# oakink/OakInk2-TaMF

Measured on AMD Instinct MI355X. Metric: sampled motion frames/s (1000-step DDPM, arch_mdm_l), higher is better.
Workload: dtype f16x3; 1 GPU; arch_mdm_l B=64/GPU T=196 1000-step DDPM (BASELINE.json configs[1]: arch_mdm_l B=64 T=196 1000-step DDPM on 1 GPU); step = one full reverse loop; headline dtype f16x3 = split-fp16 operands, fp32-TOLERANCE mode (1e-5 vs the reference, checked in-run); the same workload in the reference's own fp32 arithmetic is under roofline.reference_arithmetic (and the top-level fp32 entry); preset=2, clips_per_gpu=64, frames=196, ddpm_steps=1000, global_clips=64, parallelism=single GPU, world_size_seen=1, hipgraph=True, kernels_per_ddpm_step=43

## Files before the change

### oakink2-tamf_amd/csrc/tamf_attn.h

```cpp
#pragma once
#include "tamf_device.h"

template <class Op>
struct AttnArgs {
  const typename Op::elem_t* qk;
  const typename Op::elem_t* vt;
  typename Op::elem_t* out;
  int S, Sp, Skp, d, H;
  int abl;
  int ksplit, nwq, hw;
};

template <class Op, int HD>
struct AttnCfg {
  static constexpr int EB = Op::EB;
  static constexpr int KROWB = HD * EB;
  static constexpr int KG = KROWB / 128;
  static constexpr int VROWB = 32 * EB;
  static constexpr int VSTR = VROWB;
  static constexpr int K_BYTES = 32 * KROWB;
  static constexpr int V_BYTES = HD * VSTR;
  static constexpr int STAGE = K_BYTES + V_BYTES;
  static constexpr int SMEM = 2 * STAGE;
  static_assert(KROWB % 128 == 0, "head slice must be whole 128-byte groups");
};

template <class Op, int HD>
struct AttnBlock {
  typedef AttnCfg<Op, HD> C;
  static constexpr int EB = Op::EB, KG = C::KG, NT16 = HD / 16;
  static constexpr int KCH = C::KROWB / 16;
  static constexpr int VCH = C::VROWB / 16;
  static TAMF_DEV int kswz(int ch, int row) {
    if constexpr (C::KROWB >= 256) return (ch & ~15) | ((ch ^ row) & 15);
    else return ch ^ ((row >> 1) & 7);
  }
  static TAMF_DEV int vswz(int ch, int e) {
    if constexpr (C::VROWB == 128) return ch ^ ((e >> 1) & 7);
    else return ch ^ swz_chunk<64>(e);
  }
  static constexpr int K_RPP = 1024 / C::KROWB, K_PIECES = C::K_BYTES / 1024;
  static constexpr int V_RPP = 1024 / C::VROWB, V_PIECES = C::V_BYTES / 1024;

  static TAMF_DEV void issue(char* __restrict__ st, const char* kbase, const char* vbase, int kb, int Sp, int d, int Skp,
                             int wave, int nw, int lane) {
    for (int q = wave; q < K_PIECES; q += nw) {
      const int r = q * K_RPP + lane / KCH, pc = lane % KCH;
      int key = kb * 32 + r;
      key = key < Sp ? key : Sp - 1;
      __builtin_amdgcn_global_load_lds((const __attribute__((address_space(1))) void*)(kbase + (long)key * (2 * d) * EB + kswz(pc, r) * 16),
                                       (__attribute__((address_space(3))) void*)(st + q * 1024), 16, 0, 0);
    }
    for (int q = wave; q < V_PIECES; q += nw) {
      const int e = q * V_RPP + lane / VCH, pc = lane % VCH;
      __builtin_amdgcn_global_load_lds((const __attribute__((address_space(1))) void*)(vbase + ((long)e * Skp + kb * 32) * EB + vswz(pc, e) * 16),
                                       (__attribute__((address_space(3))) void*)(st + C::K_BYTES + q * 1024), 16, 0, 0);
    }
  }

  static TAMF_DEV void run(const char* __restrict__ cur, char* __restrict__ nxt, const char* kbase, const char* vbase,
                           int kb, int nkb, int S, int Sp, int d, int Skp, int wave, int nw, int lane, bool active,
                           const int4 (&qf)[KG][2], f32x4 (&o)[NT16], float& m_run, float& l_run) {
    const int lr = lane & 15, g = lane >> 4;
    const char* Ks = cur;
    const char* Vs = cur + C::K_BYTES;
    if (kb + 1 < nkb) issue(nxt, kbase, vbase, kb + 1, Sp, d, Skp, wave, nw, lane);
    if (!active) return;

    f32x4 st[2];
#pragma unroll
    for (int t = 0; t < 2; ++t) {
      st[t] = f32x4{0.f, 0.f, 0.f, 0.f};
      const int row = t * 16 + lr;
#pragma unroll
      for (int kg = 0; kg < KG; ++kg) {
        int4 kf[2];
        kf[0] = *(const int4*)(Ks + row * C::KROWB + kswz(kg * 8 + g, row) * 16);
        kf[1] = *(const int4*)(Ks + row * C::KROWB + kswz(kg * 8 + 4 + g, row) * 16);
        Op::mma(st[t], kf, qf[kg]);
      }
    }
    if (kb == nkb - 1) {
#pragma unroll
      for (int t = 0; t < 2; ++t)
#pragma unroll
        for (int r = 0; r < 4; ++r)
          if (kb * 32 + t * 16 + 4 * g + r >= S) st[t][r] = -1e30f;
    }
    float bm = fmaxf(fmaxf(fmaxf(st[0][0], st[0][1]), fmaxf(st[0][2], st[0][3])),
                     fmaxf(fmaxf(st[1][0], st[1][1]), fmaxf(st[1][2], st[1][3])));
    bm = groups_reduce<RedMax>(bm);
    constexpr float RESCALE_LOG2 = 8.0f;
    if (__builtin_amdgcn_ballot_w64(bm > m_run + RESCALE_LOG2) != 0ull) {
      const float m_new = fmaxf(m_run, bm);
      const float alpha = __builtin_amdgcn_exp2f(m_run - m_new);
      l_run *= alpha;
      m_run = m_new;
#pragma unroll
      for (int nt = 0; nt < NT16; ++nt) o[nt] *= alpha;
    }
    float ps = 0.f;
#pragma unroll
    for (int t = 0; t < 2; ++t)
#pragma unroll
      for (int r = 0; r < 4; ++r) {
        st[t][r] = __builtin_amdgcn_exp2f(st[t][r] - m_run);
        ps += st[t][r];
      }
    ps = groups_reduce<RedSum>(ps);
    l_run += ps;

    if constexpr (Op::PREC == 0) {
#pragma unroll
      for (int nt = 0; nt < NT16; ++nt) {
        const int e = nt * 16 + lr;
#pragma unroll
        for (int t = 0; t < 2; ++t) {
          const int4 vf = *(const int4*)(Vs + e * C::VSTR + vswz(t * 4 + g, e) * 16);
          o[nt] = __builtin_amdgcn_mfma_f32_16x16x4f32(as_f(vf.x), st[t][0], o[nt], 0, 0, 0);
          o[nt] = __builtin_amdgcn_mfma_f32_16x16x4f32(as_f(vf.y), st[t][1], o[nt], 0, 0, 0);
          o[nt] = __builtin_amdgcn_mfma_f32_16x16x4f32(as_f(vf.z), st[t][2], o[nt], 0, 0, 0);
          o[nt] = __builtin_amdgcn_mfma_f32_16x16x4f32(as_f(vf.w), st[t][3], o[nt], 0, 0, 0);
        }
      }
    } else {
      uint32_t wh[4], wl[4];
#pragma unroll
      for (int j = 0; j < 4; ++j) {
        const float p0 = st[(2 * j) >> 2][(2 * j) & 3], p1 = st[(2 * j + 1) >> 2][(2 * j + 1) & 3];
        Op::split2(p0, p1, wh[j], wl[j]);
      }
      const int4 ph = make_int4((int)wh[0], (int)wh[1], (int)wh[2], (int)wh[3]);
      const int4 pl = make_int4((int)wl[0], (int)wl[1], (int)wl[2], (int)wl[3]);
#pragma unroll
      for (int nt = 0; nt < NT16; ++nt) {
        const int e = nt * 16 + lr;
        const int4 vh = *(const int4*)(Vs + e * C::VSTR + vswz(g, e) * 16);
        if constexpr (Op::SPLIT) {
          const int4 vl = *(const int4*)(Vs + e * C::VSTR + vswz(4 + g, e) * 16);
          o[nt] = Op::mfma1(vl, ph, o[nt]);
          o[nt] = Op::mfma1(vh, pl, o[nt]);
        }
        o[nt] = Op::mfma1(vh, ph, o[nt]);
      }
    }
  }
};

#ifdef TAMF_TIMELINE
__device__ unsigned long long g_attn_ts[8192 * 4];
#endif

template <class Op, int HD>
__global__ __launch_bounds__(1024) void attn_kernel(const AttnArgs<Op> aa) {
  TAMF_TS(ts0);
  typedef AttnCfg<Op, HD> C;
  typedef AttnBlock<Op, HD> BLK;
  constexpr int EB = Op::EB, KG = C::KG;
  constexpr int NT16 = HD / 16;
  extern __shared__ __attribute__((aligned(16))) char smem[];

  const int tid = threadIdx.x, nthr = blockDim.x;
  const int lane = tid & 63, nw = nthr >> 6;
  const int wave = __builtin_amdgcn_readfirstlane(tid >> 6);
  const int lr = lane & 15, g = lane >> 4;
  const int bh = blockIdx.y, b = bh / aa.H, h = bh % aa.H;
  const int q0 = (blockIdx.x * nw + wave) * 16;
  const bool active = q0 < aa.Sp;
  const int S = aa.S, Sp = aa.Sp, d = aa.d;
  const long row_base = (long)b * Sp;

  int4 qf[KG][2];
  {
    int q = q0 + lr;
    q = q < Sp ? q : Sp - 1;
    const char* qb = (const char*)aa.qk + ((row_base + q) * (2 * d) + h * HD) * EB + g * 16;
#pragma unroll
    for (int kg = 0; kg < KG; ++kg) {
      qf[kg][0] = *(const int4*)(qb + kg * 128);
      qf[kg][1] = *(const int4*)(qb + kg * 128 + 64);
    }
  }

  f32x4 o[NT16];
#pragma unroll
  for (int nt = 0; nt < NT16; ++nt) o[nt] = f32x4{0.f, 0.f, 0.f, 0.f};
  float m_run = -1e30f, l_run = 0.f;

  const int nkb = (S + 31) / 32;
  const char* kbase = (const char*)aa.qk + (row_base * (2 * d) + d + h * HD) * EB;
  const char* vbase = (const char*)aa.vt + ((long)bh * HD) * aa.Skp * EB;

  BLK::issue(smem, kbase, vbase, 0, Sp, d, aa.Skp, wave, nw, lane);
  __syncthreads();
  TAMF_TS(ts1);
  for (int kb = 0; kb < nkb; ++kb) {
    BLK::run(smem + (kb & 1) * C::STAGE, smem + ((kb + 1) & 1) * C::STAGE, kbase, vbase, kb, nkb, S, Sp, d, aa.Skp, wave, nw,
             lane, active, qf, o, m_run, l_run);
    __syncthreads();
  }
#ifdef TAMF_TIMELINE
  if (tid == 0) {
    const int wg = blockIdx.y * gridDim.x + blockIdx.x;
    if (wg < 8192) {
      g_attn_ts[wg * 4 + 0] = ts0;
      g_attn_ts[wg * 4 + 1] = ts1;
      g_attn_ts[wg * 4 + 2] = wall_clock64();
      g_attn_ts[wg * 4 + 3] = tamf_hw_cu_id();
    }
  }
#endif

  if (!active) return;
  const int q = q0 + lr;
  if (q >= Sp) return;
  const float inv = 1.0f / l_run;
#pragma unroll
  for (int nt = 0; nt < NT16; ++nt) {
    float v[4] = {o[nt][0] * inv, o[nt][1] * inv, o[nt][2] * inv, o[nt][3] * inv};
    Op::template store<4>(aa.out, (row_base + q) * d + h * HD + nt * 16 + 4 * g, v);
  }
}

TAMF_DEV int attn_xcd_remap(int bid, int nblk) {
  const int q = nblk >> 3, r = nblk & 7, x = bid & 7, i = bid >> 3;
  return (x < r ? x * (q + 1) : r * (q + 1) + (x - r) * q) + i;
}

constexpr int attn_res_maxw(int nkb) { return nkb <= 4 ? 8 : 16; }
template <class Op, int HD, int NKB_>
struct AttnRes {
  typedef AttnCfg<Op, HD> C;
  typedef AttnBlock<Op, HD> BLK;
  static constexpr int EB = Op::EB, KG = C::KG, NT16 = HD / 16;
  static constexpr int NKB = NKB_, NKT = 2 * NKB;
  static constexpr int MAXW = attn_res_maxw(NKB_);
  static constexpr int S_MIN = NKB_ <= 4 ? 1 : NKB_ <= 6 ? 129 : 193;
  static constexpr int LDS_MAX = 160 * 1024;
  static constexpr bool TWO = Op::SPLIT || Op::PREC == 0;

  static int k_bytes(int Sp) { return Sp * C::KROWB; }
  static int nv1(int Sp, int nkb) {
    const int fit = (LDS_MAX - k_bytes(Sp)) / C::V_BYTES;
    return fit < nkb ? fit : nkb;
  }
  static bool fits(int S, int Sp) {
    const int nkb = (S + 31) / 32;
    if (nkb > NKB || S < S_MIN || Sp > NKT * 16 || (k_bytes(Sp) % 1024) != 0) return false;
    const int n1 = nv1(Sp, nkb);
    return n1 >= 1 && (nkb - n1) * C::V_BYTES <= k_bytes(Sp);
  }
  static int smem(int S, int Sp) {
    const int need = k_bytes(Sp) + nv1(Sp, (S + 31) / 32) * C::V_BYTES, rows = NKT * 16 * C::KROWB;
    return need > rows ? need : rows;
  }

  static constexpr int TPC_ = EB == 4 ? 2 : 4, NCH_ = (NT16 + TPC_ - 1) / TPC_, TPCE_ = NT16 < TPC_ ? NT16 : TPC_;
  static constexpr int KSPLIT_BYTES = NCH_ * 3 * TPCE_ * 1024 + 512;
  static int ksplit_extra(int S, int Sp, int nwq) {
    const int nkb = (S + 31) / 32, n1 = nv1(Sp, nkb), base = smem(S, Sp);
    int extra;
    if (n1 < nkb) {
      const int end = k_bytes(Sp) + nwq * 2048 + KSPLIT_BYTES;
      extra = end > base ? end - base : 0;
    } else {
      extra = KSPLIT_BYTES;
    }
    return base + extra <= LDS_MAX ? extra : -1;
  }

  static TAMF_DEV void issue_k(char* Ks, const char* kbase, int r0, int r1, int d, int wave, int nw, int lane) {
    const int q0 = r0 / BLK::K_RPP, np = r1 / BLK::K_RPP;
    for (int q = q0 + wave; q < np; q += nw) {
      const int r = q * BLK::K_RPP + lane / BLK::KCH, pc = lane % BLK::KCH;
      __builtin_amdgcn_global_load_lds((const __attribute__((address_space(1))) void*)(kbase + (long)r * (2 * d) * EB + BLK::kswz(pc, r) * 16),
                                       (__attribute__((address_space(3))) void*)(Ks + q * 1024), 16, 0, 0);
    }
  }
  static TAMF_DEV void issue_v(char* dst, const char* vbase, int kb0, int kb1, int Skp, int wave, int nw, int lane) {
    const int np = (kb1 - kb0) * BLK::V_PIECES;
    for (int q = wave; q < np; q += nw) {
      const int kb = kb0 + q / BLK::V_PIECES, qq = q % BLK::V_PIECES;
      const int e = qq * BLK::V_RPP + lane / BLK::VCH, pc = lane % BLK::VCH;
      __builtin_amdgcn_global_load_lds((const __attribute__((address_space(1))) void*)(vbase + ((long)e * Skp + kb * 32) * EB + BLK::vswz(pc, e) * 16),
                                       (__attribute__((address_space(3))) void*)(dst + q * 1024), 16, 0, 0);
    }
  }

  struct KOff { int o[KG][2]; };
  static TAMF_DEV KOff koff(int lr, int g) {
    KOff k;
#pragma unroll
    for (int kg = 0; kg < KG; ++kg) {
      k.o[kg][0] = lr * C::KROWB + BLK::kswz(kg * 8 + g, lr) * 16;
      k.o[kg][1] = lr * C::KROWB + BLK::kswz(kg * 8 + 4 + g, lr) * 16;
    }
    return k;
  }
  static TAMF_DEV void kfrag(const char* Ks, int i, const KOff& ko, int4 (&kf)[2]) {
    const int kt = i / KG, kg = i % KG;
    kf[0] = *(const int4*)(Ks + kt * (16 * C::KROWB) + ko.o[kg][0]);
    kf[1] = *(const int4*)(Ks + kt * (16 * C::KROWB) + ko.o[kg][1]);
  }
  template <int T0, int T1>
  static TAMF_DEV void scores(const char* __restrict__ Ks, char* __restrict__ K2, char* __restrict__ Vs, const char* kbase,
                              const char* vbase, int k2r0, int k2r1, int d, int n1, int Skp, int wave, int nw, int lane,
                              const int4 (&qf)[KG][2], f32x4 (&st)[NKT], int abl, unsigned mask = ~0u) {
    const int lr = lane & 15, g = lane >> 4;
    if (T0 == 0 && !(abl & 1)) {
      if (k2r1 > k2r0) issue_k(K2 - (long)k2r0 * C::KROWB, kbase, k2r0, k2r1, d, wave, nw, lane);
      issue_v(Vs, vbase, 0, n1, Skp, wave, nw, lane);
    }
    constexpr int F0 = T0 * KG, NF = T1 * KG, LA = 2;
    const KOff ko = koff(lr, g);
    int4 kf[LA + 1][2];
#pragma unroll
    for (int i = 0; i <= LA; ++i) kf[i][0] = kf[i][1] = qf[0][0];
    auto on = [&](int i) { return ((mask >> (i / KG / 2)) & 1u) != 0; };
#pragma unroll
    for (int i = F0; i < F0 + LA; ++i)
      if (!(abl & 4) && on(i)) kfrag(Ks, i, ko, kf[i % (LA + 1)]);
#pragma unroll
    for (int i = F0; i < NF; ++i) {
      if (i + LA < NF && !(abl & 4) && on(i + LA)) kfrag(Ks, i + LA, ko, kf[(i + LA) % (LA + 1)]);
      __builtin_amdgcn_sched_barrier(0);
      if (on(i)) {
        if (i % KG == 0) st[i / KG] = f32x4{0.f, 0.f, 0.f, 0.f};
        if (!(abl & 2)) Op::mma(st[i / KG], kf[i % (LA + 1)], qf[i % KG]);
      }
      __builtin_amdgcn_sched_barrier(0);
    }
  }
  static TAMF_DEV void vfrag(const char* vb, int nt, int vo0, int vo1, int4 (&vf)[2]) {
    vf[0] = *(const int4*)(vb + nt * (16 * C::VSTR) + vo0);
    if constexpr (TWO) vf[1] = *(const int4*)(vb + nt * (16 * C::VSTR) + vo1);
  }
  static TAMF_DEV void pv(const char* __restrict__ Vs, char* __restrict__ dma_dst, const char* vbase, int kb0, int kb1, int dkb0,
                          int dkb1, int Skp, int wave, int nw, int lane, const uint32_t (&ph)[NKB][4], const uint32_t (&pl)[NKB][4],
                          f32x4 (&o)[NT16], int abl, unsigned mask = ~0u) {
    const int lr = lane & 15, g = lane >> 4;
    const int vo0 = lr * C::VSTR + BLK::vswz(g, lr) * 16, vo1 = lr * C::VSTR + BLK::vswz(4 + g, lr) * 16;
    if (dkb1 > dkb0 && !(abl & 1)) issue_v(dma_dst, vbase, dkb0, dkb1, Skp, wave, nw, lane);
#pragma unroll
    for (int kb = 0; kb < NKB; ++kb) {
      if (kb >= kb0 && kb < kb1 && ((mask >> kb) & 1u)) {
        const char* vb = Vs + (kb - kb0) * C::V_BYTES;
        const int4 p_h = make_int4((int)ph[kb][0], (int)ph[kb][1], (int)ph[kb][2], (int)ph[kb][3]);
        const int4 p_l = make_int4((int)pl[kb][0], (int)pl[kb][1], (int)pl[kb][2], (int)pl[kb][3]);
        constexpr int LA = 2;
        int4 vf[LA + 1][2];
#pragma unroll
        for (int nt = 0; nt <= LA; ++nt) vf[nt][0] = vf[nt][1] = p_h;
#pragma unroll
        for (int nt = 0; nt < LA; ++nt)
          if (!(abl & 4)) vfrag(vb, nt, vo0, vo1, vf[nt]);
#pragma unroll
        for (int nt = 0; nt < NT16; ++nt) {
          if (nt + LA < NT16 && !(abl & 4)) vfrag(vb, nt + LA, vo0, vo1, vf[(nt + LA) % (LA + 1)]);
          __builtin_amdgcn_sched_barrier(0);
          const int4 vh = vf[nt % (LA + 1)][0];
          if (!(abl & 2)) {
            if constexpr (Op::PREC == 0) {
              const int4 v1 = vf[nt % (LA + 1)][1];
              o[nt] = __builtin_amdgcn_mfma_f32_16x16x4f32(as_f(vh.x), __builtin_bit_cast(float, ph[kb][0]), o[nt], 0, 0, 0);
              o[nt] = __builtin_amdgcn_mfma_f32_16x16x4f32(as_f(vh.y), __builtin_bit_cast(float, ph[kb][1]), o[nt], 0, 0, 0);
              o[nt] = __builtin_amdgcn_mfma_f32_16x16x4f32(as_f(vh.z), __builtin_bit_cast(float, ph[kb][2]), o[nt], 0, 0, 0);
              o[nt] = __builtin_amdgcn_mfma_f32_16x16x4f32(as_f(vh.w), __builtin_bit_cast(float, ph[kb][3]), o[nt], 0, 0, 0);
              o[nt] = __builtin_amdgcn_mfma_f32_16x16x4f32(as_f(v1.x), __builtin_bit_cast(float, pl[kb][0]), o[nt], 0, 0, 0);
              o[nt] = __builtin_amdgcn_mfma_f32_16x16x4f32(as_f(v1.y), __builtin_bit_cast(float, pl[kb][1]), o[nt], 0, 0, 0);
              o[nt] = __builtin_amdgcn_mfma_f32_16x16x4f32(as_f(v1.z), __builtin_bit_cast(float, pl[kb][2]), o[nt], 0, 0, 0);
              o[nt] = __builtin_amdgcn_mfma_f32_16x16x4f32(as_f(v1.w), __builtin_bit_cast(float, pl[kb][3]), o[nt], 0, 0, 0);
            } else {
              if constexpr (Op::SPLIT) {
                const int4 vl = vf[nt % (LA + 1)][1];
                o[nt] = Op::mfma1(vl, p_h, o[nt]);
                o[nt] = Op::mfma1(vh, p_l, o[nt]);
              }
              o[nt] = Op::mfma1(vh, p_h, o[nt]);
            }
          }
          __builtin_amdgcn_sched_barrier(0);
        }
      }
    }
  }
};

template <class Op, int HD, int NKB_>
__global__ __launch_bounds__(attn_res_maxw(NKB_) * 64) void attn_res_kernel(const AttnArgs<Op> aa) {
  typedef AttnCfg<Op, HD> C;
  typedef AttnRes<Op, HD, NKB_> R;
  constexpr int EB = Op::EB, KG = C::KG, NT16 = HD / 16, NKB = R::NKB, NKT = R::NKT;
  extern __shared__ __attribute__((aligned(16))) char smem[];

  const int tid = threadIdx.x, nthr = blockDim.x;
  const int lane = tid & 63, nw = nthr >> 6;
  const int wave = __builtin_amdgcn_readfirstlane(tid >> 6);
  const int lr = lane & 15, g = lane >> 4;
  int bh = blockIdx.y;
  if (gridDim.x == 1 && !(TAMF_ABL(aa.abl) & 32)) bh = attn_xcd_remap(bh, gridDim.y);
  const int b = bh / aa.H, h = bh % aa.H;
  const int S = aa.S, Sp = aa.Sp, d = aa.d;
  const int nwq = aa.ksplit ? aa.nwq : nw;
  const int nqt = (Sp + 15) / 16;
  const int nqt_own = aa.ksplit ? nqt - 1 : nqt;
  int tile = blockIdx.x * nwq + wave;
  int hq = -1;
  unsigned kmask = ~0u;
  bool idle = wave >= nwq || tile >= nqt_own;
  if (aa.ksplit && blockIdx.x == gridDim.x - 1) {
#pragma unroll
    for (int j = 0; j < 4; ++j)
      if (wave == ((aa.hw >> (4 * j)) & 15)) hq = j;
    if (hq >= 0) { idle = false; tile = nqt - 1; kmask = 0x11111111u << hq; }
  }
  if (idle) { kmask = 0u; tile = nqt - 1; }
  const int q0 = tile * 16;
  const long row_base = (long)b * Sp;
  const int nkb = (S + 31) / 32;
  const int kbytes = Sp * C::KROWB;
  int n1 = (R::LDS_MAX - kbytes) / C::V_BYTES;
  n1 = n1 < nkb ? n1 : nkb;
  char* Ks = smem;
  char* Vs = smem + kbytes;

  const char* kbase = (const char*)aa.qk + (row_base * (2 * d) + d + h * HD) * EB;
  const char* vbase = (const char*)aa.vt + ((long)bh * HD) * aa.Skp * EB;

  int4 qf[KG][2];
  {
    int q = q0 + lr;
    q = q < Sp ? q : Sp - 1;
    const char* qb = (const char*)aa.qk + ((row_base + q) * (2 * d) + h * HD) * EB + g * 16;
#pragma unroll
    for (int kg = 0; kg < KG; ++kg) {
      qf[kg][0] = *(const int4*)(qb + kg * 128);
      qf[kg][1] = *(const int4*)(qb + kg * 128 + 64);
    }
  }
  const int abl = TAMF_ABL(aa.abl);
  constexpr int TH = NKT / 2;
  const int kh = TH * 16 < Sp ? TH * 16 : Sp;
  if (!(abl & 1)) R::issue_k(Ks, kbase, 0, kh, d, wave, nw, lane);
  __syncthreads();

  f32x4 st[NKT];
  if (kmask != ~0u) {
#pragma unroll
    for (int kt = 0; kt < NKT; ++kt) st[kt] = f32x4{-1e30f, -1e30f, -1e30f, -1e30f};
  }
  R::template scores<0, TH>(Ks, Ks + (long)kh * C::KROWB, Vs, kbase, vbase, kh, Sp, d, n1, aa.Skp, wave, nw, lane, qf, st, abl, kmask);
  __syncthreads();
  R::template scores<TH, NKT>(Ks, Vs, Vs, kbase, vbase, 0, 0, d, 0, aa.Skp, wave, nw, lane, qf, st, abl, kmask);

#pragma unroll
  for (int kt = 0; kt < NKT; ++kt)
    if (kt * 16 + 15 >= R::S_MIN) {
#pragma unroll
      for (int r = 0; r < 4; ++r) st[kt][r] = (kt * 16 + 4 * g + r >= S) ? -1e30f : st[kt][r];
    }
  float m = -1e30f;
#pragma unroll
  for (int kt = 0; kt < NKT; ++kt) m = fmaxf(m, fmaxf(fmaxf(st[kt][0], st[kt][1]), fmaxf(st[kt][2], st[kt][3])));
  m = groups_reduce<RedMax>(m);
  float l = 0.f;
  uint32_t ph[NKB][4], pl[NKB][4];
#pragma unroll
  for (int kb = 0; kb < NKB; ++kb) {
#pragma unroll
    for (int t = 0; t < 2; ++t)
#pragma unroll
      for (int r = 0; r < 4; ++r) {
        const float p = (abl & 8) ? st[2 * kb + t][r] : __builtin_amdgcn_exp2f(st[2 * kb + t][r] - m);
        st[2 * kb + t][r] = p;
        l += p;
      }
#pragma unroll
    for (int j = 0; j < 4; ++j) {
      if constexpr (Op::PREC == 0) {
        const float p0 = st[2 * kb][j], p1 = st[2 * kb + 1][j];
        ph[kb][j] = __builtin_bit_cast(uint32_t, p0);
        pl[kb][j] = __builtin_bit_cast(uint32_t, p1);
      } else {
        if (abl & 8) { const float pa = st[2 * kb + (j >> 1)][(2 * j) & 3]; ph[kb][j] = pl[kb][j] = __builtin_bit_cast(uint32_t, pa); }
        else Op::split2(st[2 * kb + (j >> 1)][(2 * j) & 3], st[2 * kb + (j >> 1)][((2 * j) & 3) + 1], ph[kb][j], pl[kb][j]);
      }
    }
  }
  l = groups_reduce<RedSum>(l);

  f32x4 o[NT16];
#pragma unroll
  for (int nt = 0; nt < NT16; ++nt) o[nt] = f32x4{0.f, 0.f, 0.f, 0.f};

  __syncthreads();
  R::pv(Vs, Ks, vbase, 0, n1, n1, nkb, aa.Skp, wave, nw, lane, ph, pl, o, abl, kmask);
  if (n1 < nkb) {
    __syncthreads();
    R::pv(Ks, Vs, vbase, n1, nkb, 0, 0, aa.Skp, wave, nw, lane, ph, pl, o, abl, kmask);
  }
  if (idle) {
    if (aa.ksplit) __syncthreads();
    return;
  }

  if ((abl & 16) && l != 12345.0f) return;
  constexpr int TPC = Op::EB == 4 ? 2 : 4;
  constexpr int NCH = (NT16 + TPC - 1) / TPC, TPCE = NT16 < TPC ? NT16 : TPC;
  if (hq >= 0) {
    const int base_bytes = kbytes + n1 * C::V_BYTES > NKT * 16 * C::KROWB ? kbytes + n1 * C::V_BYTES : NKT * 16 * C::KROWB;
    char* part = n1 < nkb ? Vs + nwq * 2048 : smem + base_bytes;
    float* ml = (float*)(part + NCH * 3 * TPCE * 1024);
    if (g == 0) { ml[hq * 32 + lr] = m; ml[hq * 32 + 16 + lr] = l; }
#pragma unroll
    for (int ch = 0; ch < NCH; ++ch)
      if (ch != hq) {
        const int src = hq < ch ? hq : hq - 1;
#pragma unroll
        for (int tl = 0; tl < TPCE; ++tl) *(f32x4*)(part + ((ch * 3 + src) * TPCE + tl) * 1024 + lane * 16) = o[ch * TPC + tl];
      }
    __syncthreads();
    if (hq >= NCH || q0 + lr >= Sp) return;
    float mi[4], li[4], mg = -1e30f;
#pragma unroll
    for (int i = 0; i < 4; ++i) { mi[i] = ml[i * 32 + lr]; li[i] = ml[i * 32 + 16 + lr]; mg = fmaxf(mg, mi[i]); }
    float w[4], lg = 0.f;
#pragma unroll
    for (int i = 0; i < 4; ++i) { w[i] = __builtin_amdgcn_exp2f(mi[i] - mg); lg += li[i] * w[i]; }
    const float invg = 1.0f / lg;
    char* grow = (char*)aa.out + ((row_base + q0 + lr) * d + h * HD) * EB + hq * 128;
#pragma unroll
    for (int ch = 0; ch < NCH; ++ch) {
      if (ch != hq) continue;
#pragma unroll
      for (int tl = 0; tl < TPCE; ++tl) {
        f32x4 acc = f32x4{0.f, 0.f, 0.f, 0.f};
#pragma unroll
        for (int i = 0; i < 4; ++i) {
          const f32x4 mine = o[ch * TPC + tl];
          const f32x4 theirs = *(const f32x4*)(part + ((ch * 3 + (i < ch ? i : (i > 0 ? i - 1 : 0))) * TPCE + tl) * 1024 + lane * 16);
          const f32x4 oi = i == ch ? mine : theirs;
          acc += oi * w[i];
        }
        const float v0 = acc[0] * invg, v1 = acc[1] * invg, v2 = acc[2] * invg, v3 = acc[3] * invg;
        if constexpr (Op::PREC == 0) {
          *(int4*)(grow + (4 * tl + g) * 16) = make_int4(as_i(v0), as_i(v1), as_i(v2), as_i(v3));
        } else {
          uint32_t h0, l0, h1, l1;
          Op::split2(v0, v1, h0, l0);
          Op::split2(v2, v3, h1, l1);
          char* gp = grow + (2 * tl + (g >> 1)) * 16 + 8 * (g & 1);
          *(int2*)gp = make_int2((int)h0, (int)h1);
          if constexpr (Op::SPLIT) *(int2*)(gp + 64) = make_int2((int)l0, (int)l1);
        }
      }
    }
    return;
  }
  const float inv = 1.0f / l;
  constexpr int RS = 128;
  char* slot = (n1 < nkb ? Vs : Ks) + wave * (16 * RS);
  char* gout = (char*)aa.out + ((row_base + q0) * d + h * HD) * EB;
  const int srow = lane >> 3, spiece = lane & 7;
#pragma unroll
  for (int ch = 0; ch < NCH; ++ch) {
#pragma unroll
    for (int tl = 0; tl < TPCE; ++tl) {
      const int nt = ch * TPC + tl;
      const float v0 = o[nt][0] * inv, v1 = o[nt][1] * inv, v2 = o[nt][2] * inv, v3 = o[nt][3] * inv;
      if (q0 + lr >= Sp) continue;
      if constexpr (Op::PREC == 0) {
        const int c = 4 * tl + g;
        *(int4*)(slot + lr * RS + ((c ^ (lr & 7)) << 4)) = make_int4(as_i(v0), as_i(v1), as_i(v2), as_i(v3));
      } else {
        uint32_t h0, l0, h1, l1;
        Op::split2(v0, v1, h0, l0);
        Op::split2(v2, v3, h1, l1);
        const int c = 2 * tl + (g >> 1);
        char* sp = slot + lr * RS + 8 * (g & 1);
        *(int2*)(sp + ((c ^ (lr & 7)) << 4)) = make_int2((int)h0, (int)h1);
        if constexpr (Op::SPLIT) *(int2*)(sp + (((c + 4) ^ (lr & 7)) << 4)) = make_int2((int)l0, (int)l1);
      }
    }
#pragma unroll
    for (int i = 0; i < 2; ++i) {
      const int row = i * 8 + srow;
      const int4 w = *(const int4*)(slot + row * RS + ((spiece ^ (row & 7)) << 4));
      if (q0 + row < Sp && (NT16 >= TPC || spiece * 16 < NT16 * 16 * Op::EB))
        *(int4*)(gout + (long)row * d * EB + ch * 128 + spiece * 16) = w;
    }
  }
  if (aa.ksplit) __syncthreads();
}
```

### oakink2-tamf_amd/csrc/tamf_hip.hip

```cpp
#include "../../include/tamf_hip.h"

#include <hip/hip_runtime.h>

#include <algorithm>
#include <atomic>
#include <cmath>
#include <cstdio>
#include <cstdlib>
#include <cstring>
#include <map>
#include <mutex>
#include <string>
#include <type_traits>
#include <vector>

#include "tamf_attn.h"
#include "tamf_gemm.h"
#include "tamf_gemm_clip.h"
#include "tamf_gemm_deep.h"
#include "tamf_geom.h"
#include "tamf_misc.h"
#include "tamf_encoder.h"
#include "tamf_spectrum.h"
#include "tamf_shapes.h"
#include "tamf_weight_prep.h"

#define TAMF_WITH_OP(prec, EXPR)                                         \
  switch (prec) {                                                        \
    case TAMF_PREC_F32: { typedef OpF32 Op; EXPR; } break;               \
    case TAMF_PREC_BF16: { typedef OpBF16 Op; EXPR; } break;             \
    case TAMF_PREC_BF16X3: { typedef OpBF16X3 Op; EXPR; } break;         \
    default: { typedef OpF16X3 Op; EXPR; } break;                        \
  }

static thread_local std::string g_noctx_err;

struct OperandBuf {
  void* p = nullptr;
  float inv_scale = 1.0f;
};

struct LayerW {
  OperandBuf Win, Wout, W1, W2;
  float *c2_in = nullptr, *c2_ff = nullptr;
  float *g_att = nullptr, *bb_att = nullptr, *g_ffn = nullptr, *bb_ffn = nullptr;
};

struct GraphKey {
  int B = -1, T = -1, n_steps = -1, steps_per_graph = 0;
  bool operator==(const GraphKey& o) const {
    return B == o.B && T == o.T && n_steps == o.n_steps && steps_per_graph == o.steps_per_graph;
  }
};

struct GuardRec {
  char* base;
  size_t bytes, guard;
  const char* tag;
  bool ws;
};
static constexpr unsigned char GUARD_BYTE = 0xA5;
static std::atomic<size_t> g_guard_bytes{0};
static thread_local const char* g_alloc_tag = "";

struct Workspaces {
  int Bmax = 0, Tmax = 0;
  long Mmax = 0;
  float *xs = nullptr, *cobj = nullptr, *X = nullptr, *pstatic = nullptr;
  OperandBuf xs_op, h1_op, X_op, QK_op, Vt_op, A_op, H_op;
  void *X_st = nullptr, *xs_st = nullptr;
  int* tcur = nullptr;
  unsigned* status = nullptr;
  unsigned char* side_dev = nullptr;
  int* objnum_dev = nullptr;
  float2 *stat_att = nullptr, *stat_ffn = nullptr;
  LoopParams* loop_params = nullptr;
  std::vector<void*> ws_allocs;
};

struct tamf_ctx : Workspaces {
  tamf_arch arch{};
  int prec = 0, device = 0;
  int d = 0, ff = 0, L = 0, H = 0, hd = 0, P = 0, F = 0, has_t = 0;
  int XK = 0;
  int XN = 128;
  int EB = 4;
  std::string err;
  std::vector<void*> allocs;
  bool alloc_ws = false;
  std::vector<GuardRec> guards;
  std::map<std::string, std::vector<int64_t>> expected;
  std::map<std::string, std::vector<float>> raw;
  bool finalized = false, cond_set = false;
  int n_t = 0;
  int n_steps = 0;
  std::vector<float> h_c1, h_c2, h_sigma;
  float *c1 = nullptr, *c2 = nullptr, *sigma = nullptr;
  std::vector<LayerW> layers;
  OperandBuf Wfused, Wm2, Wf;
  float *bm2 = nullptr, *bf = nullptr;
  float* pe = nullptr;
  float* temb = nullptr;
  float* temb_loop = nullptr;
  int temb_loop_cap = 0;
  bool tmap_on = false, in_loop = false;
  int tmap_max = -1;
  OperandBuf Wt1_f32, Wt2_f32;
  float *bt1 = nullptr, *bt2 = nullptr;
  float *WtxtT = nullptr, *btxt = nullptr, *WshapeT = nullptr, *bshape = nullptr, *WobjT = nullptr, *bobj = nullptr;
  float *WcT = nullptr, *bc = nullptr, *rh = nullptr, *lh = nullptr;
  int B = 0, T = 0, S = 0, Sp = 0, Skp = 0, M = 0;
  float* enc_w = nullptr;
  int enc_kin = 0;
  unsigned host_status = 0;
  std::string weight_note;
  hipStream_t cap_stream = nullptr;
  hipGraph_t graph = nullptr;
  hipGraphExec_t graph_exec = nullptr;
  GraphKey graph_key;
  hipEvent_t graph_done = nullptr;
  bool graph_in_flight = false;
  int sched_cap = 0;
  int graph_captures = 0, graph_launches_last_loop = 0;
  int step_kernels = 0;
  bool prof_on = false;
  std::vector<hipEvent_t> prof_ev;
  std::vector<std::string> prof_names;
  std::vector<double> prof_flops;
};

static std::vector<tamf_ctx*> g_live_ctx;
static std::mutex g_live_mu;
static std::recursive_mutex g_launch_mu;
#ifdef TAMF_TEST_HOOKS
#define TAMF_LAUNCH_LOCK std::lock_guard<std::recursive_mutex> launch_lock_(g_launch_mu)
#else
#define TAMF_LAUNCH_LOCK ((void)0)
#endif
#define TAMF_STATE_LOCK std::lock_guard<std::recursive_mutex> state_lock_(g_launch_mu)

static int fail(tamf_ctx* ctx, int code, const std::string& msg) {
  if (ctx) ctx->err = msg;
  else g_noctx_err = msg;
  return code;
}
static int launched() {
  const hipError_t e = hipGetLastError();
  return e == hipSuccess ? 0 : fail(nullptr, TAMF_ERR_HIP, hipGetErrorString(e));
}
enum : unsigned { KIND_G = 1u << TAMF_KIND_G, KIND_R = 1u << TAMF_KIND_R, KIND_E = 1u << TAMF_KIND_E };
static int need_kind(tamf_ctx* ctx, const char* func, unsigned mask) {
  if (!ctx) return fail(ctx, TAMF_ERR_INVALID, std::string(func) + ": null ctx");
  if (mask & (1u << ctx->arch.kind)) return 0;
  if (ctx->arch.kind == TAMF_KIND_E) return fail(ctx, TAMF_ERR_STATE, std::string(func) + ": not available on a SegmentEncoder (TAMF_KIND_E) context");
  return fail(ctx, TAMF_ERR_STATE, std::string(func) + (mask == KIND_E   ? " needs a SegmentEncoder (TAMF_KIND_E) context"
                                                        : mask == KIND_G ? " needs a G context"
                                                        : mask == KIND_R ? " needs an R context"
                                                                         : " needs a G or R context"));
}
#define HIPCHK(ctx, call)                                                                                         \
  do {                                                                                                            \
    hipError_t e_ = (call);                                                                                       \
    if (e_ != hipSuccess)                                                                                         \
      return fail(ctx, TAMF_ERR_HIP, std::string(#call) + ": " + hipGetErrorString(e_) + " (" + __FILE__ + ":" +  \
                                         std::to_string(__LINE__) + ")");                                        \
  } while (0)
#define TRY(expr)           \
  do {                      \
    int rc_ = (expr);       \
    if (rc_ != 0) return rc_; \
  } while (0)

static inline dim3 grid1d(long n, int bs = 256) { return dim3((unsigned)((n + bs - 1) / bs)); }

static std::atomic<int> g_fail_alloc_in{-1};
static int dev_alloc(tamf_ctx* ctx, void** p, size_t bytes, bool zero = false) {
  if (bytes == 0) bytes = 16;
  const size_t guard = g_guard_bytes.load();
  if (g_fail_alloc_in.load() >= 0 && g_fail_alloc_in.fetch_sub(1) == 0)
    return fail(ctx, TAMF_ERR_NOMEM, "hipMalloc failed: injected by tamf_test_fail_alloc_after");
  hipError_t e = hipMalloc(p, bytes + 2 * guard);
  if (e != hipSuccess) return fail(ctx, TAMF_ERR_NOMEM, std::string("hipMalloc failed: ") + hipGetErrorString(e));
  (ctx->alloc_ws ? ctx->ws_allocs : ctx->allocs).push_back(*p);
  if (guard) {
    char* base = (char*)*p;
    HIPCHK(ctx, hipMemset(base, GUARD_BYTE, guard));
    HIPCHK(ctx, hipMemset(base + guard + bytes, GUARD_BYTE, guard));
    ctx->guards.push_back(GuardRec{base, bytes, guard, g_alloc_tag, ctx->alloc_ws});
    *p = base + guard;
  }
  if (zero) HIPCHK(ctx, hipMemset(*p, 0, bytes));
  return 0;
}
template <class T>
static int dev_upload(tamf_ctx* ctx, T** p, const T* host, size_t n) {
  TRY(dev_alloc(ctx, (void**)p, n * sizeof(T)));
  HIPCHK(ctx, hipMemcpy(*p, host, n * sizeof(T), hipMemcpyHostToDevice));
  return 0;
}

static int upload_operand(tamf_ctx* ctx, int prec, const float* w, int N, int K, int ldk, OperandBuf* out, const char* what) {
  const PackedOperand po = pack_operand(prec, w, N, K, ldk);
  if (po.refused) return fail(ctx, po.error_code(), po.error_message(what));
  out->inv_scale = po.inv_scale;
  if (po.small_share_noted()) {
    ctx->host_status |= TAMF_STATUS_F16_WEIGHT_RANGE;
    if (ctx->weight_note.empty()) ctx->weight_note = po.range_note(what);
  }
  return dev_upload(ctx, (unsigned char**)&out->p, po.image.data(), po.image.size());
}
static int upload_vec(tamf_ctx* ctx, float** p, const std::vector<float>& v) { return dev_upload(ctx, p, v.data(), v.size()); }

#include "tamf_launch.h"

extern "C" const char* tamf_last_error(const tamf_ctx* ctx) { return ctx ? ctx->err.c_str() : g_noctx_err.c_str(); }

static int alloc_operand(tamf_ctx* ctx, OperandBuf* ob, long elems, bool zero = false) {
  return dev_alloc(ctx, &ob->p, (size_t)elems * ctx->EB, zero);
}

static int check_dims(const tamf_arch* arch, int max_batch, int max_frames) {
  if (max_batch <= 0 || max_frames <= 0 || max_frames > 4990) return fail(nullptr, TAMF_ERR_INVALID, "bad max_batch/max_frames");
  if (!dims_fit_32bit_offsets(max_batch, max_frames, arch->ff_size, arch->latent_dim))
    return fail(nullptr, TAMF_ERR_INVALID, "max_batch x max_frames too large for one context (32-bit operand offsets): split the batch");
  return 0;
}

static int place_scratch_views(tamf_ctx* ctx, const ScratchLayout& sl) {
  char* host = (char*)ctx->H_op.p;
  ctx->QK_op.p = host + sl.qk_off;
  ctx->A_op.p = host + sl.a_off;
  ctx->h1_op.p = host + sl.h1_off;
  const size_t guard = g_guard_bytes.load();
  if (!guard) return 0;
  const struct { size_t off, bytes; const char* tag; } views[3] = {{(size_t)sl.qk_off, (size_t)sl.qk_bytes, "view QK_op of H_op's allocation"},
                                                                  {(size_t)sl.a_off, (size_t)sl.a_bytes, "view A_op of H_op's allocation"},
                                                                  {(size_t)sl.h1_off, (size_t)sl.h1_bytes, "view h1_op of H_op's allocation"}};
  for (const auto& v : views) {
    HIPCHK(ctx, hipMemset(host + v.off - guard, GUARD_BYTE, guard));
    ctx->guards.push_back(GuardRec{host + v.off - guard, v.bytes, guard, v.tag, true});
  }
  return 0;
}

static int alloc_workspaces(tamf_ctx* ctx, int max_batch, int max_frames) {
  const int d = ctx->d;
  const SeqShape smax = seq_shape_max(max_frames, ctx->P);
  const long BT = (long)max_batch * max_frames;
  const long Mmax = (long)max_batch * smax.Sp;
  ctx->Mmax = Mmax;
  ctx->Bmax = max_batch;
  ctx->Tmax = max_frames;
  ctx->alloc_ws = true;
  int rc = 0;
#define A(call)             \
  do {                      \
    g_alloc_tag = #call;    \
    if (rc == 0) rc = call; \
  } while (0)
  A(dev_alloc(ctx, (void**)&ctx->xs, BT * ctx->XK * 4, true));
  if (ctx->prec == TAMF_PREC_F32) ctx->xs_op.p = ctx->xs;
  else { A(alloc_operand(ctx, &ctx->xs_op, BT * ctx->XK, true)); ctx->xs_st = ctx->xs_op.p; }
  A(dev_alloc(ctx, (void**)&ctx->cobj, BT * d * 4));
  const ScratchLayout sl = scratch_layout(Mmax, BT, d, ctx->ff, ctx->EB, g_guard_bytes.load());
  if (!sl.alias) A(alloc_operand(ctx, &ctx->h1_op, BT * d));
  A(dev_alloc(ctx, (void**)&ctx->X, Mmax * d * 4, true));
  if (ctx->prec == TAMF_PREC_F32) ctx->X_op.p = ctx->X;
  else { A(alloc_operand(ctx, &ctx->X_op, Mmax * d, true)); ctx->X_st = ctx->X_op.p; }
  if (!sl.alias) A(alloc_operand(ctx, &ctx->QK_op, Mmax * 2 * d, true));
  A(alloc_operand(ctx, &ctx->Vt_op, (long)max_batch * d * smax.Skp, true));
  if (!sl.alias) A(alloc_operand(ctx, &ctx->A_op, Mmax * d, true));
  if (!sl.alias) A(alloc_operand(ctx, &ctx->H_op, Mmax * ctx->ff, true));
  else {
    A(dev_alloc(ctx, &ctx->H_op.p, sl.host_bytes, true));
    A(place_scratch_views(ctx, sl));
  }
  A(dev_alloc(ctx, (void**)&ctx->pstatic, (long)max_batch * ctx->P * d * 4, true));
  A(dev_alloc(ctx, (void**)&ctx->tcur, (long)max_batch * 4, true));
  A(dev_alloc(ctx, (void**)&ctx->status, 16, true));
  A(dev_alloc(ctx, (void**)&ctx->side_dev, max_batch, true));
  A(dev_alloc(ctx, (void**)&ctx->objnum_dev, (long)max_batch * 4, true));
  A(dev_alloc(ctx, (void**)&ctx->stat_att, Mmax * (d / 32) * 8, true));
  A(dev_alloc(ctx, (void**)&ctx->stat_ffn, Mmax * (d / 32) * 8, true));
  A(dev_alloc(ctx, (void**)&ctx->loop_params, sizeof(LoopParams), true));
#undef A
  g_alloc_tag = "(weights / tables)";
  ctx->alloc_ws = false;
  return rc;
}

static int enc_max_frames(int ff, int kin) {
  int t = 0;
  while (t < 5000 && enc_lds_bytes(t + 1 + ENC_P + 1, ff, kin) <= ENC_LDS_BYTES) ++t;
  return t;
}
static int enc_check_shape(const tamf_arch* a, int max_batch, int max_frames) {
  if (a->latent_dim != ENC_D || a->num_heads != 4)
    return fail(nullptr, TAMF_ERR_INVALID, "SegmentEncoder (TAMF_KIND_E): latent_dim must be 64 with num_heads 4 (head dim 16)");
  if (a->ff_size < 16 || a->ff_size > 512 || a->ff_size % 16)
    return fail(nullptr, TAMF_ERR_INVALID, "SegmentEncoder (TAMF_KIND_E): ff_size must be a multiple of 16 in [16, 512]");
  if (a->num_layers < 1 || a->num_layers > 64) return fail(nullptr, TAMF_ERR_INVALID, "SegmentEncoder (TAMF_KIND_E): num_layers must be in [1, 64]");
  if (a->input_dim < 1 || a->input_dim > 128 || a->obj_input_dim < 1 || a->obj_input_dim > 16 || a->hand_shape_dim < 1 ||
      a->hand_shape_dim > 64 || a->obj_embed_dim < 1 || a->obj_embed_dim > 4096)
    return fail(nullptr, TAMF_ERR_INVALID, "SegmentEncoder (TAMF_KIND_E): input_dim must be in [1, 128], obj_input_dim in [1, 16], "
                                           "hand_shape_dim in [1, 64], obj_embed_dim in [1, 4096]");
  if (max_batch <= 0 || max_batch > (1 << 20) || max_frames <= 0) return fail(nullptr, TAMF_ERR_INVALID, "bad max_batch/max_frames");
  const int tmax = enc_max_frames(a->ff_size, round_up(a->input_dim + a->obj_input_dim, 4));
  if (max_frames > tmax)
    return fail(nullptr, TAMF_ERR_INVALID, "SegmentEncoder (TAMF_KIND_E): max_frames " + std::to_string(max_frames) + " exceeds the limit of " +
                                               std::to_string(tmax) + " frames (a clip's token rows live in the 160 KiB LDS of one CU)");
  return 0;
}
static int enc_alloc_workspaces(tamf_ctx* ctx, int max_batch, int max_frames) {
  ctx->Bmax = max_batch;
  ctx->Tmax = max_frames;
  ctx->alloc_ws = true;
  g_alloc_tag = "encoder workspaces";
  int rc = dev_alloc(ctx, (void**)&ctx->pstatic, (size_t)max_batch * ENC_P * ctx->d * 4, true);
  if (rc == 0) rc = dev_alloc(ctx, (void**)&ctx->objnum_dev, (size_t)max_batch * 4, true);
  g_alloc_tag = "(weights / tables)";
  ctx->alloc_ws = false;
  return rc;
}
static int alloc_workspaces_of_kind(tamf_ctx* ctx, int max_batch, int max_frames) {
  return ctx->arch.kind == TAMF_KIND_E ? enc_alloc_workspaces(ctx, max_batch, max_frames) : alloc_workspaces(ctx, max_batch, max_frames);
}

static int enc_check_create(const tamf_arch* arch, int max_batch, int max_frames, int precision) {
  if (precision != TAMF_PREC_F32) return fail(nullptr, TAMF_ERR_INVALID, "SegmentEncoder (TAMF_KIND_E) runs in fp32 only (TAMF_PREC_F32)");
  return enc_check_shape(arch, max_batch, max_frames);
}
static int gr_check_arch(const tamf_arch* arch, int precision) {
  const int d = arch->latent_dim;
  if (!(d == 128 || d == 256 || d == 512)) return fail(nullptr, TAMF_ERR_INVALID, "latent_dim must be 128, 256 or 512");
  if (arch->num_heads <= 0 || d % arch->num_heads) return fail(nullptr, TAMF_ERR_INVALID, "bad num_heads");
  const int hd = d / arch->num_heads;
  if (!(hd == 64 || hd == 128)) return fail(nullptr, TAMF_ERR_INVALID, "head dim (latent_dim/num_heads) must be 64 or 128");
  if (arch->ff_size <= 0 || arch->ff_size % 128) return fail(nullptr, TAMF_ERR_INVALID, "ff_size must be a multiple of 128");
  if (arch->num_layers <= 0 || arch->num_layers > 64) return fail(nullptr, TAMF_ERR_INVALID, "bad num_layers");
  if (arch->input_dim <= 0 || arch->input_dim > 128) return fail(nullptr, TAMF_ERR_INVALID, "input_dim must be in [1,128]");
  if (precision < 0 || precision > TAMF_PREC_F16X3) return fail(nullptr, TAMF_ERR_INVALID, "unknown precision");
  if (arch->kind != TAMF_KIND_G && arch->kind != TAMF_KIND_R) return fail(nullptr, TAMF_ERR_INVALID, "unknown model kind");
  return 0;
}
static int enc_prepare(tamf_ctx* ctx) {
  hipError_t e = lds_once<encoder_kernel>((int)ENC_LDS_BYTES);
  if (e != hipSuccess) return fail(ctx, TAMF_ERR_HIP, std::string("encoder kernel attribute setup failed: ") + hipGetErrorString(e));
  return 0;
}
static int gr_prepare(tamf_ctx* ctx) {
  {
    int cus = 0;
    if (hipDeviceGetAttribute(&cus, hipDeviceAttributeMultiprocessorCount, ctx->device) == hipSuccess && cus > 0)
      g_wg_slots_dev[ctx->device & 63].store(2 * cus, std::memory_order_relaxed);
  }
  hipError_t pe;
  {
    TAMF_STATE_LOCK;
    pe = prepare_all<OpF32>();
    if (pe == hipSuccess && ctx->prec != TAMF_PREC_F32) TAMF_WITH_OP(ctx->prec, pe = prepare_all<Op>());
  }
  if (pe != hipSuccess) return fail(ctx, TAMF_ERR_HIP, std::string("kernel attribute setup failed: ") + hipGetErrorString(pe));
  if (hipStreamCreateWithFlags(&ctx->cap_stream, hipStreamNonBlocking) != hipSuccess) return fail(ctx, TAMF_ERR_HIP, "hipStreamCreate failed");
  return 0;
}

extern "C" int tamf_ctx_create(const tamf_arch* arch, int32_t max_batch, int32_t max_frames, int32_t precision,
                               int32_t device, tamf_ctx** out) {
  if (!arch || !out) return fail(nullptr, TAMF_ERR_INVALID, "null argument");
  *out = nullptr;
  const bool enc = arch->kind == TAMF_KIND_E;
  if (int rc = enc ? enc_check_create(arch, max_batch, max_frames, precision) : gr_check_arch(arch, precision)) return rc;
  int ndev = 0;
  hipError_t de = hipGetDeviceCount(&ndev);
  if (de != hipSuccess || ndev <= 0)
    return fail(nullptr, TAMF_ERR_HIP, std::string("no HIP device visible (") + hipGetErrorString(de) +
                                           "): libtamf_hip has no CPU fallback");
  if (device < 0 || device >= ndev) return fail(nullptr, TAMF_ERR_INVALID, "device index out of range");
  if (!enc)
    if (int rc = check_dims(arch, max_batch, max_frames)) return rc;

  tamf_ctx* ctx = new tamf_ctx();
  ctx->arch = *arch;
  ctx->prec = precision;
  ctx->device = device;
  ctx->d = arch->latent_dim;
  ctx->ff = arch->ff_size;
  ctx->L = arch->num_layers;
  ctx->H = arch->num_heads;
  ctx->hd = arch->latent_dim / arch->num_heads;
  ctx->F = arch->input_dim;
  ctx->has_t = arch->kind == TAMF_KIND_G ? 1 : 0;
  ctx->EB = precision == TAMF_PREC_BF16 ? 2 : 4;
  if (enc) {
    ctx->P = ENC_P;
    ctx->enc_kin = round_up(arch->input_dim + arch->obj_input_dim, 4);
  } else {
    ctx->P = arch->kind == TAMF_KIND_G ? PREFIX_ROWS_G : PREFIX_ROWS_R;
    ctx->XK = arch->kind == TAMF_KIND_G ? 128 : round_up(arch->input_dim + arch->h2o_dim, 64);
    ctx->layers.resize(ctx->L);
  }
  ctx->expected = expected_shapes(ctx->arch);

  auto bail = [&](int rc) {
    std::string e = ctx->err;
    tamf_ctx_destroy(ctx);
    g_noctx_err = e;
    return rc;
  };
  if (hipSetDevice(device) != hipSuccess) return bail(fail(ctx, TAMF_ERR_HIP, "hipSetDevice failed"));
  if (int rc = enc ? enc_prepare(ctx) : gr_prepare(ctx)) return bail(rc);
  if (int rc = alloc_workspaces_of_kind(ctx, max_batch, max_frames)) return bail(rc);
  if (!enc && hipEventCreateWithFlags(&ctx->graph_done, hipEventDisableTiming) != hipSuccess)
    return bail(fail(ctx, TAMF_ERR_HIP, "hipEventCreate failed"));
  {
    std::lock_guard<std::mutex> lk(g_live_mu);
    g_live_ctx.push_back(ctx);
  }
  *out = ctx;
  return 0;
}

extern "C" void tamf_ctx_destroy(tamf_ctx* ctx) {
  if (!ctx) return;
  TAMF_LAUNCH_LOCK;
  {
    std::lock_guard<std::mutex> lk(g_live_mu);
    g_live_ctx.erase(std::remove(g_live_ctx.begin(), g_live_ctx.end(), ctx), g_live_ctx.end());
  }
  (void)hipSetDevice(ctx->device);
  (void)hipDeviceSynchronize();
  if (ctx->graph_done) (void)hipEventDestroy(ctx->graph_done);
  if (ctx->graph_exec) (void)hipGraphExecDestroy(ctx->graph_exec);
  if (ctx->graph) (void)hipGraphDestroy(ctx->graph);
  if (ctx->cap_stream) (void)hipStreamDestroy(ctx->cap_stream);
  for (void* p : ctx->allocs) (void)hipFree(p);
  for (void* p : ctx->ws_allocs) (void)hipFree(p);
  delete ctx;
}

static int retire_graph(tamf_ctx* ctx);

struct TakenWorkspaces {
  Workspaces ws;
  std::vector<GuardRec> guards;
};
static TakenWorkspaces ws_take(tamf_ctx* c) {
  TakenWorkspaces t;
  std::swap(t.ws, static_cast<Workspaces&>(*c));
  const auto first_ws = std::stable_partition(c->guards.begin(), c->guards.end(), [](const GuardRec& g) { return !g.ws; });
  t.guards.assign(first_ws, c->guards.end());
  c->guards.erase(first_ws, c->guards.end());
  return t;
}
static void ws_put(tamf_ctx* c, TakenWorkspaces& t) {
  std::swap(t.ws, static_cast<Workspaces&>(*c));
  c->guards.insert(c->guards.end(), t.guards.begin(), t.guards.end());
}
static void ws_free(const TakenWorkspaces& t) {
  for (void* p : t.ws.ws_allocs) (void)hipFree(p);
}

extern "C" int tamf_ctx_resize(tamf_ctx* ctx, int32_t max_batch, int32_t max_frames) {
  TAMF_LAUNCH_LOCK;
  if (!ctx) return fail(ctx, TAMF_ERR_INVALID, "null ctx");
  const bool enc = ctx->arch.kind == TAMF_KIND_E;
  if (int rc = enc ? enc_check_shape(&ctx->arch, max_batch, max_frames) : check_dims(&ctx->arch, max_batch, max_frames)) {
    ctx->err = g_noctx_err;
    return rc;
  }
  HIPCHK(ctx, hipSetDevice(ctx->device));
  HIPCHK(ctx, hipDeviceSynchronize());
  if (!enc) TRY(retire_graph(ctx));
  TakenWorkspaces old = ws_take(ctx);
  int rc = alloc_workspaces_of_kind(ctx, max_batch, max_frames);
  if (rc == 0 && old.ws.status && ctx->status &&
      hipMemcpy(ctx->status, old.ws.status, 16, hipMemcpyDeviceToDevice) != hipSuccess)
    rc = fail(ctx, TAMF_ERR_HIP, "tamf_ctx_resize: carrying the status word over failed");
  if (rc != 0) {
    const std::string why = ctx->err;
    ws_free(ws_take(ctx));
    ws_put(ctx, old);
    ctx->err = "tamf_ctx_resize(" + std::to_string(max_batch) + ", " + std::to_string(max_frames) + ") failed, the context keeps its " +
               std::to_string(ctx->Bmax) + " x " + std::to_string(ctx->Tmax) + " workspaces: " + why;
    return rc;
  }
  ws_free(old);
  if (!enc) {
    ctx->cond_set = false;
    ctx->B = ctx->T = ctx->S = ctx->Sp = ctx->Skp = ctx->M = 0;
  }
  return 0;
}

extern "C" int tamf_load_weight(tamf_ctx* ctx, const char* name, const float* host_data, const int64_t* shape,
                                int32_t ndim) {
  if (!ctx || !name || !host_data || !shape || ndim <= 0) return fail(ctx, TAMF_ERR_INVALID, "null/invalid argument");
  if (ctx->finalized) return fail(ctx, TAMF_ERR_STATE, "weights already finalised");
  const auto it = ctx->expected.find(name);
  if (it == ctx->expected.end()) return 0;
  std::vector<int64_t> shp(shape, shape + ndim);
  if (shp != it->second) return fail(ctx, TAMF_ERR_INVALID, std::string("shape mismatch for ") + name);
  int64_t n = 1;
  for (auto v : shp) n *= v;
  ctx->raw[name].assign(host_data, host_data + n);
  return 0;
}

static int upload_f32(tamf_ctx* ctx, const std::string& name, float** p) {
  const auto& v = ctx->raw.at(name);
  return dev_upload(ctx, p, v.data(), v.size());
}
static int upload_T(tamf_ctx* ctx, const std::string& name, int N, int K, float** p) {
  return upload_vec(ctx, p, transposed(ctx->raw.at(name).data(), N, K));
}
static int upload_prefix_tables(tamf_ctx* ctx) {
  const int d = ctx->d;
  TRY(upload_T(ctx, "hand_shape_process.shape_embed.weight", d, ctx->arch.hand_shape_dim, &ctx->WshapeT));
  TRY(upload_f32(ctx, "hand_shape_process.shape_embed.bias", &ctx->bshape));
  TRY(upload_T(ctx, "obj_embed_process.embedding.weight", d, ctx->arch.obj_embed_dim, &ctx->WobjT));
  TRY(upload_f32(ctx, "obj_embed_process.embedding.bias", &ctx->bobj));
  TRY(upload_f32(ctx, "hand_side_process.rh_embed", &ctx->rh));
  return upload_f32(ctx, "hand_side_process.lh_embed", &ctx->lh);
}
static int enc_finalize(tamf_ctx* ctx) {
  const int d = ctx->d, ff = ctx->ff, F = ctx->F, qd = ctx->arch.obj_input_dim, kin = ctx->enc_kin, hd = ctx->hd, H = ctx->H;
  auto R = [&](const std::string& n) -> const float* { return ctx->raw.at(n).data(); };
  const EncHeadOff ho = enc_head_off(kin, F);
  const EncLayerOff lo = enc_layer_off(ff);
  std::vector<float> w((size_t)(ho.layers + (long)ctx->L * lo.stride), 0.f);
  auto put = [&](long off, const std::string& n, size_t cnt) { memcpy(w.data() + off, R(n), cnt * 4); };
  put(ho.cls, "classification_token", d);
  {
    const float *Wm1 = R("input_merge.0.weight"), *bm1 = R("input_merge.0.bias");
    const float *Wp = R("input_process.poseEmbedding.weight"), *bp = R("input_process.poseEmbedding.bias");
    const float *Wq = R("obj_input_process.poseEmbedding.weight"), *bq = R("obj_input_process.poseEmbedding.bias");
    input_bias_two_terms_per_column(Wm1, d, bm1, bp, bq, w.data() + ho.bin);
    compose_block(Wm1, 2 * d, 0, d, Wp, F, w.data() + ho.win, kin, 1);
    compose_block(Wm1, 2 * d, d, d, Wq, qd, w.data() + ho.win + F, kin, 1);
  }
  put(ho.wm2, "input_merge.2.weight", (size_t)d * d);
  put(ho.bm2, "input_merge.2.bias", d);
  put(ho.p0, "output_process.poseFinal.0.weight", (size_t)d * d);
  put(ho.pb0, "output_process.poseFinal.0.bias", d);
  put(ho.p2, "output_process.poseFinal.2.weight", (size_t)d * d);
  put(ho.pb2, "output_process.poseFinal.2.bias", d);
  put(ho.p4, "output_process.poseFinal.4.weight", (size_t)F * d);
  put(ho.pb4, "output_process.poseFinal.4.bias", F);
  for (int l = 0; l < ctx->L; ++l) {
    const std::string p = "seqTransEncoder.layers." + std::to_string(l);
    const long base = ho.layers + (long)l * lo.stride;
    const float *Win = R(p + ".self_attn.in_proj_weight"), *bin = R(p + ".self_attn.in_proj_bias");
    for (int h = 0; h < H; ++h)
      for (int part = 0; part < 3; ++part)
        for (int j = 0; j < hd; ++j) {
          const int dst = h * 3 * hd + part * hd + j, src = part * d + h * hd + j;
          memcpy(w.data() + base + lo.wqkv + (long)dst * d, Win + (size_t)src * d, (size_t)d * 4);
          w[base + lo.bqkv + dst] = bin[src];
        }
    put(base + lo.wo, p + ".self_attn.out_proj.weight", (size_t)d * d);
    put(base + lo.bo, p + ".self_attn.out_proj.bias", d);
    put(base + lo.w1, p + ".linear1.weight", (size_t)ff * d);
    put(base + lo.b1, p + ".linear1.bias", ff);
    put(base + lo.w2, p + ".linear2.weight", (size_t)d * ff);
    put(base + lo.b2, p + ".linear2.bias", d);
    put(base + lo.g1, p + ".norm1.weight", d);
    put(base + lo.be1, p + ".norm1.bias", d);
    put(base + lo.g2, p + ".norm2.weight", d);
    put(base + lo.be2, p + ".norm2.bias", d);
  }
  TRY(dev_upload(ctx, &ctx->enc_w, w.data(), w.size()));
  TRY(upload_f32(ctx, "sequence_pos_encoder.pe", &ctx->pe));
  return upload_prefix_tables(ctx);
}

extern "C" int tamf_finalize_weights(tamf_ctx* ctx, int32_t max_timesteps, void* stream) {
  TAMF_LAUNCH_LOCK;
  if (!ctx) return fail(ctx, TAMF_ERR_INVALID, "null ctx");
  if (ctx->finalized) return fail(ctx, TAMF_ERR_STATE, "weights already finalised");
  if (max_timesteps <= 0 || max_timesteps > 5000) return fail(ctx, TAMF_ERR_INVALID, "max_timesteps must be in [1,5000]");
  HIPCHK(ctx, hipSetDevice(ctx->device));
  hipStream_t st = (hipStream_t)stream;
  for (const auto& kv : ctx->expected)
    if (!ctx->raw.count(kv.first)) return fail(ctx, TAMF_ERR_MISSING, "missing checkpoint tensor: " + kv.first);
  auto done = [&]() {
    ctx->raw.clear();
    ctx->expected.clear();
    ctx->finalized = true;
    if (!ctx->weight_note.empty()) ctx->err = ctx->weight_note;
    return 0;
  };
  if (ctx->arch.kind == TAMF_KIND_E) {
    TRY(enc_finalize(ctx));
    return done();
  }
  const int d = ctx->d, ff = ctx->ff, F = ctx->F, prec = ctx->prec;
  auto R = [&](const std::string& n) -> const float* { return ctx->raw.at(n).data(); };
  auto upload_folded = [&](const std::string& weight, const std::string& bias, int N, int Npad, const float* g, const float* be, OperandBuf* ob,
                           float** c2) -> int {
    const FoldedLinear f = fold_layernorm(R(weight), R(bias), N, Npad, d, g, be);
    TRY(upload_operand(ctx, prec, f.w.data(), Npad, d, d, ob, weight.c_str()));
    return upload_vec(ctx, c2, f.c2);
  };
  auto upload_residual_ln = [&](const float* g, const float* be, const std::string& bias, float** g_dev, float** bb_dev) -> int {
    const ResidualLn r = residual_ln(g, be, R(bias), d);
    TRY(upload_vec(ctx, g_dev, r.g));
    return upload_vec(ctx, bb_dev, r.bb);
  };

  for (int l = 0; l < ctx->L; ++l) {
    const std::string p = "seqTransEncoder.layers." + std::to_string(l);
    LayerW& w = ctx->layers[l];
    {
      const std::string pp = "seqTransEncoder.layers." + std::to_string(l - 1);
      const float* g_in = l ? R(pp + ".norm2.weight") : nullptr;
      const float* be_in = l ? R(pp + ".norm2.bias") : nullptr;
      const float* g1 = R(p + ".norm1.weight");
      const float* be1 = R(p + ".norm1.bias");
      TRY(upload_folded(p + ".self_attn.in_proj_weight", p + ".self_attn.in_proj_bias", 3 * d, 3 * d, g_in, be_in, &w.Win, &w.c2_in));
      TRY(upload_folded(p + ".linear1.weight", p + ".linear1.bias", ff, ff, g1, be1, &w.W1, &w.c2_ff));
      TRY(upload_residual_ln(g_in, be_in, p + ".self_attn.out_proj.bias", &w.g_att, &w.bb_att));
      TRY(upload_residual_ln(g1, be1, p + ".linear2.bias", &w.g_ffn, &w.bb_ffn));
    }
    TRY(upload_operand(ctx, prec, R(p + ".self_attn.out_proj.weight"), d, d, d, &w.Wout, (p + ".self_attn.out_proj.weight").c_str()));
    TRY(upload_operand(ctx, prec, R(p + ".linear2.weight"), d, ff, ff, &w.W2, (p + ".linear2.weight").c_str()));
  }
  {
    const bool isR = ctx->arch.kind == TAMF_KIND_R;
    const FusedInput fi = fuse_input(d, F, ctx->arch.obj_input_dim, ctx->arch.h2o_dim, ctx->XK, R("input_merge.0.weight"), R("input_merge.0.bias"),
                                     R("input_process.poseEmbedding.weight"), R("input_process.poseEmbedding.bias"),
                                     R("obj_input_process.poseEmbedding.weight"), R("obj_input_process.poseEmbedding.bias"),
                                     isR ? R("h2o_dist_input_process.poseEmbedding.weight") : nullptr,
                                     isR ? R("h2o_dist_input_process.poseEmbedding.bias") : nullptr);
    TRY(upload_operand(ctx, prec, fi.w.data(), d, ctx->XK, ctx->XK, &ctx->Wfused, "input_merge.0.weight x poseEmbedding.weight (fused)"));
    TRY(upload_vec(ctx, &ctx->WcT, fi.wct));
    TRY(upload_vec(ctx, &ctx->bc, fi.bias));
  }
  TRY(upload_operand(ctx, prec, R("input_merge.2.weight"), d, d, d, &ctx->Wm2, "input_merge.2.weight"));
  TRY(upload_f32(ctx, "input_merge.2.bias", &ctx->bm2));
  {
    const std::string pl = "seqTransEncoder.layers." + std::to_string(ctx->L - 1);
    TRY(upload_folded("output_process.poseFinal.weight", "output_process.poseFinal.bias", F, ctx->XN, R(pl + ".norm2.weight"), R(pl + ".norm2.bias"),
                      &ctx->Wf, &ctx->bf));
  }
  TRY(upload_f32(ctx, "sequence_pos_encoder.pe", &ctx->pe));
  if (ctx->arch.hand_shape_dim > 64 || ctx->arch.obj_input_dim > COBJ_QMAX || d > 1024)
    return fail(ctx, TAMF_ERR_INVALID, "hand_shape_dim > 64, obj_input_dim > 16 or latent_dim > 1024");
  TRY(upload_prefix_tables(ctx));
  if (ctx->has_t) {
    TRY(upload_T(ctx, "embed_text.weight", d, ctx->arch.clip_dim, &ctx->WtxtT));
    TRY(upload_f32(ctx, "embed_text.bias", &ctx->btxt));
    TRY(upload_operand(ctx, TAMF_PREC_F32, R("embed_timestep.time_embed.0.weight"), d, d, d, &ctx->Wt1_f32, "embed_timestep.time_embed.0.weight"));
    TRY(upload_operand(ctx, TAMF_PREC_F32, R("embed_timestep.time_embed.2.weight"), d, d, d, &ctx->Wt2_f32, "embed_timestep.time_embed.2.weight"));
    TRY(upload_f32(ctx, "embed_timestep.time_embed.0.bias", &ctx->bt1));
    TRY(upload_f32(ctx, "embed_timestep.time_embed.2.bias", &ctx->bt2));
    ctx->n_t = max_timesteps;
    float* tmp = nullptr;
    TRY(dev_alloc(ctx, (void**)&ctx->temb, (size_t)ctx->n_t * d * 4));
    TRY(dev_alloc(ctx, (void**)&tmp, (size_t)ctx->n_t * d * 4));
    GemmArgs<OpF32> g1{ctx->pe, d, (const float*)ctx->Wt1_f32.p, d, ctx->n_t, d, d, 0};
    EpiBiasAct<OpF32> e1{ctx->bt1, nullptr, 0, tmp, d, ACT_SILU};
    HIPCHK(ctx, gemm128<OpF32>(g1, e1, st));
    GemmArgs<OpF32> g2{tmp, d, (const float*)ctx->Wt2_f32.p, d, ctx->n_t, d, d, 0};
    EpiSeqRows<OpF32> e2{ctx->bt2, ctx->pe, 0, ctx->temb, nullptr, d, 0x7FFFFFFF, 0, 0, nullptr, nullptr, nullptr, 0, 0, 0};
    HIPCHK(ctx, gemm128<OpF32>(g2, e2, st));
  }
  HIPCHK(ctx, hipStreamSynchronize(st));
  return done();
}

static int retire_graph(tamf_ctx* ctx) {
  if (ctx->graph_in_flight) {
    HIPCHK(ctx, hipEventSynchronize(ctx->graph_done));
    ctx->graph_in_flight = false;
  }
  if (ctx->graph_exec) { (void)hipGraphExecDestroy(ctx->graph_exec); ctx->graph_exec = nullptr; }
  if (ctx->graph) { (void)hipGraphDestroy(ctx->graph); ctx->graph = nullptr; }
  ctx->graph_key = GraphKey();
  return 0;
}

extern "C" int tamf_set_schedule(tamf_ctx* ctx, int32_t n_steps, const double* c1, const double* c2, const double* logvar) {
  TAMF_LAUNCH_LOCK;
  TRY(need_kind(ctx, __func__, KIND_G | KIND_R));
  if (!c1 || !c2 || !logvar || n_steps <= 0) return fail(ctx, TAMF_ERR_INVALID, "null/invalid argument");
  HIPCHK(ctx, hipSetDevice(ctx->device));
  ctx->h_c1.resize(n_steps);
  ctx->h_c2.resize(n_steps);
  ctx->h_sigma.resize(n_steps);
  for (int i = 0; i < n_steps; ++i) {
    ctx->h_c1[i] = (float)c1[i];
    ctx->h_c2[i] = (float)c2[i];
    ctx->h_sigma[i] = expf(0.5f * (float)logvar[i]);
  }
  ctx->n_steps = n_steps;
  if (ctx->tmap_on) {
    TRY(retire_graph(ctx));
    ctx->tmap_on = false;
    ctx->tmap_max = -1;
  }
  if (n_steps > ctx->sched_cap) {
    TRY(retire_graph(ctx));
    const int cap = std::max(n_steps, 1000);
    TRY(dev_alloc(ctx, (void**)&ctx->c1, (size_t)cap * 4));
    TRY(dev_alloc(ctx, (void**)&ctx->c2, (size_t)cap * 4));
    TRY(dev_alloc(ctx, (void**)&ctx->sigma, (size_t)cap * 4));
    ctx->sched_cap = cap;
  }
  HIPCHK(ctx, hipDeviceSynchronize());
  HIPCHK(ctx, hipMemcpy(ctx->c1, ctx->h_c1.data(), (size_t)n_steps * 4, hipMemcpyHostToDevice));
  HIPCHK(ctx, hipMemcpy(ctx->c2, ctx->h_c2.data(), (size_t)n_steps * 4, hipMemcpyHostToDevice));
  HIPCHK(ctx, hipMemcpy(ctx->sigma, ctx->h_sigma.data(), (size_t)n_steps * 4, hipMemcpyHostToDevice));
  return 0;
}

extern "C" int tamf_set_timestep_map(tamf_ctx* ctx, int32_t n_steps, const int32_t* map_host) {
  TAMF_LAUNCH_LOCK;
  TRY(need_kind(ctx, __func__, KIND_G));
  if (!ctx->finalized) return fail(ctx, TAMF_ERR_STATE, "tamf_set_timestep_map needs a G context with finalised weights");
  if (ctx->n_steps <= 0 || n_steps != ctx->n_steps) return fail(ctx, TAMF_ERR_STATE, "tamf_set_timestep_map: set the schedule of the same length first");
  HIPCHK(ctx, hipSetDevice(ctx->device));
  TRY(retire_graph(ctx));
  if (!map_host) {
    ctx->tmap_on = false;
    ctx->tmap_max = -1;
    return 0;
  }
  int mx = -1;
  for (int i = 0; i < n_steps; ++i) {
    if (map_host[i] < 0 || map_host[i] >= ctx->n_t)
      return fail(ctx, TAMF_ERR_INVALID, "timestep map entry " + std::to_string(map_host[i]) + " outside the timestep table (max_timesteps = " + std::to_string(ctx->n_t) + ")");
    if (i && map_host[i] <= map_host[i - 1]) return fail(ctx, TAMF_ERR_INVALID, "timestep map must be strictly increasing (respace.py:76-82)");
    mx = std::max(mx, (int)map_host[i]);
  }
  if (n_steps > ctx->temb_loop_cap) {
    const int cap = std::max(n_steps, 1000);
    TRY(dev_alloc(ctx, (void**)&ctx->temb_loop, (size_t)cap * ctx->d * 4));
    ctx->temb_loop_cap = cap;
  }
  int* map_dev = nullptr;
  HIPCHK(ctx, hipDeviceSynchronize());
  HIPCHK(ctx, hipMalloc((void**)&map_dev, (size_t)n_steps * 4));
  hipError_t e = hipMemcpy(map_dev, map_host, (size_t)n_steps * 4, hipMemcpyHostToDevice);
  if (e == hipSuccess) {
    hipLaunchKernelGGL(gather_rows_kernel, grid1d((long)n_steps * ctx->d), dim3(256), 0, nullptr, ctx->temb_loop, ctx->temb, map_dev, n_steps, ctx->d);
    e = hipGetLastError();
  }
  if (e == hipSuccess) e = hipDeviceSynchronize();
  (void)hipFree(map_dev);
  HIPCHK(ctx, e);
  ctx->tmap_on = true;
  ctx->tmap_max = mx;
  return 0;
}

static int check_obj_num(tamf_ctx* ctx, const int32_t* obj_num_host, int B, int nobj) {
  if (obj_num_host)
    for (int b = 0; b < B; ++b)
      if (obj_num_host[b] < 1 || obj_num_host[b] > nobj)
        return fail(ctx, TAMF_ERR_INVALID, "obj_num[" + std::to_string(b) + "] = " + std::to_string(obj_num_host[b]) + " outside [1, nobj]");
  return 0;
}
static int upload_obj_num(tamf_ctx* ctx, const int32_t* obj_num_host, int B, hipStream_t st, const int** cnt) {
  *cnt = nullptr;
  if (!obj_num_host) return 0;
  HIPCHK(ctx, hipMemcpyAsync(ctx->objnum_dev, obj_num_host, sizeof(int32_t) * B, hipMemcpyHostToDevice, st));
  *cnt = ctx->objnum_dev;
  return 0;
}

extern "C" int tamf_set_cond(tamf_ctx* ctx, int32_t B, int32_t T, int32_t nobj, const float* text_emb_dev,
                             const uint8_t* hand_side_host, const float* shape_dev, const float* obj_emb_dev,
                             const float* obj_traj_dev, void* stream) {
  return tamf_set_cond_ragged(ctx, B, T, nobj, nullptr, text_emb_dev, hand_side_host, shape_dev, obj_emb_dev, obj_traj_dev, stream);
}

extern "C" int tamf_set_cond_ragged(tamf_ctx* ctx, int32_t B, int32_t T, int32_t nobj, const int32_t* obj_num_host,
                                    const float* text_emb_dev, const uint8_t* hand_side_host, const float* shape_dev,
                                    const float* obj_emb_dev, const float* obj_traj_dev, void* stream) {
  TAMF_LAUNCH_LOCK;
  TRY(need_kind(ctx, __func__, KIND_G | KIND_R));
  if (!ctx->finalized) return fail(ctx, TAMF_ERR_STATE, "weights not finalised");
  if (B <= 0 || B > ctx->Bmax || T <= 0 || T > ctx->Tmax || nobj <= 0) return fail(ctx, TAMF_ERR_INVALID, "B/T/nobj out of range");
  if (!hand_side_host || !shape_dev || !obj_emb_dev || !obj_traj_dev || (ctx->has_t && !text_emb_dev))
    return fail(ctx, TAMF_ERR_INVALID, "null conditioning tensor");
  for (int b = 0; b < B; ++b)
    if (hand_side_host[b] > 1) return fail(ctx, TAMF_ERR_INVALID, "unexpected hand_side: " + std::to_string(hand_side_host[b]));
  TRY(check_obj_num(ctx, obj_num_host, B, nobj));
  HIPCHK(ctx, hipSetDevice(ctx->device));
  hipStream_t st = (hipStream_t)stream;
  const int* cnt = nullptr;
  TRY(upload_obj_num(ctx, obj_num_host, B, st, &cnt));
  const int d = ctx->d, P = ctx->P, ht = ctx->has_t, nrows = P - ht;
  ctx->B = B;
  ctx->T = T;
  const SeqShape sq = seq_shape(T, P);
  ctx->S = sq.S;
  ctx->Sp = sq.Sp;
  ctx->Skp = sq.Skp;
  ctx->M = B * sq.Sp;
  ctx->cond_set = false;
  HIPCHK(ctx, hipMemcpyAsync(ctx->side_dev, hand_side_host, B, hipMemcpyHostToDevice, st));
  const int sd = ctx->arch.hand_shape_dim, od = ctx->arch.obj_embed_dim, qd = ctx->arch.obj_input_dim, cd = ht ? ctx->arch.clip_dim : 0;
  PrefixArgs pa{};
  pa.text = ht ? text_emb_dev : nullptr; pa.WtxtT = ctx->WtxtT; pa.btxt = ctx->btxt;
  pa.side = ctx->side_dev; pa.rh = ctx->rh; pa.lh = ctx->lh;
  pa.shape = shape_dev; pa.WshapeT = ctx->WshapeT; pa.bshape = ctx->bshape;
  pa.oemb = obj_emb_dev; pa.WobjT = ctx->WobjT; pa.bobj = ctx->bobj; pa.cnt = cnt;
  pa.pe = ctx->pe; pa.pstatic = ctx->pstatic;
  pa.B = B; pa.d = d; pa.T = T; pa.sd = sd; pa.nobj = nobj; pa.od = od; pa.clip_dim = cd; pa.nrows = nrows; pa.ht = ht;
  const size_t psm = (size_t)(std::max(std::max(cd, od), sd) + 1024) * sizeof(float);
  hipLaunchKernelGGL(prefix_rows_kernel, dim3(B, nrows), dim3(1024), psm, st, pa);
  hipLaunchKernelGGL(cobj_kernel, dim3((unsigned)(((long)B * T + COBJ_ROWS - 1) / COBJ_ROWS)), dim3(256), 0, st, obj_traj_dev, ctx->WcT, ctx->bc,
                     ctx->cobj, B, nobj, T, qd, d, cnt);
  HIPCHK(ctx, hipGetLastError());
  ctx->cond_set = true;
  return 0;
}

template <class Op>
static int enqueue_step(tamf_ctx* ctx, hipStream_t st, const EpiHead<Op>& head_in, int t_off = 0) {
  typedef typename Op::elem_t E;
  const int d = ctx->d, ff = ctx->ff, B = ctx->B, T = ctx->T, S = ctx->S, Sp = ctx->Sp, M = ctx->M, P = ctx->P;
  int nk = 0;
  const double BS = (double)B * S, BT = (double)B * T, dd = d, F = ctx->F;
  auto mark = [&](const char* name, double flops) {
    ++nk;
    if (!ctx->prof_on) return;
    hipEvent_t ev;
    if (hipEventCreate(&ev) != hipSuccess) return;
    (void)hipEventRecord(ev, st);
    ctx->prof_ev.push_back(ev);
    ctx->prof_names.push_back(name);
    ctx->prof_flops.push_back(flops);
  };
  {
    GemmArgs<Op> ga{(const E*)ctx->xs_op.p, ctx->XK, (const E*)ctx->Wfused.p, ctx->XK, B * T, d, ctx->XK, 0};
    EpiBiasAct<Op> ep{nullptr, ctx->cobj, d, (E*)ctx->h1_op.p, d, ACT_SILU, {ctx->Wfused.inv_scale, ctx->status}};
    HIPCHK(ctx, gemm128<Op>(ga, ep, st));
    mark("gemm_input_merge0", BT * (2.0 * F * dd + 2.0 * dd * (ctx->arch.kind == TAMF_KIND_R ? 3 : 2) * dd +
                                    (ctx->arch.kind == TAMF_KIND_R ? 2.0 * ctx->arch.h2o_dim * dd : 0.0)));
  }
  {
    GemmArgs<Op> ga{(const E*)ctx->h1_op.p, d, (const E*)ctx->Wm2.p, d, B * T, d, d, 0};
    const float* temb_now = (ctx->in_loop && ctx->tmap_on) ? ctx->temb_loop : ctx->temb;
    EpiSeqRows<Op> ep{ctx->bm2, ctx->pe + (long)P * d, d, ctx->X, (E*)ctx->X_st, d, T, Sp, P, ctx->pstatic, temb_now, ctx->tcur, ctx->has_t, S, t_off, {ctx->Wm2.inv_scale, ctx->status}};
    HIPCHK(ctx, launch_rows<Op>(ga, ep, st));
    mark("gemm_input_merge2", BT * 2.0 * dd * dd + (ctx->has_t ? B * 4.0 * dd * dd : 0.0));
  }
  const float qscale = 1.4426950408889634f / sqrtf((float)ctx->hd);
  const int NB = d / 32;
  const float inv_d = 1.0f / (float)d;
  for (int l = 0; l < ctx->L; ++l) {
    LayerW& w = ctx->layers[l];
    const LnStats ln_in{l ? ctx->stat_ffn : nullptr, NB, inv_d, 1e-5f};
    const LnStats ln_ff{ctx->stat_att, NB, inv_d, 1e-5f};
    {
      GemmArgs<Op> ga{(const E*)ctx->X_op.p, d, (const E*)w.Win.p, d, M, 3 * d, d, 0};
      EpiQKV<Op, true> ep{w.c2_in, (E*)ctx->QK_op.p, (E*)ctx->Vt_op.p, d, ctx->H, ctx->hd, Sp, ctx->Skp, qscale, {w.Win.inv_scale, ctx->status}, ln_in};
      HIPCHK(ctx, launch_qkv<Op>(ga, ep, B, Sp, st, [&](const char* name, int cols) { mark(name, BS * 2.0 * dd * cols); }));
    }
    {
      AttnArgs<Op> aa{(const E*)ctx->QK_op.p, (const E*)ctx->Vt_op.p, (E*)ctx->A_op.p, S, Sp, ctx->Skp, d, ctx->H, 0};
      HIPCHK(ctx, launch_attn<Op>(aa, B, ctx->hd, st));
      mark("attention", 4.0 * B * (double)S * S * dd);
    }
    {
      GemmArgs<Op> ga{(const E*)ctx->A_op.p, d, (const E*)w.Wout.p, d, M, d, d, 0};
      EpiResid<Op> ep{w.bb_att, w.g_att, ctx->X, (E*)ctx->X_st, d, ctx->stat_att, ACT_NONE, {w.Wout.inv_scale, ctx->status}, ln_in};
      HIPCHK(ctx, launch_resid<Op>(ga, ep, B, Sp, st));
      mark("gemm_outproj", BS * 2.0 * dd * dd);
    }
    {
      GemmArgs<Op> ga{(const E*)ctx->X_op.p, d, (const E*)w.W1.p, d, M, ff, d, 0};
      EpiBiasAct<Op, true> ep{w.c2_ff, nullptr, 0, (E*)ctx->H_op.p, ff, ACT_GELU, {w.W1.inv_scale, ctx->status}, ln_ff};
      HIPCHK(ctx, launch_ffn1<Op>(ga, ep, B, Sp, st));
      mark("gemm_ffn1_gelu", BS * 2.0 * dd * ff);
    }
    {
      GemmArgs<Op> ga{(const E*)ctx->H_op.p, ff, (const E*)w.W2.p, ff, M, d, ff, 0};
      EpiResid<Op> ep{w.bb_ffn, w.g_ffn, ctx->X, (E*)ctx->X_st, d, ctx->stat_ffn, ACT_NONE, {w.W2.inv_scale, ctx->status}, ln_ff};
      HIPCHK(ctx, launch_resid<Op>(ga, ep, B, Sp, st));
      mark("gemm_ffn2", BS * 2.0 * dd * ff);
    }
  }
  {
    GemmArgs<Op> ga{(const E*)ctx->X_op.p, d, (const E*)ctx->Wf.p, d, M, ctx->XN, d, 0};
    EpiHead<Op> head = head_in;
    head.t_off = t_off;
    HIPCHK(ctx, launch_rows<Op>(ga, head, st));
    mark("gemm_head_ddpm", BT * 2.0 * dd * F);
  }
  ctx->step_kernels = nk;
  return 0;
}

template <class Op>
static EpiHead<Op> make_head(tamf_ctx* ctx, int mode) {
  EpiHead<Op> h{};
  h.bias = ctx->bf;
  h.mode = mode;
  h.F = ctx->F;
  h.T = ctx->T;
  h.Sp = ctx->Sp;
  h.P = ctx->P;
  h.XK = ctx->XK;
  h.xs = ctx->xs;
  h.xs_op = (typename Op::elem_t*)ctx->xs_st;
  h.tcur = ctx->tcur;
  h.c1 = ctx->c1;
  h.c2 = ctx->c2;
  h.sigma = ctx->sigma;
  h.n_steps = ctx->n_steps;
  h.lp = ctx->loop_params;
  h.ctl = EpiCtl{ctx->Wf.inv_scale, ctx->status};
  h.ln = LnStats{ctx->stat_ffn, ctx->d / 32, 1.0f / (float)ctx->d, 1e-5f};
  return h;
}

template <class Op>
static int denoise_impl(tamf_ctx* ctx, const float* x, const int64_t* t_dev, float* out, hipStream_t st) {
  typedef typename Op::elem_t E;
  const int B = ctx->B, T = ctx->T;
  hipLaunchKernelGGL((state_in_kernel<Op>), grid1d((long)B * T * (ctx->XK / 8)), dim3(256), 0, st, x, ctx->xs, (E*)ctx->xs_st,
                     B, ctx->F, T, ctx->XK, 0, 0ull, 0ll, ctx->status);
  hipLaunchKernelGGL(set_t_kernel, grid1d(B), dim3(256), 0, st, ctx->tcur, (const long long*)t_dev, 0, B, ctx->n_t > 0 ? ctx->n_t : 1);
  EpiHead<Op> h = make_head<Op>(ctx, HEAD_X0);
  h.x0_out = out;
  TRY(enqueue_step<Op>(ctx, st, h));
  HIPCHK(ctx, hipGetLastError());
  return 0;
}

extern "C" int tamf_denoise(tamf_ctx* ctx, const float* x_dev, const int64_t* t_dev, float* x0_out_dev, void* stream) {
  TAMF_LAUNCH_LOCK;
  TRY(need_kind(ctx, __func__, KIND_G));
  if (!x_dev || !t_dev || !x0_out_dev) return fail(ctx, TAMF_ERR_INVALID, "null argument");
  if (!ctx->cond_set) return fail(ctx, TAMF_ERR_STATE, "conditioning not set");
  HIPCHK(ctx, hipSetDevice(ctx->device));
  hipStream_t st = (hipStream_t)stream;
  TAMF_WITH_OP(ctx->prec, return denoise_impl<Op>(ctx, x_dev, t_dev, x0_out_dev, st));
  return 0;
}

template <class Op>
static int refine_impl(tamf_ctx* ctx, const float* x_in, const float* h2o, float* out, hipStream_t st) {
  typedef typename Op::elem_t E;
  const int B = ctx->B, T = ctx->T;
  hipLaunchKernelGGL((refine_in_kernel<Op>), grid1d((long)B * T * (ctx->XK / 8)), dim3(256), 0, st, x_in, h2o, (E*)ctx->xs_op.p,
                     B * T, ctx->F, ctx->arch.h2o_dim, ctx->XK, ctx->status);
  EpiHead<Op> h = make_head<Op>(ctx, HEAD_RESIDUAL);
  h.x0_out = out;
  h.x_in = x_in;
  TRY(enqueue_step<Op>(ctx, st, h));
  HIPCHK(ctx, hipGetLastError());
  return 0;
}

extern "C" int tamf_refine(tamf_ctx* ctx, const float* sample_pose_repr_dev, const float* h2o_dist_dev, float* out_dev,
                           void* stream) {
  TAMF_LAUNCH_LOCK;
  TRY(need_kind(ctx, __func__, KIND_R));
  if (!sample_pose_repr_dev || !h2o_dist_dev || !out_dev) return fail(ctx, TAMF_ERR_INVALID, "null argument");
  if (!ctx->cond_set) return fail(ctx, TAMF_ERR_STATE, "conditioning not set");
  HIPCHK(ctx, hipSetDevice(ctx->device));
  hipStream_t st = (hipStream_t)stream;
  TAMF_WITH_OP(ctx->prec, return refine_impl<Op>(ctx, sample_pose_repr_dev, h2o_dist_dev, out_dev, st));
  return 0;
}

extern "C" int tamf_ddpm_step(tamf_ctx* ctx, const float* x_t_dev, const float* x0_dev, int32_t t, const float* noise_dev,
                              float* x_out_dev, int64_t n, void* stream) {
  TRY(need_kind(ctx, __func__, KIND_G | KIND_R));
  if (!x_t_dev || !x0_dev || !x_out_dev || n <= 0) return fail(ctx, TAMF_ERR_INVALID, "null/invalid argument");
  if (ctx->n_steps <= 0) return fail(ctx, TAMF_ERR_STATE, "schedule not set");
  if (t < 0 || t >= ctx->n_steps) return fail(ctx, TAMF_ERR_INVALID, "t out of range");
  if (t != 0 && !noise_dev) return fail(ctx, TAMF_ERR_INVALID, "noise required for t != 0");
  HIPCHK(ctx, hipSetDevice(ctx->device));
  hipLaunchKernelGGL(ddpm_step_kernel, grid1d(n), dim3(256), 0, (hipStream_t)stream, x_t_dev, x0_dev, noise_dev, x_out_dev,
                     (long)n, ctx->h_c1[t], ctx->h_c2[t], ctx->h_sigma[t], t);
  HIPCHK(ctx, hipGetLastError());
  return 0;
}

template <class Op>
static int loop_impl(tamf_ctx* ctx, const float* noise, uint64_t seed, int64_t clip_base, float* out, float* dump,
                     int use_graph, hipStream_t st) {
  typedef typename Op::elem_t E;
  const int B = ctx->B, T = ctx->T, N = ctx->n_steps;
  hipLaunchKernelGGL((state_in_kernel<Op>), grid1d((long)B * T * (ctx->XK / 8)), dim3(256), 0, st, noise, ctx->xs,
                     (E*)ctx->xs_st, B, ctx->F, T, ctx->XK, noise ? 0 : 1, (unsigned long long)seed,
                     (long long)clip_base, ctx->status);
  hipLaunchKernelGGL(set_t_kernel, grid1d(B), dim3(256), 0, st, ctx->tcur, (const long long*)nullptr, N - 1, B, ctx->n_t > 0 ? ctx->n_t : 1);
  EpiHead<Op> h = make_head<Op>(ctx, HEAD_DDPM);
  struct InLoop {
    tamf_ctx* c;
    explicit InLoop(tamf_ctx* c_) : c(c_) { c->in_loop = true; }
    ~InLoop() { c->in_loop = false; }
  } in_loop_(ctx);
  hipLaunchKernelGGL(set_loop_params_kernel, dim3(1), dim3(64), 0, st, ctx->loop_params, noise, dump, (long)B * ctx->F * T,
                     (unsigned long long)seed, (long long)clip_base);
  if (!use_graph) {
    for (int i = 0; i < N; ++i) {
      TRY(enqueue_step<Op>(ctx, st, h));
      hipLaunchKernelGGL(advance_t_kernel, grid1d(B), dim3(256), 0, st, ctx->tcur, B, 1);
    }
  } else {
    int G = 1;
    for (int g = 2; g <= 16; ++g)
      if (N % g == 0) G = g;
    GraphKey key;
    key.B = B; key.T = T; key.n_steps = N; key.steps_per_graph = G;
    if (!(key == ctx->graph_key) || !ctx->graph_exec) {
      TRY(retire_graph(ctx));
      HIPCHK(ctx, hipStreamBeginCapture(ctx->cap_stream, hipStreamCaptureModeRelaxed));
      int rc = 0;
      for (int g = 0; g < G && rc == 0; ++g) rc = enqueue_step<Op>(ctx, ctx->cap_stream, h, g);
      hipLaunchKernelGGL(advance_t_kernel, grid1d(B), dim3(256), 0, ctx->cap_stream, ctx->tcur, B, G);
      hipError_t ee = hipStreamEndCapture(ctx->cap_stream, &ctx->graph);
      if (rc) return rc;
      HIPCHK(ctx, ee);
      HIPCHK(ctx, hipGraphInstantiate(&ctx->graph_exec, ctx->graph, nullptr, nullptr, 0));
      ctx->graph_key = key;
      ++ctx->graph_captures;
    }
    for (int i = 0; i < N / G; ++i) HIPCHK(ctx, hipGraphLaunch(ctx->graph_exec, st));
    ctx->graph_launches_last_loop = N / G;
    HIPCHK(ctx, hipEventRecord(ctx->graph_done, st));
    ctx->graph_in_flight = true;
  }
  hipLaunchKernelGGL(state_out_kernel, grid1d((long)B * ctx->F * T), dim3(256), 0, st, ctx->xs, out, B, ctx->F, T, ctx->XK);
  HIPCHK(ctx, hipGetLastError());
  return 0;
}

extern "C" int tamf_sample_loop(tamf_ctx* ctx, const float* noise_dev, uint64_t seed, int64_t clip_id_base, float* x0_out_dev,
                                float* dump_dev, int32_t use_graph, void* stream) {
  TAMF_LAUNCH_LOCK;
  TRY(need_kind(ctx, __func__, KIND_G));
  if (!x0_out_dev) return fail(ctx, TAMF_ERR_INVALID, "null argument");
  if (!ctx->cond_set) return fail(ctx, TAMF_ERR_STATE, "conditioning not set");
  if (ctx->n_steps <= 0) return fail(ctx, TAMF_ERR_STATE, "schedule not set");
  if (ctx->n_steps > ctx->n_t) return fail(ctx, TAMF_ERR_STATE, "schedule longer than the timestep table (max_timesteps)");
  HIPCHK(ctx, hipSetDevice(ctx->device));
  hipStream_t st = (hipStream_t)stream;
  TAMF_WITH_OP(ctx->prec, return loop_impl<Op>(ctx, noise_dev, seed, clip_id_base, x0_out_dev, dump_dev, use_graph, st));
  return 0;
}

extern "C" int tamf_get_status_flags(tamf_ctx* ctx, uint32_t* flags, int32_t clear, void* stream) {
  TRY(need_kind(ctx, __func__, KIND_G | KIND_R));
  if (!flags) return fail(ctx, TAMF_ERR_INVALID, "null argument");
  HIPCHK(ctx, hipSetDevice(ctx->device));
  HIPCHK(ctx, hipStreamSynchronize((hipStream_t)stream));
  unsigned v = 0;
  HIPCHK(ctx, hipMemcpy(&v, ctx->status, sizeof(v), hipMemcpyDeviceToHost));
  *flags = v | ctx->host_status;
  if (clear && v) HIPCHK(ctx, hipMemset(ctx->status, 0, sizeof(v)));
  return 0;
}

extern "C" int tamf_step_kernel_count(const tamf_ctx* ctx) { return ctx ? ctx->step_kernels : 0; }

extern "C" int tamf_loop_stats(const tamf_ctx* ctx, int32_t* graph_captures, int32_t* graph_launches_last_loop) {
  if (!ctx) return TAMF_ERR_INVALID;
  if (graph_captures) *graph_captures = ctx->graph_captures;
  if (graph_launches_last_loop) *graph_launches_last_loop = ctx->graph_launches_last_loop;
  return 0;
}

template <class Op>
static int profile_impl(tamf_ctx* ctx, hipStream_t st) {
  EpiHead<Op> h = make_head<Op>(ctx, HEAD_DDPM);
  hipLaunchKernelGGL(set_loop_params_kernel, dim3(1), dim3(64), 0, st, ctx->loop_params, (const float*)nullptr, (float*)nullptr,
                     (long)ctx->B * ctx->F * ctx->T, 1ull, 0ll);
  return enqueue_step<Op>(ctx, st, h);
}

template <class Body>
static int profile_run(tamf_ctx* ctx, int32_t max_n, float* ms_host, double* flops_host, char* names_host, hipStream_t st, Body body) {
  ctx->prof_ev.clear();
  ctx->prof_names.clear();
  ctx->prof_flops.clear();
  hipEvent_t ev0;
  HIPCHK(ctx, hipEventCreate(&ev0));
  hipEvent_t cal[6];
  for (hipEvent_t& e : cal) HIPCHK(ctx, hipEventCreate(&e));
  ctx->prof_on = true;
  for (hipEvent_t& e : cal) (void)hipEventRecord(e, st);
  (void)hipEventRecord(ev0, st);
  int rc = body();
  ctx->prof_on = false;
  hipError_t se = hipStreamSynchronize(st);
  int n = 0;
  if (rc == 0 && se == hipSuccess) {
    float gaps[5];
    for (int i = 0; i < 5; ++i) {
      gaps[i] = 0.f;
      (void)hipEventElapsedTime(&gaps[i], cal[i], cal[i + 1]);
    }
    std::sort(gaps, gaps + 5);
    const float ev_cost = gaps[2];
    hipEvent_t prev = ev0;
    for (size_t i = 0; i < ctx->prof_ev.size() && n < max_n; ++i, ++n) {
      float ms = 0.f;
      (void)hipEventElapsedTime(&ms, prev, ctx->prof_ev[i]);
      ms = ms > ev_cost ? ms - ev_cost : ms;
      ms_host[n] = ms;
      flops_host[n] = ctx->prof_flops[i];
      snprintf(names_host + (size_t)n * 48, 48, "%s", ctx->prof_names[i].c_str());
      prev = ctx->prof_ev[i];
    }
  }
  for (hipEvent_t e : ctx->prof_ev) (void)hipEventDestroy(e);
  for (hipEvent_t e : cal) (void)hipEventDestroy(e);
  (void)hipEventDestroy(ev0);
  ctx->prof_ev.clear();
  if (rc) return rc;
  HIPCHK(ctx, se);
  return n;
}

extern "C" int tamf_step_profile(tamf_ctx* ctx, int32_t max_n, float* ms_host, double* flops_host, char* names_host,
                                 void* stream) {
  TAMF_LAUNCH_LOCK;
  TRY(need_kind(ctx, __func__, KIND_G));
  if (!ms_host || !flops_host || !names_host || max_n <= 0) return fail(ctx, TAMF_ERR_INVALID, "null/invalid argument");
  if (!ctx->cond_set || ctx->n_steps <= 0) return fail(ctx, TAMF_ERR_STATE, "conditioning / schedule not set");
  HIPCHK(ctx, hipSetDevice(ctx->device));
  hipStream_t st = (hipStream_t)stream;
  hipLaunchKernelGGL(set_t_kernel, grid1d(ctx->B), dim3(256), 0, st, ctx->tcur, (const long long*)nullptr, ctx->n_steps / 2, ctx->B, ctx->n_t > 0 ? ctx->n_t : 1);
  return profile_run(ctx, max_n, ms_host, flops_host, names_host, st, [&]() {
    int rc = 0;
    TAMF_WITH_OP(ctx->prec, rc = profile_impl<Op>(ctx, st));
    return rc;
  });
}

extern "C" int tamf_refine_profile(tamf_ctx* ctx, const float* sample_pose_repr_dev, const float* h2o_dist_dev, float* out_dev,
                                   int32_t max_n, float* ms_host, double* flops_host, char* names_host, void* stream) {
  TAMF_LAUNCH_LOCK;
  TRY(need_kind(ctx, __func__, KIND_R));
  if (!sample_pose_repr_dev || !h2o_dist_dev || !out_dev || !ms_host || !flops_host || !names_host || max_n <= 0)
    return fail(ctx, TAMF_ERR_INVALID, "null/invalid argument");
  if (!ctx->cond_set) return fail(ctx, TAMF_ERR_STATE, "conditioning not set");
  HIPCHK(ctx, hipSetDevice(ctx->device));
  hipStream_t st = (hipStream_t)stream;
  return profile_run(ctx, max_n, ms_host, flops_host, names_host, st, [&]() {
    int rc = 0;
    TAMF_WITH_OP(ctx->prec, rc = refine_impl<Op>(ctx, sample_pose_repr_dev, h2o_dist_dev, out_dev, st));
    return rc;
  });
}

extern "C" int tamf_encode(tamf_ctx* ctx, int32_t B, int32_t T, int32_t nobj, const int32_t* obj_num_host, const float* pose_repr_dev,
                           const float* shape_dev, const uint8_t* hand_side_dev, const float* obj_emb_dev, const float* obj_traj_dev,
                           float* encoding_out_dev, float* activation_out_dev, void* stream) {
  TAMF_LAUNCH_LOCK;
  TRY(need_kind(ctx, __func__, KIND_E));
  if (!ctx->finalized) return fail(ctx, TAMF_ERR_STATE, "weights not finalised");
  if (B <= 0 || B > ctx->Bmax || T <= 0 || T > ctx->Tmax || nobj <= 0)
    return fail(ctx, TAMF_ERR_INVALID, "B/T/nobj out of range (B = " + std::to_string(B) + " of max_batch " + std::to_string(ctx->Bmax) +
                                           ", T = " + std::to_string(T) + " of max_frames " + std::to_string(ctx->Tmax) + ")");
  if (!pose_repr_dev || !shape_dev || !hand_side_dev || !obj_emb_dev || !obj_traj_dev || !encoding_out_dev)
    return fail(ctx, TAMF_ERR_INVALID, "null tensor");
  TRY(check_obj_num(ctx, obj_num_host, B, nobj));
  HIPCHK(ctx, hipSetDevice(ctx->device));
  hipStream_t st = (hipStream_t)stream;
  const int* cnt = nullptr;
  TRY(upload_obj_num(ctx, obj_num_host, B, st, &cnt));
  const int d = ctx->d, sd = ctx->arch.hand_shape_dim, od = ctx->arch.obj_embed_dim;
  PrefixArgs pa{};
  pa.side = hand_side_dev; pa.rh = ctx->rh; pa.lh = ctx->lh;
  pa.shape = shape_dev; pa.WshapeT = ctx->WshapeT; pa.bshape = ctx->bshape;
  pa.oemb = obj_emb_dev; pa.WobjT = ctx->WobjT; pa.bobj = ctx->bobj; pa.cnt = cnt;
  pa.pe = ctx->pe; pa.pstatic = ctx->pstatic;
  pa.B = B; pa.d = d; pa.T = T; pa.sd = sd; pa.nobj = nobj; pa.od = od; pa.clip_dim = 0; pa.nrows = ENC_P; pa.ht = 0;
  hipLaunchKernelGGL(prefix_rows_kernel, dim3(B, ENC_P), dim3(1024), (size_t)(std::max(od, sd) + 1024) * sizeof(float), st, pa);
  EncArgs ea{};
  ea.w = ctx->enc_w; ea.pe = ctx->pe; ea.pstatic = ctx->pstatic; ea.pose = pose_repr_dev; ea.traj = obj_traj_dev; ea.cnt = cnt;
  ea.enc = encoding_out_dev; ea.act = activation_out_dev;
  ea.T = T; ea.nobj = nobj; ea.F = ctx->F; ea.qd = ctx->arch.obj_input_dim; ea.kin = ctx->enc_kin; ea.ff = ctx->ff; ea.L = ctx->L;
  hipLaunchKernelGGL(encoder_kernel, dim3(B), dim3(ENC_NT), (size_t)enc_lds_bytes(T + ENC_P + 1, ctx->ff, ctx->enc_kin), st, ea);
  HIPCHK(ctx, hipGetLastError());
  return 0;
}

extern "C" int tamf_pose_decode(const float* pose_repr_dev, int64_t n_frames, int32_t n_joints, float* tsl_out_dev,
                                float* quat_out_dev, void* stream) {
  if (!pose_repr_dev || !quat_out_dev || n_frames <= 0 || n_joints <= 0) return fail(nullptr, TAMF_ERR_INVALID, "bad argument");
  hipLaunchKernelGGL(pose_decode_kernel, grid1d(n_frames * n_joints), dim3(256), 0, (hipStream_t)stream, pose_repr_dev,
                     tsl_out_dev, quat_out_dev, (long)n_frames, n_joints, 3 + 6 * n_joints);
  return launched();
}

static int h2o_launch(const float* hand_verts_dev, const float* obj_traj_dev, const float* obj_points_dev,
                      const int32_t* obj_num_dev, int32_t B, int32_t T, int32_t V, int32_t nobj, int32_t P, float* h2o_out_dev,
                      float* frame_min_dev, void* stream) {
  if (!hand_verts_dev || !obj_traj_dev || !obj_points_dev || (!h2o_out_dev && !frame_min_dev))
    return fail(nullptr, TAMF_ERR_INVALID, "null argument");
  if (B <= 0 || T <= 0 || V <= 0 || nobj <= 0 || P <= 0) return fail(nullptr, TAMF_ERR_INVALID, "bad shape");
  if (V > 256 * H2O_VPT) return fail(nullptr, TAMF_ERR_INVALID, "at most 1024 hand vertices per frame (MANO has 778)");
  if (B > 65535) return fail(nullptr, TAMF_ERR_INVALID, "batch too large for one launch");
  hipLaunchKernelGGL(h2o_dist_kernel, dim3(T, B), dim3(256), 0, (hipStream_t)stream, hand_verts_dev, obj_traj_dev,
                     obj_points_dev, (const int*)obj_num_dev, h2o_out_dev, frame_min_dev, T, V, nobj, P);
  return launched();
}

extern "C" int tamf_h2o_dist(const float* hand_verts_dev, const float* obj_traj_dev, const float* obj_points_dev,
                             const int32_t* obj_num_dev, int32_t B, int32_t T, int32_t V, int32_t nobj, int32_t P,
                             float* h2o_out_dev, void* stream) {
  if (!h2o_out_dev) return fail(nullptr, TAMF_ERR_INVALID, "null argument");
  return h2o_launch(hand_verts_dev, obj_traj_dev, obj_points_dev, obj_num_dev, B, T, V, nobj, P, h2o_out_dev, nullptr, stream);
}

extern "C" int tamf_contact_min_dist(const float* hand_verts_dev, const float* obj_traj_dev, const float* obj_points_dev,
                                     const int32_t* obj_num_dev, int32_t B, int32_t T, int32_t V, int32_t nobj, int32_t P,
                                     float* min_dist_out_dev, void* stream) {
  if (!min_dist_out_dev) return fail(nullptr, TAMF_ERR_INVALID, "null argument");
  return h2o_launch(hand_verts_dev, obj_traj_dev, obj_points_dev, obj_num_dev, B, T, V, nobj, P, nullptr, min_dist_out_dev, stream);
}

extern "C" int tamf_transform_points(const void* obj_traj_dev, const void* obj_points_dev, int32_t n_obj, int32_t T, int32_t P,
                                     int32_t is_f64, void* out_dev, void* stream) {
  if (!obj_traj_dev || !obj_points_dev || !out_dev) return fail(nullptr, TAMF_ERR_INVALID, "null argument");
  if (n_obj <= 0 || T <= 0 || P <= 0 || n_obj > 65535) return fail(nullptr, TAMF_ERR_INVALID, "bad shape");
  if (is_f64)
    hipLaunchKernelGGL((transform_points_kernel<double>), dim3(T, n_obj), dim3(256), 0, (hipStream_t)stream, (const double*)obj_traj_dev,
                       (const double*)obj_points_dev, (double*)out_dev, T, P);
  else
    hipLaunchKernelGGL((transform_points_kernel<float>), dim3(T, n_obj), dim3(256), 0, (hipStream_t)stream, (const float*)obj_traj_dev,
                       (const float*)obj_points_dev, (float*)out_dev, T, P);
  return launched();
}

extern "C" int tamf_vertex_normals(const float* verts_dev, int64_t n_mesh, int32_t V, const int32_t* csr_off_dev,
                                    const int32_t* csr_ent_dev, float* normals_out_dev, void* stream) {
  if (!verts_dev || !csr_off_dev || !csr_ent_dev || !normals_out_dev) return fail(nullptr, TAMF_ERR_INVALID, "null argument");
  if (n_mesh <= 0 || V <= 0) return fail(nullptr, TAMF_ERR_INVALID, "bad shape");
  hipLaunchKernelGGL(vertex_normals_kernel, grid1d((long)n_mesh * V), dim3(256), 0, (hipStream_t)stream, verts_dev, csr_off_dev,
                     csr_ent_dev, normals_out_dev, (long)n_mesh, V);
  return launched();
}

extern "C" int tamf_mesh_contains(const double* verts_dev, const int32_t* faces_dev, int32_t n_faces, const double* points_dev,
                                  int64_t n_points, const double* scale3, const double* translate3, int32_t resolution,
                                  double* tri_workspace_dev, uint8_t* contains_out_dev, void* stream) {
  if (!verts_dev || !faces_dev || !points_dev || !scale3 || !translate3 || !tri_workspace_dev || !contains_out_dev)
    return fail(nullptr, TAMF_ERR_INVALID, "null argument");
  if (n_faces <= 0 || n_points <= 0 || resolution <= 1) return fail(nullptr, TAMF_ERR_INVALID, "bad shape");
  hipStream_t st = (hipStream_t)stream;
  hipLaunchKernelGGL(mesh_prepare_kernel, grid1d(n_faces), dim3(256), 0, st, verts_dev, (const int*)faces_dev, n_faces, scale3[0],
                     scale3[1], scale3[2], translate3[0], translate3[1], translate3[2], tri_workspace_dev);
  hipLaunchKernelGGL(mesh_contains_kernel, grid1d(n_points), dim3(256), 0, st, tri_workspace_dev, n_faces, points_dev,
                     (long)n_points, scale3[0], scale3[1], scale3[2], translate3[0], translate3[1], translate3[2],
                     (double)resolution, contains_out_dev);
  return launched();
}

extern "C" int tamf_power_spectrum_sum(const float* joints_dev, const int32_t* len_host, int32_t N, int32_t T, int32_t F,
                                       int32_t accumulate, double* psd_sum_dev, double* psd_clip_dev, void* stream) {
  if (N < 1 || F < 1) return fail(nullptr, TAMF_ERR_INVALID, "bad shape (N = " + std::to_string(N) + ", F = " + std::to_string(F) + ")");
  if (T < 3) return fail(nullptr, TAMF_ERR_INVALID, "T = " + std::to_string(T) + ": the second difference needs at least 3 frames");
  if (T > PS_MAX_T)
    return fail(nullptr, TAMF_ERR_INVALID, "T = " + std::to_string(T) + " above the " + std::to_string(PS_MAX_T) +
                                               " frames whose accelerations and twiddle table fit the LDS");
  if (!joints_dev || !psd_sum_dev) return fail(nullptr, TAMF_ERR_INVALID, "null argument");
  if (len_host)
    for (int n = 0; n < N; ++n)
      if (len_host[n] < 1 || len_host[n] > T)
        return fail(nullptr, TAMF_ERR_INVALID, "len[" + std::to_string(n) + "] = " + std::to_string(len_host[n]) + " outside [1, T]");
  const int L = T - 2, K = L / 2 + 1;
  const size_t lds = ps_lds_bytes(L);
  const hipError_t e = lds_once<power_spectrum_kernel>((int)ps_lds_bytes(PS_MAX_T - 2));
  if (e != hipSuccess) return fail(nullptr, TAMF_ERR_HIP, std::string("power spectrum kernel attribute setup failed: ") + hipGetErrorString(e));
  const dim3 grid((F + PS_FT - 1) / PS_FT, (K + PS_KT - 1) / PS_KT);
  PsLens lens;
  memset(&lens, 0, sizeof(lens));
  for (int n0 = 0; n0 < N; n0 += PS_LENS) {
    const int n = std::min(PS_LENS, N - n0);
    if (len_host)
      for (int i = 0; i < n; ++i) lens.v[i] = (uint16_t)len_host[n0 + i];
    hipLaunchKernelGGL(power_spectrum_kernel, grid, dim3(PS_NT), lds, (hipStream_t)stream, joints_dev + (size_t)n0 * T * F, lens,
                       len_host ? 1 : 0, n, T, F, (accumulate || n0 > 0) ? 1 : 0, psd_sum_dev,
                       psd_clip_dev ? psd_clip_dev + (size_t)n0 * L * F : nullptr);
  }
  return launched();
}

#ifdef TAMF_TEST_HOOKS
#include "tamf_hip_hooks.h"
#endif
```

### oakink2-tamf_amd/csrc/tamf_hip_hooks.h

```cpp
#pragma once
#include "../../include/tamf_hip_test.h"

extern "C" int tamf_test_set_guard_bytes(int64_t bytes) {
  if (bytes < 0 || bytes > (1 << 20) || bytes % 256) return fail(nullptr, TAMF_ERR_INVALID, "guard bytes must be a multiple of 256 in [0, 1 MiB]");
  g_guard_bytes.store((size_t)bytes);
  return 0;
}

extern "C" int tamf_test_fail_alloc_after(int32_t n) {
  g_fail_alloc_in.store(n);
  return 0;
}
extern "C" int tamf_test_poke(tamf_ctx* ctx, int32_t alloc_index, int64_t offset, int32_t nbytes) {
  if (!ctx || alloc_index < 0 || (size_t)alloc_index >= ctx->guards.size() || nbytes <= 0) return fail(ctx, TAMF_ERR_INVALID, "bad argument");
  const GuardRec& g = ctx->guards[alloc_index];
  if (offset < -(int64_t)g.guard || offset + nbytes > (int64_t)(g.bytes + g.guard)) return fail(ctx, TAMF_ERR_INVALID, "outside the allocation and its margins");
  HIPCHK(ctx, hipSetDevice(ctx->device));
  HIPCHK(ctx, hipMemset(g.base + g.guard + offset, 0, nbytes));
  return 0;
}

extern "C" int tamf_test_check_guards(tamf_ctx* ctx, int32_t* n_checked) {
  if (!ctx) return fail(ctx, TAMF_ERR_INVALID, "null ctx");
  HIPCHK(ctx, hipSetDevice(ctx->device));
  HIPCHK(ctx, hipDeviceSynchronize());
  if (n_checked) *n_checked = (int32_t)ctx->guards.size();
  std::vector<unsigned char> host;
  int bad = 0;
  std::string report;
  for (size_t i = 0; i < ctx->guards.size(); ++i) {
    const GuardRec& g = ctx->guards[i];
    host.resize(g.guard);
    for (int side = 0; side < 2; ++side) {
      const char* src = side ? g.base + g.guard + g.bytes : g.base;
      HIPCHK(ctx, hipMemcpy(host.data(), src, g.guard, hipMemcpyDeviceToHost));
      size_t first = g.guard, last = 0, n = 0;
      for (size_t k = 0; k < g.guard; ++k)
        if (host[k] != GUARD_BYTE) {
          if (first == g.guard) first = k;
          last = k;
          ++n;
        }
      if (n) {
        ++bad;
        if (report.size() < 1500)
          report += std::string(report.empty() ? "" : "; ") + "allocation #" + std::to_string(i) + " [" + g.tag + "] of " +
                    std::to_string(g.bytes) + " bytes: " + std::to_string(n) + " bytes written " +
                    (side ? "BEYOND its end (offsets +" + std::to_string(first) + " .. +" + std::to_string(last) + ")"
                          : "BELOW its start (offsets -" + std::to_string(g.guard - first) + " .. -" + std::to_string(g.guard - last) + ")");
      }
    }
  }
  if (bad) return fail(ctx, TAMF_ERR_STATE, "out-of-bounds device stores: " + report);
  return 0;
}

extern "C" int tamf_test_fill_scratch(tamf_ctx* ctx, int32_t byte) {
  TAMF_LAUNCH_LOCK;
  TRY(need_kind(ctx, __func__, KIND_G | KIND_R));
  if (byte < 0 || byte > 255) return fail(ctx, TAMF_ERR_INVALID, "byte must be in [0, 255]");
  HIPCHK(ctx, hipSetDevice(ctx->device));
  HIPCHK(ctx, hipDeviceSynchronize());
  const size_t eb = (size_t)ctx->EB, M = (size_t)ctx->Mmax, d = (size_t)ctx->d, BT = (size_t)ctx->Bmax * ctx->Tmax;
  HIPCHK(ctx, hipMemset(ctx->H_op.p, byte, M * ctx->ff * eb));
  HIPCHK(ctx, hipMemset(ctx->QK_op.p, byte, M * 2 * d * eb));
  HIPCHK(ctx, hipMemset(ctx->A_op.p, byte, M * d * eb));
  HIPCHK(ctx, hipMemset(ctx->h1_op.p, byte, BT * d * eb));
  HIPCHK(ctx, hipDeviceSynchronize());
  return 0;
}

struct TmpBufs {
  std::vector<void*> v;
  ~TmpBufs() {
    for (void* p : v) (void)hipFree(p);
  }
  void* get(size_t bytes) {
    void* p = nullptr;
    if (hipMalloc(&p, bytes ? bytes : 16) != hipSuccess) return nullptr;
    v.push_back(p);
    return p;
  }
};

template <class Op>
static int test_gemm_impl(int M, int N, int K, const float* a, const float* w, const float* bias, int act, float* c,
                          const float* gamma, const float2* stats_in, float2* stats_out, bool resid, hipStream_t st) {
  typedef typename Op::elem_t E;
  if (prepare_all<Op>() != hipSuccess) return fail(nullptr, TAMF_ERR_HIP, "prepare failed");
  const int Kp = round_up(K, 64);
  TmpBufs tb;
  E* ao = (E*)tb.get((size_t)M * Kp * Op::EB);
  E* wo = (E*)tb.get((size_t)N * Kp * Op::EB);
  E* yo = (E*)tb.get((size_t)M * N * Op::EB);
  if (!ao || !wo || !yo) return fail(nullptr, TAMF_ERR_NOMEM, "hipMalloc failed");
  hipLaunchKernelGGL((pack_operand_kernel<Op>), grid1d((long)M * (Kp / 8)), dim3(256), 0, st, a, ao, (long)M, K, Kp);
  hipLaunchKernelGGL((pack_operand_kernel<Op>), grid1d((long)N * (Kp / 8)), dim3(256), 0, st, w, wo, (long)N, K, Kp);
  GemmArgs<Op> ga{ao, Kp, wo, Kp, M, N, Kp, 0};
  hipError_t e;
  if (resid) {
    EpiResid<Op> ep{bias, gamma, c, Op::PREC == 0 ? nullptr : yo, N, stats_out, ACT_NONE, {}, LnStats{stats_in, N / 32, 1.0f / (float)N, 1e-5f}};
    const int sp = clip_rows_of_m(M);
    e = sp ? launch_resid<Op>(ga, ep, M / sp, sp, st) : launch_rows<Op>(ga, ep, st);
  } else {
    EpiStoreF32 ep{bias, c, N, act};
    const int nc = M / 208;
    bool done = false;
    if (M % 208 == 0 && N % 256 == 0 && ClipLaunch<Op, 4, EpiStoreF32>::applies(nc, 208, N, Kp)) {
      e = ClipLaunch<Op, 4, EpiStoreF32>::launch(nullptr, ao, Kp, wo, Kp, nc, 208, N, Kp, ep, st);
      done = true;
    } else {
      const int sp = clip_rows_of_m(M);
      if (sp) {
        TAMF_CLIP_NSUB(sp, {
          if (ClipLaunch<Op, 2, EpiStoreF32, NSP, 2>::applies_parts(M / sp, sp, N, Kp)) {
            e = ClipLaunch<Op, 2, EpiStoreF32, NSP, 2>::launch(nullptr, ao, Kp, wo, Kp, M / sp, sp, N, Kp, ep, st);
            done = true;
          } else if (ClipLaunch<Op, 2, EpiStoreF32, NS>::applies(M / sp, sp, N, Kp)) {
            e = ClipLaunch<Op, 2, EpiStoreF32, NS>::launch(nullptr, ao, Kp, wo, Kp, M / sp, sp, N, Kp, ep, st);
            done = true;
          }
        })
      }
    }
    if (!done) e = gemm128<Op>(ga, ep, st);
  }
  if (e != hipSuccess) return fail(nullptr, TAMF_ERR_HIP, std::string("gemm launch: ") + hipGetErrorString(e));
  if (hipStreamSynchronize(st) != hipSuccess) return fail(nullptr, TAMF_ERR_HIP, "sync failed");
  e = hipGetLastError();
  if (e != hipSuccess) return fail(nullptr, TAMF_ERR_HIP, std::string("gemm run: ") + hipGetErrorString(e));
  return 0;
}

extern "C" int tamf_test_gemm(int32_t precision, int32_t M, int32_t N, int32_t K, const float* a_dev, const float* w_dev,
                              const float* bias_dev, int32_t act, float* c_dev, void* stream) {
  TAMF_LAUNCH_LOCK;
  if (M <= 0 || N <= 0 || K <= 0 || N % 128) return fail(nullptr, TAMF_ERR_INVALID, "N must be a multiple of 128");
  hipStream_t st = (hipStream_t)stream;
  if (precision < 0 || precision > TAMF_PREC_F16X3) return fail(nullptr, TAMF_ERR_INVALID, "unknown precision");
  TAMF_WITH_OP(precision, return test_gemm_impl<Op>(M, N, K, a_dev, w_dev, bias_dev, act, c_dev, nullptr, nullptr, nullptr, false, st));
  return 0;
}

extern "C" int tamf_test_gemm_resid(int32_t precision, int32_t M, int32_t N, int32_t K, const float* a_dev, const float* w_dev,
                                    const float* bb_dev, const float* gamma_dev, const float* stats_in_dev, float* x_dev,
                                    float* stats_out_dev, void* stream) {
  TAMF_LAUNCH_LOCK;
  if (M <= 0 || K <= 0 || !(N == 128 || N == 256 || N == 512)) return fail(nullptr, TAMF_ERR_INVALID, "N must be 128/256/512");
  if (!a_dev || !w_dev || !bb_dev || !gamma_dev || !x_dev || !stats_out_dev) return fail(nullptr, TAMF_ERR_INVALID, "null argument");
  hipStream_t st = (hipStream_t)stream;
  if (precision < 0 || precision > TAMF_PREC_F16X3) return fail(nullptr, TAMF_ERR_INVALID, "unknown precision");
  TAMF_WITH_OP(precision, return test_gemm_impl<Op>(M, N, K, a_dev, w_dev, bb_dev, 0, x_dev, gamma_dev, (const float2*)stats_in_dev,
                                                    (float2*)stats_out_dev, true, st));
  return 0;
}

template <class Op>
static int test_attn_impl(int B, int S, int H, int hd, const float* qkv, float* out, hipStream_t st) {
  typedef typename Op::elem_t E;
  const int d = H * hd, Sp = round_up(S, 8), Skp = round_up(S, 32);
  const long M = (long)B * Sp;
  TmpBufs tb;
  const size_t qk_n = (size_t)M * 2 * d, vt_n = (size_t)B * d * Skp, o_n = (size_t)M * d;
  E* qk = (E*)tb.get(qk_n * Op::EB);
  E* vt = (E*)tb.get(vt_n * Op::EB);
  E* oo = (E*)tb.get(o_n * Op::EB);
  float* of = (float*)tb.get(o_n * 4);
  if (!qk || !vt || !oo || !of) return fail(nullptr, TAMF_ERR_NOMEM, "hipMalloc failed");
  (void)hipMemsetAsync(vt, 0, vt_n * Op::EB, st);
  const float qscale = 1.4426950408889634f / sqrtf((float)hd);
  hipLaunchKernelGGL((qkv_pack_kernel<Op>), grid1d(M * 3 * d), dim3(256), 0, st, qkv, qk, vt, B, S, Sp, Skp, H, hd, qscale);
  AttnArgs<Op> aa{qk, vt, oo, S, Sp, Skp, d, H, 0};
  hipError_t e = launch_attn<Op>(aa, B, hd, st);
  if (e != hipSuccess) return fail(nullptr, TAMF_ERR_HIP, std::string("attn launch: ") + hipGetErrorString(e));
  hipLaunchKernelGGL((unpack_operand_kernel<Op>), grid1d(M * d), dim3(256), 0, st, oo, of, M, d, d);
  for (int b = 0; b < B; ++b)
    (void)hipMemcpyAsync(out + (size_t)b * S * d, of + (size_t)b * Sp * d, (size_t)S * d * 4, hipMemcpyDeviceToDevice, st);
  if (hipStreamSynchronize(st) != hipSuccess) return fail(nullptr, TAMF_ERR_HIP, "sync failed");
  e = hipGetLastError();
  if (e != hipSuccess) return fail(nullptr, TAMF_ERR_HIP, std::string("attn run: ") + hipGetErrorString(e));
  return 0;
}

extern "C" int tamf_test_attention(int32_t precision, int32_t B, int32_t S, int32_t H, int32_t hd, const float* qkv_dev,
                                   float* out_dev, void* stream) {
  TAMF_LAUNCH_LOCK;
  if (B <= 0 || S <= 0 || H <= 0 || !(hd == 64 || hd == 128)) return fail(nullptr, TAMF_ERR_INVALID, "bad attention shape");
  hipStream_t st = (hipStream_t)stream;
  if (precision < 0 || precision > TAMF_PREC_F16X3) return fail(nullptr, TAMF_ERR_INVALID, "unknown precision");
  TAMF_WITH_OP(precision, return test_attn_impl<Op>(B, S, H, hd, qkv_dev, out_dev, st));
  return 0;
}

template <class Op>
__global__ void fill_operand_kernel(typename Op::elem_t* out, long n, unsigned salt) {
  const long i = ((long)blockIdx.x * blockDim.x + threadIdx.x) * 8;
  if (i >= n) return;
  float v[8];
#pragma unroll
  for (int j = 0; j < 8; ++j) {
    unsigned h = (unsigned)(i + j) * 2654435761u + salt;
    h ^= h >> 15; h *= 2246822519u; h ^= h >> 13;
    v[j] = (float)(h >> 8) * (2.0f / 16777216.0f) - 1.0f;
  }
  Op::template store<8>(out, i, v);
}

template <class Op>
static int bench_gemm_impl(int epi_kind, int M, int N, int K, int iters, float* ms_out, hipStream_t st) {
  typedef typename Op::elem_t E;
  if (prepare_all<Op>() != hipSuccess) return fail(nullptr, TAMF_ERR_HIP, "prepare failed");
  TmpBufs tb;
  const long an = (long)M * K, wn = (long)N * K, on = (long)M * N;
  E* a = (E*)tb.get((size_t)an * Op::EB);
  E* w = (E*)tb.get((size_t)wn * Op::EB);
  E* o = (E*)tb.get((size_t)on * Op::EB);
  E* o2 = (E*)tb.get((size_t)on * Op::EB);
  float* x = (float*)tb.get((size_t)on * 4);
  float* vec = (float*)tb.get((size_t)N * 4 * 4);
  if (!a || !w || !o || !o2 || !x || !vec) return fail(nullptr, TAMF_ERR_NOMEM, "hipMalloc failed");
  hipLaunchKernelGGL((fill_operand_kernel<Op>), grid1d(an / 8), dim3(256), 0, st, a, an, 1u);
  hipLaunchKernelGGL((fill_operand_kernel<Op>), grid1d(wn / 8), dim3(256), 0, st, w, wn, 2u);
  hipLaunchKernelGGL((fill_operand_kernel<OpF32>), grid1d(on / 8), dim3(256), 0, st, x, on, 3u);
  hipLaunchKernelGGL((fill_operand_kernel<OpF32>), grid1d(N * 4 / 8), dim3(256), 0, st, vec, (long)N * 4, 4u);
  GemmArgs<Op> ga{a, K, w, K, M, N, K, 0};
  hipEvent_t e0, e1;
  if (hipEventCreate(&e0) != hipSuccess || hipEventCreate(&e1) != hipSuccess) return fail(nullptr, TAMF_ERR_HIP, "event");
  hipError_t e = hipSuccess;
  for (int it = -2; it < iters && e == hipSuccess; ++it) {
    if (it == 0) (void)hipEventRecord(e0, st);
    if (epi_kind == 2) {
      e = hipErrorInvalidValue;
    } else if (epi_kind == 3) {
      EpiStoreF32 ep{vec, x, N, ACT_NONE};
      if (M % 208 == 0 && ClipLaunch<Op, 2, EpiStoreF32>::applies(M / 208, 208, N, K))
        e = ClipLaunch<Op, 2, EpiStoreF32>::launch(nullptr, a, K, w, K, M / 208, 208, N, K, ep, st);
      else
        e = gemm128<Op>(ga, ep, st);
    } else if (epi_kind == 1) {
      const int d = N / 3;
      EpiQKV<Op> ep{vec, o, o2, d, d / 128, 128, 208, 224, 0.1f};
      e = gemm128<Op>(ga, ep, st);
    } else if (epi_kind >= 10 && epi_kind <= 12) {
      {
        const LnStats ln{(const float2*)x, K / 32, 1.0f / (float)K, 1e-5f};
        if (epi_kind == 10) {
          EpiBiasAct<Op, true> ep{vec, nullptr, 0, o, N, ACT_GELU, {}, ln};
          e = clip_rows_of_m(M) == 208 ? launch_ffn1<Op>(ga, ep, M / 208, 208, st) : gemm128<Op>(ga, ep, st);
        } else if (epi_kind == 11) {
          const int d = N / 3;
          EpiQKV<Op, true> ep{vec, o, o2, d, d / 128, 128, 208, 224, 0.1f, {}, ln};
          e = gemm128<Op>(ga, ep, st);
        } else {
          EpiResid<Op> ep{vec, vec + N, x, o, N, (float2*)o2, ACT_NONE, {}, LnStats{nullptr, N / 32, 1.0f / (float)N, 1e-5f}};
          e = clip_rows_of_m(M) == 208 ? launch_resid<Op>(ga, ep, M / 208, 208, st) : gemm128<Op>(ga, ep, st);
        }
      }
    } else {
      EpiBiasAct<Op> ep{vec, nullptr, 0, o, N, ACT_GELU};
      if (M % 208 == 0 && ClipLaunch<Op, 4, EpiBiasAct<Op>>::applies(M / 208, 208, N, K)) {
        e = ClipLaunch<Op, 4, EpiBiasAct<Op>>::launch(nullptr, a, K, w, K, M / 208, 208, N, K, ep, st);
      } else {
        if (g_krot >= 0 && (g_krot & 0x20000)) ep.ldo = 0;
        if (g_krot >= 0 && (g_krot & 0x8000)) ep.act = ACT_NONE;
        e = gemm128<Op>(ga, ep, st);
      }
    }
  }
  (void)hipEventRecord(e1, st);
  hipError_t se = hipStreamSynchronize(st);
  float ms = 0.f;
  (void)hipEventElapsedTime(&ms, e0, e1);
  (void)hipEventDestroy(e0);
  (void)hipEventDestroy(e1);
  if (e != hipSuccess || se != hipSuccess)
    return fail(nullptr, TAMF_ERR_HIP, std::string("bench gemm: ") + hipGetErrorString(e != hipSuccess ? e : se));
  *ms_out = ms / iters;
  return 0;
}

template <class Op>
static int bench_attn_impl(int B, int S, int H, int hd, int iters, int abl, float* ms_out, hipStream_t st) {
  typedef typename Op::elem_t E;
  if (prepare_all<Op>() != hipSuccess) return fail(nullptr, TAMF_ERR_HIP, "prepare failed");
  const int d = H * hd, Sp = round_up(S, 8), Skp = round_up(S, 32);
  const long M = (long)B * Sp, qk_n = M * 2 * d, vt_n = (long)B * d * Skp, o_n = M * d;
  TmpBufs tb;
  E* qk = (E*)tb.get((size_t)qk_n * Op::EB);
  E* vt = (E*)tb.get((size_t)vt_n * Op::EB);
  E* oo = (E*)tb.get((size_t)o_n * Op::EB);
  if (!qk || !vt || !oo) return fail(nullptr, TAMF_ERR_NOMEM, "hipMalloc failed");
  hipLaunchKernelGGL((fill_operand_kernel<Op>), grid1d(qk_n / 8), dim3(256), 0, st, qk, qk_n, 5u);
  hipLaunchKernelGGL((fill_operand_kernel<Op>), grid1d(vt_n / 8), dim3(256), 0, st, vt, vt_n, 6u);
  AttnArgs<Op> aa{qk, vt, oo, S, Sp, Skp, d, H, abl};
  hipEvent_t e0, e1;
  if (hipEventCreate(&e0) != hipSuccess || hipEventCreate(&e1) != hipSuccess) return fail(nullptr, TAMF_ERR_HIP, "event");
  hipError_t e = hipSuccess;
  for (int it = -2; it < iters && e == hipSuccess; ++it) {
    if (it == 0) (void)hipEventRecord(e0, st);
    e = launch_attn<Op>(aa, B, hd, st);
  }
  (void)hipEventRecord(e1, st);
  hipError_t se = hipStreamSynchronize(st);
  float ms = 0.f;
  (void)hipEventElapsedTime(&ms, e0, e1);
  (void)hipEventDestroy(e0);
  (void)hipEventDestroy(e1);
  if (e != hipSuccess || se != hipSuccess)
    return fail(nullptr, TAMF_ERR_HIP, std::string("bench attention: ") + hipGetErrorString(e != hipSuccess ? e : se));
  *ms_out = ms / iters;
  return 0;
}

extern "C" int tamf_bench_attention(int32_t precision, int32_t B, int32_t S, int32_t H, int32_t hd, int32_t iters, int32_t abl,
                                    int32_t tuning, float* ms_out, void* stream) {
  TAMF_LAUNCH_LOCK;
  if (B <= 0 || S <= 0 || H <= 0 || !(hd == 64 || hd == 128) || iters <= 0 || !ms_out) return fail(nullptr, TAMF_ERR_INVALID, "bad argument");
  if (precision < 0 || precision > TAMF_PREC_F16X3) return fail(nullptr, TAMF_ERR_INVALID, "unknown precision");
  const int saved_rot = g_krot, saved_sel = g_sel;
  tamf_set_gemm_tuning(tuning);
  int rc = 0;
  TAMF_WITH_OP(precision, rc = bench_attn_impl<Op>(B, S, H, hd, iters, abl, ms_out, (hipStream_t)stream));
  g_krot = saved_rot;
  g_sel = saved_sel;
  return rc;
}

extern "C" int tamf_bench_mfma_rate(int32_t precision, int32_t millis, float* tflops_out, float* mhz_out, void* stream) {
  if (precision < 0 || precision > TAMF_PREC_F16X3 || millis <= 0 || millis > 20000 || !tflops_out) return fail(nullptr, TAMF_ERR_INVALID, "bad argument");
  hipStream_t st = (hipStream_t)stream;
  float* sink = nullptr;
  int cus = 0, dev = 0;
  if (hipGetDevice(&dev) != hipSuccess || hipDeviceGetAttribute(&cus, hipDeviceAttributeMultiprocessorCount, dev) != hipSuccess || cus <= 0)
    return fail(nullptr, TAMF_ERR_HIP, "no device");
  const int grid = 2 * cus, block = 512, iters = 4000;
  if (hipMalloc(&sink, (size_t)grid * block * sizeof(float)) != hipSuccess) return fail(nullptr, TAMF_ERR_HIP, "hipMalloc failed");
  hipEvent_t e0 = nullptr, e1 = nullptr;
  hipEventCreate(&e0);
  hipEventCreate(&e1);
  auto launch = [&]() {
    if (precision == TAMF_PREC_F32) hipLaunchKernelGGL(mfma_rate_kernel<0>, dim3(grid), dim3(block), 0, st, sink, iters);
    else if (precision == TAMF_PREC_F16X3) hipLaunchKernelGGL(mfma_rate_kernel<2>, dim3(grid), dim3(block), 0, st, sink, iters);
    else hipLaunchKernelGGL(mfma_rate_kernel<1>, dim3(grid), dim3(block), 0, st, sink, iters);
  };
  float ms1 = 0.f, ms = 0.f;
  launch();
  hipEventRecord(e0, st);
  launch();
  hipEventRecord(e1, st);
  hipEventSynchronize(e1);
  hipEventElapsedTime(&ms1, e0, e1);
  const int n_all = (int)(millis / (ms1 > 1e-3f ? ms1 : 1e-3f)) + 3, n_settle = n_all / 3, n = n_all - n_settle;
  for (int i = 0; i < n_settle; ++i) launch();
  hipEventRecord(e0, st);
  for (int i = 0; i < n; ++i) launch();
  hipEventRecord(e1, st);
  hipError_t e = hipEventSynchronize(e1);
  hipEventElapsedTime(&ms, e0, e1);
  hipEventDestroy(e0);
  hipEventDestroy(e1);
  hipFree(sink);
  if (e != hipSuccess || !(ms > 0.f)) return fail(nullptr, TAMF_ERR_HIP, e != hipSuccess ? hipGetErrorString(e) : "no time measured");
  const double mfmas = (double)n * grid * (block / 64) * (double)iters * 8;
  const double flop_per_mfma = precision == TAMF_PREC_F32 ? 2.0 * 16 * 16 * 4 : 2.0 * 16 * 16 * 32;
  *tflops_out = (float)(mfmas * flop_per_mfma / (ms * 1e-3) / 1e12);
  if (mhz_out) *mhz_out = (float)(mfmas / (cus * 4.0) * (precision == TAMF_PREC_F32 ? 32.0 : 16.0) / (ms * 1e-3) / 1e6);
  return 0;
}

extern "C" int tamf_bench_gemm(int32_t precision, int32_t epi_kind, int32_t krot, int32_t M, int32_t N, int32_t K,
                               int32_t iters, float* ms_out, void* stream) {
  TAMF_LAUNCH_LOCK;
  if (M <= 0 || N <= 0 || K <= 0 || iters <= 0 || !ms_out) return fail(nullptr, TAMF_ERR_INVALID, "bad argument");
  if (epi_kind == 1 && (N % 384 || M % 208)) return fail(nullptr, TAMF_ERR_INVALID, "qkv bench needs N = 3d, M multiple of 208");
  const int saved_rot = g_krot, saved_sel = g_sel;
  tamf_set_gemm_tuning(krot);
  hipStream_t st = (hipStream_t)stream;
  int rc = 0;
  if (precision < 0 || precision > TAMF_PREC_F16X3) rc = fail(nullptr, TAMF_ERR_INVALID, "unknown precision");
  else TAMF_WITH_OP(precision, rc = bench_gemm_impl<Op>(epi_kind, M, N, K, iters, ms_out, st));
  g_krot = saved_rot;
  g_sel = saved_sel;
  return rc;
}

extern "C" int tamf_set_gemm_tuning(int32_t krot) {
  TAMF_LAUNCH_LOCK;
  int sel = krot >= 0 ? (krot >> 20) & 0x7FF : 0;
  const int low = krot & 0xFFFFF;
  int rot = -1;
  if (krot >= 0 && low == 0x7FFFF) sel |= 2048;
  else if (krot >= 0 && low != 0xFFFFF) rot = low;
  if (sel != g_sel || rot != g_krot) {
    std::lock_guard<std::mutex> lk(g_live_mu);
    for (tamf_ctx* c : g_live_ctx) (void)retire_graph(c);
  }
  g_sel = sel;
  g_krot = rot;
  return 0;
}

extern "C" int tamf_test_philox(uint64_t seed, int64_t clip_id_base, int32_t draw, int32_t B, int32_t n_feat, int32_t T,
                                float* out_dev, void* stream) {
  if (B <= 0 || n_feat <= 0 || T <= 0 || !out_dev) return fail(nullptr, TAMF_ERR_INVALID, "bad argument");
  hipLaunchKernelGGL(philox_fill_kernel, grid1d((long)B * n_feat * T), dim3(256), 0, (hipStream_t)stream, out_dev,
                     (unsigned long long)seed, (long long)clip_id_base, (unsigned)draw, B, n_feat, T);
  hipError_t e = hipGetLastError();
  if (e != hipSuccess) return fail(nullptr, TAMF_ERR_HIP, hipGetErrorString(e));
  return 0;
}

#ifdef TAMF_TIMELINE
extern "C" int tamf_debug_timeline(int which, void* dst, size_t bytes) {
  if (which == 0) return (int)hipMemcpyFromSymbol(dst, HIP_SYMBOL(g_gemm_ts), bytes, 0, hipMemcpyDeviceToHost);
  if (which == 2) return (int)hipMemcpyFromSymbol(dst, HIP_SYMBOL(g_clip_ts), bytes, 0, hipMemcpyDeviceToHost);
  return (int)hipMemcpyFromSymbol(dst, HIP_SYMBOL(g_attn_ts), bytes, 0, hipMemcpyDeviceToHost);
}
#endif
```

### oakink2-tamf_amd/csrc/tamf_shapes.h

```cpp
#pragma once

static inline int round_up(int v, int m) { return (v + m - 1) / m * m; }

static inline int clip_tile_rows(int Sp) { return (Sp > 176 && Sp <= 208) ? 208 : (Sp > 144 && Sp <= 176) ? 176 : 0; }
static constexpr int CLIP_TILE_ROWS_MAX = 208;
static inline int clip_rows_of_m(int M) { return M % 208 == 0 ? 208 : (M % 168 == 0 ? 168 : 0); }

static inline double round_util(int tiles, int slots) { return (double)tiles / (double)(((tiles + slots - 1) / slots) * slots); }

static inline int vt_row_keys(int S, int Sp) {
  const int tile = clip_tile_rows(Sp);
  return ((S > tile ? S : tile) + 31) / 32 * 32;
}

static constexpr int PREFIX_ROWS_G = 5, PREFIX_ROWS_R = 3;
struct SeqShape {
  int S, Sp, Skp;
};
static inline SeqShape seq_shape(int T, int P) {
  SeqShape s{};
  s.S = T + P;
  s.Sp = round_up(s.S, 8);
  s.Skp = vt_row_keys(s.S, s.Sp);
  return s;
}
static inline SeqShape seq_shape_max(int Tmax, int P) {
  SeqShape s = seq_shape(Tmax, P);
  s.Skp = round_up(s.S > CLIP_TILE_ROWS_MAX ? s.S : CLIP_TILE_ROWS_MAX, 32);
  return s;
}
static inline bool dims_fit_32bit_offsets(int max_batch, int max_frames, int ff_size, int latent_dim) {
  const long long mmax = (long long)max_batch * seq_shape(max_frames, PREFIX_ROWS_G).Sp;
  const long long widest = ff_size > 3LL * latent_dim ? ff_size : 3LL * latent_dim;
  return mmax * widest * 4 < (1LL << 32) && (long long)max_batch * max_frames * 896 * 4 < (1LL << 32);
}

struct ScratchLayout {
  bool alias;
  unsigned long long host_bytes;
  unsigned long long qk_off, a_off, h1_off;
  unsigned long long qk_bytes, a_bytes, h1_bytes, hidden_bytes;
};
static inline ScratchLayout scratch_layout(long long Mmax, long long BT, int d, int ff, int elem_bytes, unsigned long long guard) {
  auto up = [](unsigned long long v) { return (v + 255ull) / 256ull * 256ull; };
  ScratchLayout s{};
  s.hidden_bytes = up((unsigned long long)Mmax * ff * elem_bytes);
  s.qk_bytes = up((unsigned long long)Mmax * 2 * d * elem_bytes);
  s.a_bytes = up((unsigned long long)Mmax * d * elem_bytes);
  s.h1_bytes = up((unsigned long long)BT * d * elem_bytes);
  s.host_bytes = s.hidden_bytes;
  s.alias = s.qk_bytes + s.a_bytes <= s.hidden_bytes && s.h1_bytes <= s.qk_bytes;
  if (!s.alias) return s;
  if (guard == 0) {
    s.qk_off = 0;
    s.a_off = s.qk_bytes;
    s.h1_off = 0;
  } else {
    s.qk_off = s.hidden_bytes + guard;
    s.a_off = s.qk_off + s.qk_bytes + guard;
    s.h1_off = s.a_off + s.a_bytes + guard;
    s.host_bytes = s.h1_off + s.h1_bytes;
  }
  return s;
}
```

### oakink2-tamf_amd/oakink2_tamf_amd/_lib.py

```python
from __future__ import annotations

import ctypes
import os
import shutil
import subprocess
import threading
from dataclasses import dataclass
from typing import NamedTuple

_HERE = os.path.dirname(os.path.abspath(__file__))
CSRC = os.path.normpath(os.path.join(_HERE, "..", "csrc"))
INCLUDE = os.path.normpath(os.path.join(_HERE, "..", "..", "include"))
LIB_DIR = os.path.join(_HERE, "lib")
LIB_PATH = os.path.join(LIB_DIR, "libtamf_hip.so")
HOOKS_PATH = os.path.join(LIB_DIR, "libtamf_hip_hooks.so")
EVAL_LIB_PATH = os.path.join(LIB_DIR, "libtamf_eval.so")
MANO_LIB_PATH = os.path.join(LIB_DIR, "libtamf_mano.so")
POINTENC_LIB_PATH = os.path.join(LIB_DIR, "libtamf_pointenc.so")
TEXTENC_LIB_PATH = os.path.join(LIB_DIR, "libtamf_textenc.so")
ENCTRAIN_LIB_PATH = os.path.join(LIB_DIR, "libtamf_enctrain.so")
CONTACT_LIB_PATH = os.path.join(LIB_DIR, "libtamf_contact.so")
REFINETRAIN_LIB_PATH = os.path.join(LIB_DIR, "libtamf_refinetrain.so")
MDMTRAIN_LIB_PATH = os.path.join(LIB_DIR, "libtamf_mdmtrain.so")
OPTIM_LIB_PATH = os.path.join(LIB_DIR, "libtamf_optim.so")
RENDER_LIB_PATH = os.path.join(LIB_DIR, "libtamf_render.so")
SURFACE_LIB_PATH = os.path.join(LIB_DIR, "libtamf_surface.so")
MESHDIST_LIB_PATH = os.path.join(LIB_DIR, "libtamf_meshdist.so")
SDFGRID_LIB_PATH = os.path.join(LIB_DIR, "libtamf_sdfgrid.so")
WINDING_LIB_PATH = os.path.join(LIB_DIR, "libtamf_winding.so")

EXPORTS = [
    "tamf_ctx_create", "tamf_ctx_resize", "tamf_ctx_destroy", "tamf_last_error", "tamf_load_weight", "tamf_finalize_weights",
    "tamf_set_schedule", "tamf_set_timestep_map", "tamf_set_cond", "tamf_set_cond_ragged", "tamf_denoise", "tamf_ddpm_step", "tamf_sample_loop", "tamf_refine",
    "tamf_encode",
    "tamf_pose_decode", "tamf_h2o_dist", "tamf_contact_min_dist", "tamf_mesh_contains", "tamf_transform_points", "tamf_vertex_normals",
    "tamf_power_spectrum_sum",
    "tamf_get_status_flags", "tamf_step_kernel_count", "tamf_loop_stats", "tamf_step_profile", "tamf_refine_profile",
]
HOOK_EXPORTS = [
    "tamf_test_gemm", "tamf_test_gemm_resid", "tamf_test_attention", "tamf_test_philox", "tamf_test_set_guard_bytes", "tamf_test_check_guards",
    "tamf_test_poke", "tamf_test_fail_alloc_after", "tamf_test_fill_scratch", "tamf_bench_gemm", "tamf_bench_attention", "tamf_bench_mfma_rate", "tamf_set_gemm_tuning",
]
EVAL_EXPORTS = [
    "tamf_eval_last_error", "tamf_voxelize_lattice", "tamf_mesh_contains_count_workspace", "tamf_mesh_contains_count",
]
MANO_EXPORTS = [
    "tamf_mano_last_error", "tamf_mano_model_create", "tamf_mano_model_destroy", "tamf_mano_model_set_tiles", "tamf_mano_forward",
    "tamf_mano_backward",
]
POINTENC_EXPORTS = [
    "tamf_pointenc_last_error", "tamf_pointenc_model_create", "tamf_pointenc_load_weight", "tamf_pointenc_finalize", "tamf_pointenc_destroy",
    "tamf_pointenc_fold_bn", "tamf_pointenc_fps", "tamf_pointenc_group", "tamf_pointenc_workspace_bytes", "tamf_pointenc_encode",
]
TEXTENC_EXPORTS = [
    "tamf_textenc_last_error", "tamf_textenc_model_create", "tamf_textenc_load_weight", "tamf_textenc_finalize", "tamf_textenc_destroy",
    "tamf_textenc_workspace_bytes", "tamf_textenc_encode",
]
ENCTRAIN_EXPORTS = [
    "tamf_enctrain_last_error", "tamf_enctrain_create", "tamf_enctrain_destroy", "tamf_enctrain_bind", "tamf_enctrain_step",
    "tamf_enctrain_dropout_mask",
]
CONTACT_EXPORTS = [
    "tamf_contact_last_error", "tamf_contact_forward", "tamf_contact_backward",
]
REFINETRAIN_EXPORTS = [
    "tamf_refinetrain_last_error", "tamf_refinetrain_create", "tamf_refinetrain_destroy", "tamf_refinetrain_bind", "tamf_refinetrain_forward",
    "tamf_refinetrain_backward", "tamf_refinetrain_dropout_mask", "tamf_refinetrain_set_profile", "tamf_refinetrain_get_profile",
]
MDMTRAIN_EXPORTS = [
    "tamf_mdmtrain_last_error", "tamf_mdmtrain_create", "tamf_mdmtrain_destroy", "tamf_mdmtrain_bind", "tamf_mdmtrain_forward",
    "tamf_mdmtrain_backward", "tamf_mdmtrain_dropout_mask", "tamf_mdmtrain_set_profile", "tamf_mdmtrain_get_profile",
]
OPTIM_EXPORTS = [
    "tamf_optim_last_error", "tamf_optim_create", "tamf_optim_destroy", "tamf_optim_bind", "tamf_optim_grad_norms", "tamf_optim_step",
]
RENDER_EXPORTS = [
    "tamf_render_last_error", "tamf_render_project", "tamf_render_clear", "tamf_render_raster", "tamf_render_points", "tamf_render_shade_mesh",
    "tamf_render_shade_points", "tamf_render_fill", "tamf_render_raster_behind", "tamf_render_points_behind", "tamf_render_shade_mesh_colors",
    "tamf_render_shade_points_colors", "tamf_render_composite", "tamf_render_resolve",
]
SURFACE_EXPORTS = [
    "tamf_surface_last_error", "tamf_surface_workspace_bytes", "tamf_surface_sample",
]
MESHDIST_EXPORTS = [
    "tamf_meshdist_last_error", "tamf_meshdist_workspace", "tamf_meshdist_prepare", "tamf_meshdist_points_workspace", "tamf_meshdist_points",
    "tamf_meshdist_lattice",
]
SDFGRID_EXPORTS = [
    "tamf_sdfgrid_last_error", "tamf_sdfgrid_forward", "tamf_sdfgrid_backward",
]
WINDING_EXPORTS = [
    "tamf_winding_last_error", "tamf_winding_workspace", "tamf_winding_prepare", "tamf_winding_points_workspace", "tamf_winding_points",
    "tamf_winding_lattice",
]


class TamfBuildError(RuntimeError):
    pass


def _include_closure(root: str):
    import re

    seen, todo = [], [root]
    while todo:
        name = todo.pop()
        path = os.path.join(CSRC, name)
        if name in seen or not os.path.exists(path):
            continue
        seen.append(name)
        with open(path) as f:
            todo += [m for m in re.findall(r'^\s*#\s*include\s+"([^"/]+)"', f.read(), flags=re.M)]
    return sorted(seen)


def _compile(hipcc: str, workdir: str, extra, name: str, source: str):
    os.makedirs(workdir, exist_ok=True)
    out = os.path.join(workdir, name)
    cmd = [hipcc, "-O3", "--offload-arch=gfx950", "-std=c++17", "-shared", "-fPIC", "-Wno-unused-value", "-Wno-unused-function", "-save-temps=obj",
           "-o", out, os.path.join(CSRC, source)] + list(extra)
    res = subprocess.run(cmd, capture_output=True, text=True, cwd=workdir)
    if res.returncode != 0:
        raise TamfBuildError("hipcc failed:\n" + res.stdout + res.stderr)
    asm = [f for f in os.listdir(workdir) if f.endswith("gfx950.s")]
    return out, (os.path.join(workdir, asm[0]) if asm else None)


def _check_counted_waits(asms, verbose: bool) -> None:
    import warnings

    from . import _isa_check

    n = nd = 0
    for a in asms:
        if a is None:
            raise _isa_check.IsaMismatch("hipcc left no device assembly to check")
        n = _isa_check.check(a)
        nd = _isa_check.check_deep(a)
    if verbose:
        print(f"ISA check: all {n} clip_gemm_kernel and {nd} gemm_deep_kernel instantiations match the counted waits (both builds)")
    try:
        _isa_check.check_scratch(asms[0])
    except _isa_check.IsaMismatch as e:
        warnings.warn(f"libtamf_hip: {e}")


class Output(NamedTuple):
    file: str
    flags: tuple
    exports: list


@dataclass(frozen=True)
class Library:
    name: str
    root: str
    headers: tuple
    outputs: tuple
    kernels: tuple = ()
    counted_waits: bool = False

    @property
    def sources(self):
        return _include_closure(self.root)

    @property
    def paths(self):
        return [os.path.join(LIB_DIR, o.file) for o in self.outputs]

    @property
    def stamp_path(self) -> str:
        return self.paths[0] + ".src.sha256"

    def digest(self) -> str:
        import hashlib

        h = hashlib.sha256()
        for tag, path in [("csrc/" + s, os.path.join(CSRC, s)) for s in self.sources] + [("include/" + h_, os.path.join(INCLUDE, h_)) for h_ in self.headers]:
            if os.path.exists(path):
                h.update(tag.encode())
                with open(path, "rb") as f:
                    h.update(f.read())
        return h.hexdigest()

    def stale(self) -> bool:
        if not all(os.path.exists(p) for p in self.paths):
            return True
        try:
            with open(self.stamp_path) as f:
                return f.read().strip() != self.digest()
        except OSError:
            return True

    def _compile_all(self, hipcc: str, wd: str, extra=()):
        from concurrent.futures import ThreadPoolExecutor

        with ThreadPoolExecutor(max_workers=2) as ex:
            return list(ex.map(lambda o: _compile(hipcc, os.path.join(wd, o.file), o.flags + tuple(extra), o.file, self.root), self.outputs))

    def _report_kernels(self, asm, verbose: bool) -> None:
        from . import _isa_check

        if asm is None:
            raise TamfBuildError(f"hipcc left no device assembly of {self.outputs[0].file} to check")
        rep = _isa_check.scratch_report(asm, prefixes=self.kernels)
        if len(rep) < len(self.kernels):
            raise TamfBuildError(f"{self.outputs[0].file}: kernel descriptors missing from the device assembly (found {[r[0] for r in rep]})")
        for name, scratch, vgprs in rep:
            if verbose:
                print(f"{self.name}: {name}: {vgprs} vgprs, {scratch} B scratch")
            if scratch > _isa_check.SCRATCH_LIMIT:
                import warnings

                warnings.warn(f"{self.name}: {name} keeps {scratch} bytes of scratch per lane ({vgprs} vgprs)")

    def build(self, force: bool = False, verbose: bool = False) -> str:
        if not force and not self.stale():
            return self.paths[0]
        hipcc = shutil.which("hipcc") or "/opt/rocm/bin/hipcc"
        if not os.path.exists(hipcc):
            raise TamfBuildError(f"hipcc not found: cannot build {self.outputs[0].file}")
        os.makedirs(LIB_DIR, exist_ok=True)
        import fcntl
        import tempfile

        from . import _isa_check

        with open(self.paths[0] + ".lock", "w") as lock:
            fcntl.flock(lock, fcntl.LOCK_EX)
            if not force and not self.stale():
                return self.paths[0]
            with tempfile.TemporaryDirectory(prefix="tamf_build_", dir=LIB_DIR) as wd:
                built = self._compile_all(hipcc, wd)
                safe = False
                if self.counted_waits:
                    try:
                        _check_counted_waits([asm for _, asm in built], verbose)
                    except (_isa_check.IsaMismatch, IndexError, KeyError, ValueError) as e:
                        import warnings

                        warnings.warn(f"{self.name}: {e}\nrebuilding with -DTAMF_CLIP_SAFE_WAIT (counted waits -> vmcnt(0))")
                        for o in self.outputs:
                            shutil.rmtree(os.path.join(wd, o.file), ignore_errors=True)
                        built = self._compile_all(hipcc, wd, ["-DTAMF_CLIP_SAFE_WAIT"])
                        safe = True
                if self.kernels:
                    self._report_kernels(built[0][1], verbose)
                digest = self.digest()
                for (out, _), path in reversed(list(zip(built, self.paths))):
                    os.replace(out, path)
                with open(self.stamp_path + ".tmp", "w") as f:
                    f.write(digest + "\n")
                os.replace(self.stamp_path + ".tmp", self.stamp_path)
        if verbose:
            print("built", " and ".join(self.paths[:1] + [o.file for o in self.outputs[1:]]) + (" (safe waits)" if safe else ""))
        return self.paths[0]


SAMPLER = Library("libtamf_hip", "tamf_hip.hip", ("tamf_hip.h", "tamf_hip_test.h"),
                  (Output("libtamf_hip.so", (), EXPORTS), Output("libtamf_hip_hooks.so", ("-DTAMF_TEST_HOOKS",), EXPORTS + HOOK_EXPORTS)),
                  counted_waits=True)
EVAL = Library("libtamf_eval", "tamf_eval.hip", ("tamf_eval.h", "tamf_hip.h"),
               (Output("libtamf_eval.so", (), EVAL_EXPORTS),),
               kernels=("_Z23voxelize_lattice_kernel", "_Z26mesh_contains_count_kernel"))
MANO = Library("libtamf_mano", "tamf_mano.hip", ("tamf_mano.h", "tamf_hip.h"),
               (Output("libtamf_mano.so", (), MANO_EXPORTS),),
               kernels=("_Z19mano_forward_kernelILi1EE", "_Z19mano_forward_kernelILi2EE", "_Z19mano_forward_kernelILi4EE"))
POINTENC = Library("libtamf_pointenc", "tamf_pointenc.hip", ("tamf_pointenc.h", "tamf_hip.h"),
                   (Output("libtamf_pointenc.so", (), POINTENC_EXPORTS),),
                   kernels=("_Z10fps_kernelILi8ELb1EE", "_Z10fps_kernelILi16ELb1EE", "_Z10fps_kernelILi32ELb0EE", "_Z12group_kernel", "_Z15f32_gemm_kernelI5PeEpiE", "_Z11attn_kernel"))
TEXTENC = Library("libtamf_textenc", "tamf_textenc.hip", ("tamf_textenc.h", "tamf_hip.h"),
                  (Output("libtamf_textenc.so", (), TEXTENC_EXPORTS),),
                  kernels=("_Z12embed_kernel", "_Z9ln_kernel", "_Z15f32_gemm_kernelI5TeEpiE", "_Z11attn_kernel"))
ENCTRAIN = Library("libtamf_enctrain", "tamf_enctrain.hip", ("tamf_enctrain.h", "tamf_hip.h"),
                   (Output("libtamf_enctrain.so", (), ENCTRAIN_EXPORTS),),
                   kernels=("_Z10lin_kernel", "_Z12wgrad_kernel", "_Z15attn_fwd_kernel", "_Z17attn_bwd_q_kernel", "_Z18attn_bwd_kv_kernel"))
CONTACT = Library("libtamf_contact", "tamf_contact.hip", ("tamf_contact.h", "tamf_hip.h"),
                  (Output("libtamf_contact.so", (), CONTACT_EXPORTS),),
                  kernels=("_Z18contact_h2o_kernel", "_Z18contact_o2h_kernel", "_Z23contact_backward_kernel"))
REFINETRAIN = Library("libtamf_refinetrain", "tamf_refinetrain.hip", ("tamf_refinetrain.h", "tamf_hip.h"),
                      (Output("libtamf_refinetrain.so", (), REFINETRAIN_EXPORTS),),
                      kernels=("_Z13tg_lin_kernelILb0EE", "_Z13tg_lin_kernelILb1EE", "_Z15tg_wgrad_kernel", "_Z18tg_attn_fwd_kernel", "_Z20tg_attn_bwd_q_kernel",
                               "_Z21tg_attn_bwd_kv_kernel"))
MDMTRAIN = Library("libtamf_mdmtrain", "tamf_mdmtrain.hip", ("tamf_mdmtrain.h", "tamf_hip.h"),
                   (Output("libtamf_mdmtrain.so", (), MDMTRAIN_EXPORTS),),
                   kernels=("_Z13tg_lin_kernelILb0EE", "_Z13tg_lin_kernelILb1EE", "_Z15tg_wgrad_kernel", "_Z18tg_attn_fwd_kernelILi64EE",
                            "_Z18tg_attn_fwd_kernelILi128EE", "_Z20tg_attn_bwd_q_kernelILi64EE", "_Z20tg_attn_bwd_q_kernelILi128EE",
                            "_Z21tg_attn_bwd_kv_kernelILi64EE", "_Z21tg_attn_bwd_kv_kernelILi128EE"))
OPTIM = Library("libtamf_optim", "tamf_optim.hip", ("tamf_optim.h", "tamf_hip.h"),
                (Output("libtamf_optim.so", (), OPTIM_EXPORTS),),
                kernels=("_Z18optim_sumsq_kernel", "_Z19optim_update_kernel", "_Z17optim_norm_kernel"))
RENDER = Library("libtamf_render", "tamf_render.hip", ("tamf_render.h", "tamf_hip.h"),
                 (Output("libtamf_render.so", (), RENDER_EXPORTS),),
                 kernels=("_Z21render_project_kernel", "_Z20render_raster_kernelILb0EE", "_Z20render_raster_kernelILb1EE", "_Z20render_points_kernelILb0EE",
                          "_Z20render_points_kernelILb1EE", "_Z24render_shade_mesh_kernelILb0EE", "_Z24render_shade_mesh_kernelILb1EE",
                          "_Z23render_composite_kernel", "_Z21render_resolve_kernel"))
SURFACE = Library("libtamf_surface", "tamf_surface.hip", ("tamf_surface.h", "tamf_hip.h"),
                  (Output("libtamf_surface.so", ("-ffp-contract=off",), SURFACE_EXPORTS),),
                  kernels=("_Z24surface_area_scan_kernel", "_Z20surface_carry_kernel", "_Z24surface_add_carry_kernel", "_Z21surface_sample_kernel"))
MESHDIST = Library("libtamf_meshdist", "tamf_meshdist.hip", ("tamf_meshdist.h", "tamf_hip.h"),
                   (Output("libtamf_meshdist.so", ("-ffp-contract=off",), MESHDIST_EXPORTS),),
                   kernels=("_Z24md_inside_prepare_kernel", "_Z22meshdist_points_kernel", "_Z23meshdist_lattice_kernel"))
SDFGRID = Library("libtamf_sdfgrid", "tamf_sdfgrid.hip", ("tamf_sdfgrid.h", "tamf_hip.h"),
                  (Output("libtamf_sdfgrid.so", ("-ffp-contract=off",), SDFGRID_EXPORTS),),
                  kernels=("_Z22sdfgrid_forward_kernel", "_Z23sdfgrid_backward_kernel"))
WINDING = Library("libtamf_winding", "tamf_winding.hip", ("tamf_winding.h", "tamf_hip.h"),
                  (Output("libtamf_winding.so", ("-ffp-contract=off",), WINDING_EXPORTS),),
                  kernels=("_Z21winding_points_kernelILb0EE", "_Z21winding_points_kernelILb1EE", "_Z21winding_reduce_kernel", "_Z22winding_lattice_kernel"))
LIBRARIES = (SAMPLER, EVAL, MANO)
PREPROCESSING = (POINTENC,)
TEXT_PREPROCESSING = (TEXTENC,)
TRAINING = (ENCTRAIN, CONTACT)
REFINE_TRAINING = (REFINETRAIN,)
DENOISER_TRAINING = (MDMTRAIN,)
OPTIMISER = (OPTIM,)
RENDERING = (RENDER,)
OBJECT_PREPROCESSING = (SURFACE,)
OBJECT_DISTANCE = (MESHDIST,)
PENETRATION_LOSS = (SDFGRID,)
OBJECT_SIGN = (WINDING,)


def build(force: bool = False, verbose: bool = False) -> str:
    for lib in LIBRARIES + PREPROCESSING + TEXT_PREPROCESSING + TRAINING + REFINE_TRAINING + DENOISER_TRAINING + OPTIMISER + RENDERING + OBJECT_PREPROCESSING + OBJECT_DISTANCE + PENETRATION_LOSS + OBJECT_SIGN:
        lib.build(force, verbose)
    return LIB_PATH


def build_mano(force: bool = False, verbose: bool = False) -> str:
    return MANO.build(force, verbose)


_lock = threading.Lock()
_loaded = {}


def _load(lib: Library, file: str) -> ctypes.CDLL:
    with _lock:
        if file not in _loaded:
            lib.build()
            import torch

            _loaded[file] = ctypes.CDLL(os.path.join(LIB_DIR, file))
        return _loaded[file]


def load() -> ctypes.CDLL:
    return _load(SAMPLER, "libtamf_hip.so")


def load_hooks() -> ctypes.CDLL:
    return _load(SAMPLER, "libtamf_hip_hooks.so")


def load_eval() -> ctypes.CDLL:
    return _load(EVAL, "libtamf_eval.so")


def load_mano_lib() -> ctypes.CDLL:
    return _load(MANO, "libtamf_mano.so")


def load_pointenc() -> ctypes.CDLL:
    return _load(POINTENC, "libtamf_pointenc.so")


def load_textenc() -> ctypes.CDLL:
    return _load(TEXTENC, "libtamf_textenc.so")


def load_enctrain() -> ctypes.CDLL:
    return _load(ENCTRAIN, "libtamf_enctrain.so")


def load_contact() -> ctypes.CDLL:
    return _load(CONTACT, "libtamf_contact.so")


def load_refinetrain() -> ctypes.CDLL:
    return _load(REFINETRAIN, "libtamf_refinetrain.so")


def load_mdmtrain() -> ctypes.CDLL:
    return _load(MDMTRAIN, "libtamf_mdmtrain.so")


def load_optim() -> ctypes.CDLL:
    return _load(OPTIM, "libtamf_optim.so")


def load_render() -> ctypes.CDLL:
    return _load(RENDER, "libtamf_render.so")


def load_surface() -> ctypes.CDLL:
    return _load(SURFACE, "libtamf_surface.so")


def load_meshdist() -> ctypes.CDLL:
    return _load(MESHDIST, "libtamf_meshdist.so")


def load_sdfgrid() -> ctypes.CDLL:
    return _load(SDFGRID, "libtamf_sdfgrid.so")


def load_winding() -> ctypes.CDLL:
    return _load(WINDING, "libtamf_winding.so")


def load_from(path: str) -> ctypes.CDLL:
    with _lock:
        if any(o.file in _loaded for o in SAMPLER.outputs):
            raise RuntimeError("libtamf_hip is already loaded in this process")
        import torch

        lib = ctypes.CDLL(path)
        for o in SAMPLER.outputs:
            _loaded[o.file] = lib
        return lib
```

### oakink2-tamf_amd/oakink2_tamf_amd/hip_backend.py

```python
from __future__ import annotations

import ctypes
from ctypes import POINTER, c_char_p, c_double, c_float, c_int32, c_int64, c_uint8, c_uint64, c_void_p
from typing import Dict, Mapping, Optional, Sequence, Tuple

import numpy as np
import torch

from . import _lib

PRECISIONS = {"f32": 0, "bf16": 1, "bf16x3": 2, "f16x3": 3}
KINDS = {"G": 0, "R": 1, "E": 2}


class TamfError(RuntimeError):
    pass


class TamfRangeError(TamfError):
    """A non-finite weight (at load) or an activation beyond +-65504 (status flag) does not fit the split-fp16 operand format of "f16x3"."""


STATUS_F16_RANGE = 1
STATUS_F16_WEIGHT_RANGE = 2
DEFAULT_PRECISION = "f16x3"


class _Arch(ctypes.Structure):
    _fields_ = [
        ("input_dim", c_int32),
        ("obj_input_dim", c_int32),
        ("hand_shape_dim", c_int32),
        ("obj_embed_dim", c_int32),
        ("latent_dim", c_int32),
        ("ff_size", c_int32),
        ("num_layers", c_int32),
        ("num_heads", c_int32),
        ("clip_dim", c_int32),
        ("h2o_dim", c_int32),
        ("kind", c_int32),
    ]


_bound = set()
_use_hooks = False


def _bind(L: ctypes.CDLL) -> ctypes.CDLL:
    if id(L) in _bound:
        return L
    L.tamf_last_error.restype = c_char_p
    L.tamf_last_error.argtypes = [c_void_p]
    L.tamf_ctx_create.argtypes = [POINTER(_Arch), c_int32, c_int32, c_int32, c_int32, POINTER(c_void_p)]
    L.tamf_ctx_destroy.argtypes = [c_void_p]
    L.tamf_ctx_destroy.restype = None
    L.tamf_load_weight.argtypes = [c_void_p, c_char_p, c_void_p, POINTER(c_int64), c_int32]
    L.tamf_finalize_weights.argtypes = [c_void_p, c_int32, c_void_p]
    L.tamf_set_schedule.argtypes = [c_void_p, c_int32, c_void_p, c_void_p, c_void_p]
    if hasattr(L, "tamf_set_timestep_map"):
        L.tamf_set_timestep_map.argtypes = [c_void_p, c_int32, c_void_p]
    L.tamf_set_cond.argtypes = [c_void_p, c_int32, c_int32, c_int32, c_void_p, c_void_p, c_void_p, c_void_p, c_void_p, c_void_p]
    if hasattr(L, "tamf_set_cond_ragged"):
        L.tamf_ctx_resize.argtypes = [c_void_p, c_int32, c_int32]
        L.tamf_set_cond_ragged.argtypes = [c_void_p, c_int32, c_int32, c_int32, c_void_p, c_void_p, c_void_p, c_void_p, c_void_p, c_void_p, c_void_p]
    L.tamf_denoise.argtypes = [c_void_p, c_void_p, c_void_p, c_void_p, c_void_p]
    L.tamf_ddpm_step.argtypes = [c_void_p, c_void_p, c_void_p, c_int32, c_void_p, c_void_p, c_int64, c_void_p]
    L.tamf_sample_loop.argtypes = [c_void_p, c_void_p, c_uint64, c_int64, c_void_p, c_void_p, c_int32, c_void_p]
    L.tamf_refine.argtypes = [c_void_p, c_void_p, c_void_p, c_void_p, c_void_p]
    if hasattr(L, "tamf_encode"):
        L.tamf_encode.argtypes = [c_void_p, c_int32, c_int32, c_int32, c_void_p] + [c_void_p] * 8
    if hasattr(L, "tamf_get_status_flags"):
        L.tamf_get_status_flags.argtypes = [c_void_p, POINTER(ctypes.c_uint32), c_int32, c_void_p]
    L.tamf_step_kernel_count.argtypes = [c_void_p]
    L.tamf_loop_stats.argtypes = [c_void_p, POINTER(c_int32), POINTER(c_int32)]
    L.tamf_step_profile.argtypes = [c_void_p, c_int32, c_void_p, c_void_p, c_void_p, c_void_p]
    if hasattr(L, "tamf_refine_profile"):
        L.tamf_refine_profile.argtypes = [c_void_p, c_void_p, c_void_p, c_void_p, c_int32, c_void_p, c_void_p, c_void_p, c_void_p]
    if hasattr(L, "tamf_test_gemm"):
        L.tamf_test_gemm.argtypes = [c_int32, c_int32, c_int32, c_int32, c_void_p, c_void_p, c_void_p, c_int32, c_void_p, c_void_p]
        L.tamf_test_attention.argtypes = [c_int32, c_int32, c_int32, c_int32, c_int32, c_void_p, c_void_p, c_void_p]
        L.tamf_test_philox.argtypes = [c_uint64, c_int64, c_int32, c_int32, c_int32, c_int32, c_void_p, c_void_p]
        L.tamf_set_gemm_tuning.argtypes = [c_int32]
    if hasattr(L, "tamf_test_gemm_resid"):
        L.tamf_test_gemm_resid.argtypes = [c_int32, c_int32, c_int32, c_int32] + [c_void_p] * 8
    if hasattr(L, "tamf_test_set_guard_bytes"):
        L.tamf_test_set_guard_bytes.argtypes = [c_int64]
        L.tamf_test_check_guards.argtypes = [c_void_p, POINTER(c_int32)]
        L.tamf_test_poke.argtypes = [c_void_p, c_int32, c_int64, c_int32]
    if hasattr(L, "tamf_test_fail_alloc_after"):
        L.tamf_test_fail_alloc_after.argtypes = [c_int32]
    if hasattr(L, "tamf_test_fill_scratch"):
        L.tamf_test_fill_scratch.argtypes = [c_void_p, c_int32]
    if hasattr(L, "tamf_bench_mfma_rate"):
        L.tamf_bench_mfma_rate.argtypes = [c_int32, c_int32, POINTER(ctypes.c_float), POINTER(ctypes.c_float), c_void_p]
    _bound.add(id(L))
    return L


def hooks() -> ctypes.CDLL:
    return _bind(_lib.load_hooks())


def use_test_hooks(on: bool = True) -> None:
    global _use_hooks
    _use_hooks = bool(on)


def lib() -> ctypes.CDLL:
    return hooks() if _use_hooks else _bind(_lib.load())


def set_guard_bytes(n: int) -> None:
    _check(hooks().tamf_test_set_guard_bytes(int(n)), None, hooks())


def hand_side_code(hs) -> int:
    if isinstance(hs, bytes):
        hs = hs.decode()
    if isinstance(hs, str):
        if hs in ("rh", "lh"):
            return 0 if hs == "rh" else 1
        raise ValueError(f"unexpected hand_side: {hs}")
    try:
        v = int(hs)
    except (TypeError, ValueError):
        raise ValueError(f"unexpected hand_side: {hs}") from None
    if v in (0, 1):
        return v
    raise ValueError(f"unexpected hand_side: {hs}")


def _stream_ptr(device: torch.device) -> int:
    return int(torch.cuda.current_stream(device).cuda_stream)


def _check(rc: int, ctx=None, L=None):
    if rc != 0:
        msg = (L or lib()).tamf_last_error(ctx)
        raise (TamfRangeError if rc == -6 else TamfError)(f"libtamf_hip error {rc}: {msg.decode() if msg else '?'}")


def _dev_f32(t: torch.Tensor, device: torch.device) -> torch.Tensor:
    return t.detach().to(device=device, dtype=torch.float32).contiguous()


def obj_num_vector(obj_num: Optional[Sequence[int]], B: int) -> Optional[np.ndarray]:
    if obj_num is None:
        return None
    num_np = np.ascontiguousarray(torch.as_tensor(obj_num).cpu().numpy() if isinstance(obj_num, torch.Tensor) else obj_num, dtype=np.int32)
    if num_np.shape != (B,):
        raise ValueError(f"obj_num must hold one count per clip: shape {num_np.shape} for B = {B}")
    return num_np


def encoder_batch(batch: Mapping, obj_num: Optional[Sequence[int]], device: torch.device, input_dim: int, n_labels: Optional[int] = None):
    side = [hand_side_code(hs) for hs in batch["hand_side"]]
    pr, sh = _dev_f32(batch["pose_repr"], device), _dev_f32(batch["shape"], device)
    oe, ot = _dev_f32(batch["obj_embedding"], device), _dev_f32(batch["obj_traj"], device)
    B, T, F = pr.shape
    nobj = ot.shape[1]
    if F != input_dim or tuple(sh.shape[:2]) != (B, T) or tuple(oe.shape[:2]) != (B, nobj) or tuple(ot.shape[:3]) != (B, nobj, T) \
            or len(side) != B or n_labels not in (None, B):
        raise ValueError(f"inconsistent encoder inputs: pose_repr {tuple(pr.shape)}, shape {tuple(sh.shape)}, obj_embedding "
                         f"{tuple(oe.shape)}, obj_traj {tuple(ot.shape)}, {len(side)} hand sides" + ("" if n_labels is None else f", {n_labels} labels"))
    return (pr, sh, oe, ot), (B, T, F, nobj), obj_num_vector(obj_num, B), torch.tensor(side, dtype=torch.uint8, device=device)


def require_gpu(device=None) -> torch.device:
    if not torch.cuda.is_available():
        raise TamfError("no MI355X/HIP device visible: the MF-MDM HIP path has no CPU fallback")
    dev = torch.device("cuda", torch.cuda.current_device()) if device is None else torch.device(device)
    if dev.type != "cuda":
        raise TamfError(f"HIP path needs a cuda (ROCm) device, got {dev}")
    if dev.index is None:
        dev = torch.device("cuda", torch.cuda.current_device())
    return dev


class TamfContext:

    def __init__(self, arch: Mapping[str, int], max_batch: int, max_frames: int, precision: Optional[str] = None,
                 device=None, kind: str = "G", range_check: bool = False):
        if precision is None:
            precision = "f32" if kind == "E" else DEFAULT_PRECISION
        self.device = require_gpu(device)
        self._L = lib()
        self.precision = precision
        self.range_check = bool(range_check) and precision == "f16x3"
        self.kind = kind
        a = _Arch(
            input_dim=int(arch.get("input_dim", 99)),
            obj_input_dim=int(arch.get("obj_input_dim", 9)),
            hand_shape_dim=int(arch.get("hand_shape_dim", 10)),
            obj_embed_dim=int(arch.get("obj_embed_dim", 768)),
            latent_dim=int(arch.get("latent_dim", 256)),
            ff_size=int(arch.get("ff_size", 1024)),
            num_layers=int(arch.get("num_layers", 8)),
            num_heads=int(arch.get("num_heads", 4)),
            clip_dim=int(arch.get("clip_dim", 512)),
            h2o_dim=int(arch.get("h2o_dim", 778)),
            kind=KINDS[kind],
        )
        self.input_dim = a.input_dim
        self.latent_dim = a.latent_dim
        self.h2o_dim = a.h2o_dim
        self.max_batch, self.max_frames = int(max_batch), int(max_frames)
        self._h = c_void_p()
        self.B = self.T = 0
        self.n_steps = 0
        self.max_timesteps = 0
        self._keep = []
        with torch.cuda.device(self.device):
            _check(self._L.tamf_ctx_create(ctypes.byref(a), max_batch, max_frames, PRECISIONS[precision],
                                           self.device.index, ctypes.byref(self._h)), None, self._L)

    def close(self):
        if getattr(self, "_h", None) and self._h.value:
            self._L.tamf_ctx_destroy(self._h)
            self._h = c_void_p()

    def __del__(self):
        try:
            self.close()
        except Exception:
            pass

    def _check(self, rc: int):
        _check(rc, self._h, self._L)

    def load_state_dict(self, sd: Mapping[str, torch.Tensor], max_timesteps: int = 5000, strict_weight_range: bool = False):
        L = self._L
        self.max_timesteps = int(max_timesteps)
        for name, t in sd.items():
            if not isinstance(t, torch.Tensor) or name.startswith("clip_model."):
                continue
            h = t.detach().to("cpu", torch.float32).contiguous()
            shape = (c_int64 * max(h.dim(), 1))(*(list(h.shape) or [1]))
            self._check(L.tamf_load_weight(self._h, name.encode(), c_void_p(h.data_ptr()), shape, max(h.dim(), 1)))
        with torch.cuda.device(self.device):
            self._check(L.tamf_finalize_weights(self._h, int(max_timesteps), c_void_p(_stream_ptr(self.device))))
        if strict_weight_range and self.precision == "f16x3" and (self.status_flags(clear=False) & STATUS_F16_WEIGHT_RANGE):
            note = L.tamf_last_error(self._h)
            raise TamfRangeError(note.decode() if note else "f16x3: a weight tensor's dynamic range exceeds the split-fp16 format")

    def set_schedule(self, coef1: np.ndarray, coef2: np.ndarray, log_variance_clipped: np.ndarray, timestep_map=None):
        c1 = np.ascontiguousarray(coef1, dtype=np.float64)
        c2 = np.ascontiguousarray(coef2, dtype=np.float64)
        lv = np.ascontiguousarray(log_variance_clipped, dtype=np.float64)
        assert c1.shape == c2.shape == lv.shape and c1.ndim == 1
        self.n_steps = int(c1.shape[0])
        self._check(self._L.tamf_set_schedule(self._h, self.n_steps, c1.ctypes.data_as(c_void_p), c2.ctypes.data_as(c_void_p),
                                            lv.ctypes.data_as(c_void_p)))
        if timestep_map is not None:
            tm = np.ascontiguousarray(timestep_map, dtype=np.int32)
            assert tm.shape == (self.n_steps,), (tm.shape, self.n_steps)
            if not np.array_equal(tm, np.arange(self.n_steps, dtype=np.int32)):
                with torch.cuda.device(self.device):
                    self._check(self._L.tamf_set_timestep_map(self._h, self.n_steps, tm.ctypes.data_as(c_void_p)))

    def set_cond(self, text_embedding: Optional[torch.Tensor], hand_side: Sequence, shape: torch.Tensor,
                 obj_embedding: torch.Tensor, obj_traj: torch.Tensor, obj_num: Optional[Sequence[int]] = None):
        side = [hand_side_code(hs) for hs in hand_side]
        B, nobj, T, _ = obj_traj.shape
        dev = self.device
        te = _dev_f32(text_embedding, dev) if text_embedding is not None else None
        sh, oe, ot = _dev_f32(shape, dev), _dev_f32(obj_embedding, dev), _dev_f32(obj_traj, dev)
        assert sh.shape[0] == B and sh.shape[1] == T and oe.shape[0] == B and oe.shape[1] == nobj
        side_np = np.asarray(side, dtype=np.uint8)
        assert side_np.shape[0] == B
        num_np = obj_num_vector(obj_num, B)
        if num_np is None and not hasattr(self._L, "tamf_set_cond_ragged"):
            with torch.cuda.device(dev):
                self._check(self._L.tamf_set_cond(self._h, B, T, nobj, c_void_p(te.data_ptr() if te is not None else 0), side_np.ctypes.data_as(c_void_p),
                                                c_void_p(sh.data_ptr()), c_void_p(oe.data_ptr()), c_void_p(ot.data_ptr()), c_void_p(_stream_ptr(dev))))
            self._keep = [te, sh, oe, ot]
            self.B, self.T = int(B), int(T)
            return
        with torch.cuda.device(dev):
            self._check(self._L.tamf_set_cond_ragged(self._h, B, T, nobj, num_np.ctypes.data_as(c_void_p) if num_np is not None else c_void_p(0),
                                                   c_void_p(te.data_ptr() if te is not None else 0), side_np.ctypes.data_as(c_void_p),
                                                   c_void_p(sh.data_ptr()), c_void_p(oe.data_ptr()), c_void_p(ot.data_ptr()),
                                                   c_void_p(_stream_ptr(dev))))
        self._keep = [te, sh, oe, ot]
        self.B, self.T = int(B), int(T)

    def _need_cond(self):
        if self.B <= 0:
            raise TamfError("conditioning not set (call set_cond first)")

    def denoise(self, x: torch.Tensor, t: torch.Tensor) -> torch.Tensor:
        self._need_cond()
        dev = self.device
        xd = _dev_f32(x, dev)
        assert tuple(xd.shape) == (self.B, self.input_dim, 1, self.T), (tuple(xd.shape), self.B, self.T)
        td = t.detach().to(device=dev, dtype=torch.int64).contiguous()
        assert td.shape == (self.B,), (tuple(td.shape), self.B)
        lo, hi = int(td.min()), int(td.max())
        if lo < 0 or hi >= self.max_timesteps:
            raise IndexError(f"timestep {lo if lo < 0 else hi} outside the timestep-embedding table [0, {self.max_timesteps})")
        out = torch.empty_like(xd)
        with torch.cuda.device(dev):
            self._check(self._L.tamf_denoise(self._h, c_void_p(xd.data_ptr()), c_void_p(td.data_ptr()), c_void_p(out.data_ptr()),
                                           c_void_p(_stream_ptr(dev))))
        self._raise_on_range()
        return out

    def encode(self, pose_repr: torch.Tensor, shape: torch.Tensor, hand_side: Sequence, obj_embedding: torch.Tensor,
               obj_traj: torch.Tensor, obj_num: Optional[Sequence[int]] = None, with_activation: bool = True):
        if self.kind != "E":
            raise TamfError(f"encode needs a SegmentEncoder context (kind 'E'), this one is kind {self.kind!r}")
        dev = self.device
        batch = dict(pose_repr=pose_repr, shape=shape, hand_side=hand_side, obj_embedding=obj_embedding, obj_traj=obj_traj)
        (pr, sh, oe, ot), (B, T, F, nobj), num_np, side_d = encoder_batch(batch, obj_num, dev, self.input_dim)
        enc = torch.empty(B, self.latent_dim, dtype=torch.float32, device=dev)
        act = torch.empty(B, F, dtype=torch.float32, device=dev) if with_activation else None
        with torch.cuda.device(dev):
            self._check(self._L.tamf_encode(self._h, B, T, nobj, num_np.ctypes.data_as(c_void_p) if num_np is not None else c_void_p(0),
                                            c_void_p(pr.data_ptr()), c_void_p(sh.data_ptr()), c_void_p(side_d.data_ptr()), c_void_p(oe.data_ptr()),
                                            c_void_p(ot.data_ptr()), c_void_p(enc.data_ptr()), c_void_p(act.data_ptr() if act is not None else 0),
                                            c_void_p(_stream_ptr(dev))))
        self._keep = [pr, sh, oe, ot, side_d]
        return enc, act

    def ddpm_step(self, x_t: torch.Tensor, x0: torch.Tensor, t: int, noise: Optional[torch.Tensor]) -> torch.Tensor:
        dev = self.device
        xt, x0d = _dev_f32(x_t, dev), _dev_f32(x0, dev)
        nz = _dev_f32(noise, dev) if noise is not None else None
        out = torch.empty_like(xt)
        with torch.cuda.device(dev):
            self._check(self._L.tamf_ddpm_step(self._h, c_void_p(xt.data_ptr()), c_void_p(x0d.data_ptr()), int(t),
                                             c_void_p(nz.data_ptr() if nz is not None else 0), c_void_p(out.data_ptr()),
                                             xt.numel(), c_void_p(_stream_ptr(dev))))
        return out

    def sample_loop(self, noise: Optional[torch.Tensor] = None, seed: int = 0, clip_id_base: int = 0,
                    dump: bool = False, use_graph: bool = True, out: Optional[torch.Tensor] = None):
        self._need_cond()
        dev = self.device
        shape = (self.B, self.input_dim, 1, self.T)
        nz = None
        if noise is not None:
            nz = _dev_f32(noise, dev)
            assert tuple(nz.shape) == (self.n_steps + 1,) + shape, (tuple(nz.shape), shape)
        if out is None:
            out = torch.empty(shape, device=dev, dtype=torch.float32)
        dmp = torch.empty((self.n_steps,) + shape, device=dev, dtype=torch.float32) if dump else None
        with torch.cuda.device(dev):
            self._check(self._L.tamf_sample_loop(self._h, c_void_p(nz.data_ptr() if nz is not None else 0), int(seed) & (2**64 - 1),
                                               int(clip_id_base), c_void_p(out.data_ptr()),
                                               c_void_p(dmp.data_ptr() if dmp is not None else 0), 1 if use_graph else 0,
                                               c_void_p(_stream_ptr(dev))))
        self._keep_loop = [nz, dmp]
        self._raise_on_range()
        return (out, dmp) if dump else out

    def _raise_on_range(self):
        if self.range_check and (self.status_flags(clear=True) & STATUS_F16_RANGE):
            raise TamfRangeError("f16x3: an activation beyond +-65504 was stored as a split-fp16 operand by this context; the result may "
                                 "differ from the reference's fp32 arithmetic (use precision='f32' or 'bf16x3')")

    def status_flags(self, clear: bool = True) -> int:
        v = ctypes.c_uint32(0)
        with torch.cuda.device(self.device):
            self._check(self._L.tamf_get_status_flags(self._h, ctypes.byref(v), 1 if clear else 0, c_void_p(_stream_ptr(self.device))))
        return int(v.value)

    def resize(self, max_batch: int, max_frames: int) -> None:
        with torch.cuda.device(self.device):
            self._check(self._L.tamf_ctx_resize(self._h, int(max_batch), int(max_frames)))
        self.max_batch, self.max_frames = int(max_batch), int(max_frames)
        self.B = self.T = 0
        self._keep = []

    def check_guards(self) -> int:
        n = c_int32(0)
        self._check(self._L.tamf_test_check_guards(self._h, ctypes.byref(n)))
        return int(n.value)

    def fill_scratch(self, byte: int = 0xFF) -> None:
        with torch.cuda.device(self.device):
            self._check(self._L.tamf_test_fill_scratch(self._h, int(byte)))

    def refine(self, sample_pose_repr: torch.Tensor, h2o_dist: torch.Tensor) -> torch.Tensor:
        dev = self.device
        xin, h2o = _dev_f32(sample_pose_repr, dev), _dev_f32(h2o_dist, dev)
        assert tuple(xin.shape) == (self.B, self.T, self.input_dim)
        assert tuple(h2o.shape) == (self.B, self.T, self.h2o_dim)
        out = torch.empty_like(xin)
        with torch.cuda.device(dev):
            self._check(self._L.tamf_refine(self._h, c_void_p(xin.data_ptr()), c_void_p(h2o.data_ptr()), c_void_p(out.data_ptr()),
                                          c_void_p(_stream_ptr(dev))))
        self._raise_on_range()
        return out

    def loop_stats(self):
        a, b = c_int32(), c_int32()
        self._check(self._L.tamf_loop_stats(self._h, ctypes.byref(a), ctypes.byref(b)))
        return int(a.value), int(b.value)

    @property
    def step_kernel_count(self) -> int:
        return int(self._L.tamf_step_kernel_count(self._h))

    def step_profile(self, max_n: int = 256):
        self._need_cond()
        ms = (c_float * max_n)()
        fl = (c_double * max_n)()
        names = ctypes.create_string_buffer(max_n * 48)
        with torch.cuda.device(self.device):
            n = self._L.tamf_step_profile(self._h, max_n, ms, fl, names, c_void_p(_stream_ptr(self.device)))
        if n < 0:
            self._check(n)
        out = []
        for i in range(n):
            nm = names.raw[i * 48:(i + 1) * 48].split(b"\0", 1)[0].decode()
            out.append((nm, float(ms[i]), float(fl[i])))
        return out


    def refine_profile(self, sample_pose_repr: torch.Tensor, h2o_dist: torch.Tensor, max_n: int = 256):
        dev = self.device
        xin, h2o = _dev_f32(sample_pose_repr, dev), _dev_f32(h2o_dist, dev)
        assert tuple(xin.shape) == (self.B, self.T, self.input_dim) and tuple(h2o.shape) == (self.B, self.T, self.h2o_dim)
        out = torch.empty_like(xin)
        ms, fl, names = (c_float * max_n)(), (c_double * max_n)(), ctypes.create_string_buffer(max_n * 48)
        with torch.cuda.device(dev):
            n = self._L.tamf_refine_profile(self._h, c_void_p(xin.data_ptr()), c_void_p(h2o.data_ptr()), c_void_p(out.data_ptr()), max_n,
                                          ms, fl, names, c_void_p(_stream_ptr(dev)))
        if n < 0:
            self._check(n)
        return [(names.raw[i * 48:(i + 1) * 48].split(b"\0", 1)[0].decode(), float(ms[i]), float(fl[i])) for i in range(n)]




def test_gemm(precision: str, a: torch.Tensor, w: torch.Tensor, bias: Optional[torch.Tensor], act: int = 0) -> torch.Tensor:
    dev = require_gpu(a.device)
    M, K = a.shape
    N = w.shape[0]
    c = torch.empty((M, N), device=dev, dtype=torch.float32)
    a, w = _dev_f32(a, dev), _dev_f32(w, dev)
    b = _dev_f32(bias, dev) if bias is not None else None
    _check(hooks().tamf_test_gemm(PRECISIONS[precision], M, N, K, c_void_p(a.data_ptr()), c_void_p(w.data_ptr()),
                                c_void_p(b.data_ptr() if b is not None else 0), act, c_void_p(c.data_ptr()),
                                c_void_p(_stream_ptr(dev))), None, hooks())
    return c


def block_stats(x: torch.Tensor) -> torch.Tensor:
    M, N = x.shape
    b = x.double().reshape(M, N // 32, 32)
    S = b.sum(-1)
    Q = ((b - S[..., None] / 32.0) ** 2).sum(-1)
    return torch.stack([S, Q], -1).float()


def test_gemm_resid(precision: str, a, w, bb, gamma, x, stats_in=None):
    dev = require_gpu(a.device)
    M, K = a.shape
    N = w.shape[0]
    a, w, bb, gamma = [_dev_f32(t, dev) for t in (a, w, bb, gamma)]
    y = _dev_f32(x, dev).clone()
    st_in = _dev_f32(stats_in, dev) if stats_in is not None else None
    st_out = torch.empty((M, N // 32, 2), device=dev, dtype=torch.float32)
    _check(hooks().tamf_test_gemm_resid(PRECISIONS[precision], M, N, K, c_void_p(a.data_ptr()), c_void_p(w.data_ptr()),
                                      c_void_p(bb.data_ptr()), c_void_p(gamma.data_ptr()),
                                      c_void_p(st_in.data_ptr() if st_in is not None else 0), c_void_p(y.data_ptr()),
                                      c_void_p(st_out.data_ptr()), c_void_p(_stream_ptr(dev))), None, hooks())
    return y, st_out


def test_attention(precision: str, qkv: torch.Tensor, H: int) -> torch.Tensor:
    dev = require_gpu(qkv.device)
    B, S, D3 = qkv.shape
    d = D3 // 3
    out = torch.empty((B, S, d), device=dev, dtype=torch.float32)
    q = _dev_f32(qkv, dev)
    _check(hooks().tamf_test_attention(PRECISIONS[precision], B, S, H, d // H, c_void_p(q.data_ptr()), c_void_p(out.data_ptr()),
                                     c_void_p(_stream_ptr(dev))), None, hooks())
    return out


def test_philox(seed: int, clip_id_base: int, draw: int, B: int, F: int, T: int, device=None) -> torch.Tensor:
    dev = require_gpu(device)
    out = torch.empty((B, F, 1, T), device=dev, dtype=torch.float32)
    _check(hooks().tamf_test_philox(seed, clip_id_base, draw, B, F, T, c_void_p(out.data_ptr()), c_void_p(_stream_ptr(dev))), None, hooks())
    torch.cuda.synchronize(dev)
    return out


def mfma_sustained_rate(precision: str, millis: int = 1500, device=None) -> Tuple[float, float]:
    dev = require_gpu(device)
    tf, mhz = ctypes.c_float(), ctypes.c_float()
    with torch.cuda.device(dev):
        _check(hooks().tamf_bench_mfma_rate(PRECISIONS[precision], int(millis), ctypes.byref(tf), ctypes.byref(mhz), c_void_p(_stream_ptr(dev))), None, hooks())
    return float(tf.value), float(mhz.value)
```

Before: 5198 frames/s.

## Write attention output in place over QK buffer and alias Vt into scratch

Attention now writes its output into the Q half of the QK buffer, using a new row stride ldo of 2*d, and the out-projection GEMM reads from there. The separate A buffer write and read goes away. Vt is also placed as a view inside the shared hidden scratch allocation when it fits, which shrinks the memory footprint. V tail masking is added so that stale or garbage data in padded Vt columns is zeroed rather than relying on zeroed memory. That adds a few AND operations per PV fragment.

```diff
diff --git a/oakink2-tamf_amd/csrc/tamf_attn.h b/oakink2-tamf_amd/csrc/tamf_attn.h
--- a/oakink2-tamf_amd/csrc/tamf_attn.h
+++ b/oakink2-tamf_amd/csrc/tamf_attn.h
@@ -6,6 +6,7 @@
   const typename Op::elem_t* qk;
   const typename Op::elem_t* vt;
   typename Op::elem_t* out;
+  int ldo;
   int S, Sp, Skp, d, H;
   int abl;
   int ksplit, nwq, hw;
@@ -39,6 +40,20 @@
     if constexpr (C::VROWB == 128) return ch ^ ((e >> 1) & 7);
     else return ch ^ swz_chunk<64>(e);
   }
+  static TAMF_DEV void vt_tail_bits(int Sp, int kb, int g, int& m0, int& m1) {
+    const int r = Sp - 32 * kb;
+    m0 = 4 * g < r ? -1 : 0;
+    m1 = 16 + 4 * g < r ? -1 : 0;
+  }
+  static TAMF_DEV void vt_tail_mask(int4& v0, int4& v1, int m0, int m1) {
+    if constexpr (Op::PREC == 0) {
+      v0.x &= m0; v0.y &= m0; v0.z &= m0; v0.w &= m0;
+      v1.x &= m1; v1.y &= m1; v1.z &= m1; v1.w &= m1;
+    } else {
+      v0.x &= m0; v0.y &= m0; v0.z &= m1; v0.w &= m1;
+      v1.x &= m0; v1.y &= m0; v1.z &= m1; v1.w &= m1;
+    }
+  }
   static constexpr int K_RPP = 1024 / C::KROWB, K_PIECES = C::K_BYTES / 1024;
   static constexpr int V_RPP = 1024 / C::VROWB, V_PIECES = C::V_BYTES / 1024;
 
@@ -110,13 +125,17 @@
     ps = groups_reduce<RedSum>(ps);
     l_run += ps;
 
+    int vm0 = -1, vm1 = -1;
+    if (kb == nkb - 1) vt_tail_bits(Sp, kb, g, vm0, vm1);
     if constexpr (Op::PREC == 0) {
 #pragma unroll
       for (int nt = 0; nt < NT16; ++nt) {
         const int e = nt * 16 + lr;
 #pragma unroll
         for (int t = 0; t < 2; ++t) {
-          const int4 vf = *(const int4*)(Vs + e * C::VSTR + vswz(t * 4 + g, e) * 16);
+          int4 vf = *(const int4*)(Vs + e * C::VSTR + vswz(t * 4 + g, e) * 16);
+          const int vm = t ? vm1 : vm0;
+          vf.x &= vm; vf.y &= vm; vf.z &= vm; vf.w &= vm;
           o[nt] = __builtin_amdgcn_mfma_f32_16x16x4f32(as_f(vf.x), st[t][0], o[nt], 0, 0, 0);
           o[nt] = __builtin_amdgcn_mfma_f32_16x16x4f32(as_f(vf.y), st[t][1], o[nt], 0, 0, 0);
           o[nt] = __builtin_amdgcn_mfma_f32_16x16x4f32(as_f(vf.z), st[t][2], o[nt], 0, 0, 0);
@@ -135,9 +154,11 @@
 #pragma unroll
       for (int nt = 0; nt < NT16; ++nt) {
         const int e = nt * 16 + lr;
-        const int4 vh = *(const int4*)(Vs + e * C::VSTR + vswz(g, e) * 16);
+        int4 vh = *(const int4*)(Vs + e * C::VSTR + vswz(g, e) * 16);
+        int4 vl = vh;
+        if constexpr (Op::SPLIT) vl = *(const int4*)(Vs + e * C::VSTR + vswz(4 + g, e) * 16);
+        vt_tail_mask(vh, vl, vm0, vm1);
         if constexpr (Op::SPLIT) {
-          const int4 vl = *(const int4*)(Vs + e * C::VSTR + vswz(4 + g, e) * 16);
           o[nt] = Op::mfma1(vl, ph, o[nt]);
           o[nt] = Op::mfma1(vh, pl, o[nt]);
         }
@@ -218,7 +239,7 @@
 #pragma unroll
   for (int nt = 0; nt < NT16; ++nt) {
     float v[4] = {o[nt][0] * inv, o[nt][1] * inv, o[nt][2] * inv, o[nt][3] * inv};
-    Op::template store<4>(aa.out, (row_base + q) * d + h * HD + nt * 16 + 4 * g, v);
+    Op::template store<4>(aa.out, (row_base + q) * aa.ldo + h * HD + nt * 16 + 4 * g, v);
   }
 }
 
@@ -336,7 +357,7 @@
     if constexpr (TWO) vf[1] = *(const int4*)(vb + nt * (16 * C::VSTR) + vo1);
   }
   static TAMF_DEV void pv(const char* __restrict__ Vs, char* __restrict__ dma_dst, const char* vbase, int kb0, int kb1, int dkb0,
-                          int dkb1, int Skp, int wave, int nw, int lane, const uint32_t (&ph)[NKB][4], const uint32_t (&pl)[NKB][4],
+                          int dkb1, int Sp, int Skp, int wave, int nw, int lane, const uint32_t (&ph)[NKB][4], const uint32_t (&pl)[NKB][4],
                           f32x4 (&o)[NT16], int abl, unsigned mask = ~0u) {
     const int lr = lane & 15, g = lane >> 4;
     const int vo0 = lr * C::VSTR + BLK::vswz(g, lr) * 16, vo1 = lr * C::VSTR + BLK::vswz(4 + g, lr) * 16;
@@ -349,6 +370,9 @@
         const int4 p_l = make_int4((int)pl[kb][0], (int)pl[kb][1], (int)pl[kb][2], (int)pl[kb][3]);
         constexpr int LA = 2;
         int4 vf[LA + 1][2];
+        const bool tail = (kb + 1) * 32 >= S_MIN;
+        int vm0 = -1, vm1 = -1;
+        if (tail) BLK::vt_tail_bits(Sp, kb, g, vm0, vm1);
 #pragma unroll
         for (int nt = 0; nt <= LA; ++nt) vf[nt][0] = vf[nt][1] = p_h;
 #pragma unroll
@@ -358,10 +382,10 @@
         for (int nt = 0; nt < NT16; ++nt) {
           if (nt + LA < NT16 && !(abl & 4)) vfrag(vb, nt + LA, vo0, vo1, vf[(nt + LA) % (LA + 1)]);
           __builtin_amdgcn_sched_barrier(0);
-          const int4 vh = vf[nt % (LA + 1)][0];
+          int4 vh = vf[nt % (LA + 1)][0], v1 = vf[nt % (LA + 1)][1];
+          if (tail) BLK::vt_tail_mask(vh, v1, vm0, vm1);
           if (!(abl & 2)) {
             if constexpr (Op::PREC == 0) {
-              const int4 v1 = vf[nt % (LA + 1)][1];
               o[nt] = __builtin_amdgcn_mfma_f32_16x16x4f32(as_f(vh.x), __builtin_bit_cast(float, ph[kb][0]), o[nt], 0, 0, 0);
               o[nt] = __builtin_amdgcn_mfma_f32_16x16x4f32(as_f(vh.y), __builtin_bit_cast(float, ph[kb][1]), o[nt], 0, 0, 0);
               o[nt] = __builtin_amdgcn_mfma_f32_16x16x4f32(as_f(vh.z), __builtin_bit_cast(float, ph[kb][2]), o[nt], 0, 0, 0);
@@ -372,7 +396,7 @@
               o[nt] = __builtin_amdgcn_mfma_f32_16x16x4f32(as_f(v1.w), __builtin_bit_cast(float, pl[kb][3]), o[nt], 0, 0, 0);
             } else {
               if constexpr (Op::SPLIT) {
-                const int4 vl = vf[nt % (LA + 1)][1];
+                const int4 vl = v1;
                 o[nt] = Op::mfma1(vl, p_h, o[nt]);
                 o[nt] = Op::mfma1(vh, p_l, o[nt]);
               }
@@ -494,10 +518,10 @@
   for (int nt = 0; nt < NT16; ++nt) o[nt] = f32x4{0.f, 0.f, 0.f, 0.f};
 
   __syncthreads();
-  R::pv(Vs, Ks, vbase, 0, n1, n1, nkb, aa.Skp, wave, nw, lane, ph, pl, o, abl, kmask);
+  R::pv(Vs, Ks, vbase, 0, n1, n1, nkb, Sp, aa.Skp, wave, nw, lane, ph, pl, o, abl, kmask);
   if (n1 < nkb) {
     __syncthreads();
-    R::pv(Ks, Vs, vbase, n1, nkb, 0, 0, aa.Skp, wave, nw, lane, ph, pl, o, abl, kmask);
+    R::pv(Ks, Vs, vbase, n1, nkb, 0, 0, Sp, aa.Skp, wave, nw, lane, ph, pl, o, abl, kmask);
   }
   if (idle) {
     if (aa.ksplit) __syncthreads();
@@ -528,7 +552,7 @@
 #pragma unroll
     for (int i = 0; i < 4; ++i) { w[i] = __builtin_amdgcn_exp2f(mi[i] - mg); lg += li[i] * w[i]; }
     const float invg = 1.0f / lg;
-    char* grow = (char*)aa.out + ((row_base + q0 + lr) * d + h * HD) * EB + hq * 128;
+    char* grow = (char*)aa.out + ((row_base + q0 + lr) * aa.ldo + h * HD) * EB + hq * 128;
 #pragma unroll
     for (int ch = 0; ch < NCH; ++ch) {
       if (ch != hq) continue;
@@ -560,7 +584,8 @@
   const float inv = 1.0f / l;
   constexpr int RS = 128;
   char* slot = (n1 < nkb ? Vs : Ks) + wave * (16 * RS);
-  char* gout = (char*)aa.out + ((row_base + q0) * d + h * HD) * EB;
+  char* gout = (char*)aa.out + ((row_base + q0) * aa.ldo + h * HD) * EB;
+  const long ldob = (long)aa.ldo * EB;
   const int srow = lane >> 3, spiece = lane & 7;
 #pragma unroll
   for (int ch = 0; ch < NCH; ++ch) {
@@ -587,7 +612,7 @@
       const int row = i * 8 + srow;
       const int4 w = *(const int4*)(slot + row * RS + ((spiece ^ (row & 7)) << 4));
       if (q0 + row < Sp && (NT16 >= TPC || spiece * 16 < NT16 * 16 * Op::EB))
-        *(int4*)(gout + (long)row * d * EB + ch * 128 + spiece * 16) = w;
+        *(int4*)(gout + row * ldob + ch * 128 + spiece * 16) = w;
     }
   }
   if (aa.ksplit) __syncthreads();
diff --git a/oakink2-tamf_amd/csrc/tamf_hip.hip b/oakink2-tamf_amd/csrc/tamf_hip.hip
--- a/oakink2-tamf_amd/csrc/tamf_hip.hip
+++ b/oakink2-tamf_amd/csrc/tamf_hip.hip
@@ -66,6 +66,7 @@
 struct Workspaces {
   int Bmax = 0, Tmax = 0;
   long Mmax = 0;
+  long vt_elems = 0;
   float *xs = nullptr, *cobj = nullptr, *X = nullptr, *pstatic = nullptr;
   OperandBuf xs_op, h1_op, X_op, QK_op, Vt_op, A_op, H_op;
   void *X_st = nullptr, *xs_st = nullptr;
@@ -226,17 +227,20 @@
   return 0;
 }
 
-static int place_scratch_views(tamf_ctx* ctx, const ScratchLayout& sl) {
+static int place_scratch_views(tamf_ctx* ctx, const ScratchLayout& sl, const VtPlacement& vp) {
   char* host = (char*)ctx->H_op.p;
   ctx->QK_op.p = host + sl.qk_off;
   ctx->A_op.p = host + sl.a_off;
   ctx->h1_op.p = host + sl.h1_off;
+  if (vp.view) ctx->Vt_op.p = host + vp.off;
   const size_t guard = g_guard_bytes.load();
   if (!guard) return 0;
-  const struct { size_t off, bytes; const char* tag; } views[3] = {{(size_t)sl.qk_off, (size_t)sl.qk_bytes, "view QK_op of H_op's allocation"},
+  const struct { size_t off, bytes; const char* tag; } views[4] = {{(size_t)vp.off, (size_t)vp.bytes, "view Vt_op of H_op's allocation"},
+                                                                  {(size_t)sl.qk_off, (size_t)sl.qk_bytes, "view QK_op of H_op's allocation"},
                                                                   {(size_t)sl.a_off, (size_t)sl.a_bytes, "view A_op of H_op's allocation"},
                                                                   {(size_t)sl.h1_off, (size_t)sl.h1_bytes, "view h1_op of H_op's allocation"}};
-  for (const auto& v : views) {
+  for (int i = vp.view ? 0 : 1; i < 4; ++i) {
+    const auto& v = views[i];
     HIPCHK(ctx, hipMemset(host + v.off - guard, GUARD_BYTE, guard));
     ctx->guards.push_back(GuardRec{host + v.off - guard, v.bytes, guard, v.tag, true});
   }
@@ -263,17 +267,20 @@
   else { A(alloc_operand(ctx, &ctx->xs_op, BT * ctx->XK, true)); ctx->xs_st = ctx->xs_op.p; }
   A(dev_alloc(ctx, (void**)&ctx->cobj, BT * d * 4));
   const ScratchLayout sl = scratch_layout(Mmax, BT, d, ctx->ff, ctx->EB, g_guard_bytes.load());
+  const long vt_elems = (long)max_batch * d * smax.Skp;
+  const VtPlacement vp = vt_placement(sl, vt_elems, ctx->EB, g_guard_bytes.load());
+  ctx->vt_elems = vt_elems;
   if (!sl.alias) A(alloc_operand(ctx, &ctx->h1_op, BT * d));
   A(dev_alloc(ctx, (void**)&ctx->X, Mmax * d * 4, true));
   if (ctx->prec == TAMF_PREC_F32) ctx->X_op.p = ctx->X;
   else { A(alloc_operand(ctx, &ctx->X_op, Mmax * d, true)); ctx->X_st = ctx->X_op.p; }
   if (!sl.alias) A(alloc_operand(ctx, &ctx->QK_op, Mmax * 2 * d, true));
-  A(alloc_operand(ctx, &ctx->Vt_op, (long)max_batch * d * smax.Skp, true));
+  if (!vp.view) A(alloc_operand(ctx, &ctx->Vt_op, vt_elems, true));
   if (!sl.alias) A(alloc_operand(ctx, &ctx->A_op, Mmax * d, true));
   if (!sl.alias) A(alloc_operand(ctx, &ctx->H_op, Mmax * ctx->ff, true));
   else {
-    A(dev_alloc(ctx, &ctx->H_op.p, sl.host_bytes, true));
-    A(place_scratch_views(ctx, sl));
+    A(dev_alloc(ctx, &ctx->H_op.p, vp.alloc_bytes, true));
+    A(place_scratch_views(ctx, sl, vp));
   }
   A(dev_alloc(ctx, (void**)&ctx->pstatic, (long)max_batch * ctx->P * d * 4, true));
   A(dev_alloc(ctx, (void**)&ctx->tcur, (long)max_batch * 4, true));
@@ -861,12 +868,12 @@
       HIPCHK(ctx, launch_qkv<Op>(ga, ep, B, Sp, st, [&](const char* name, int cols) { mark(name, BS * 2.0 * dd * cols); }));
     }
     {
-      AttnArgs<Op> aa{(const E*)ctx->QK_op.p, (const E*)ctx->Vt_op.p, (E*)ctx->A_op.p, S, Sp, ctx->Skp, d, ctx->H, 0};
+      AttnArgs<Op> aa{(const E*)ctx->QK_op.p, (const E*)ctx->Vt_op.p, (E*)ctx->QK_op.p, 2 * d, S, Sp, ctx->Skp, d, ctx->H, 0};
       HIPCHK(ctx, launch_attn<Op>(aa, B, ctx->hd, st));
       mark("attention", 4.0 * B * (double)S * S * dd);
     }
     {
-      GemmArgs<Op> ga{(const E*)ctx->A_op.p, d, (const E*)w.Wout.p, d, M, d, d, 0};
+      GemmArgs<Op> ga{(const E*)ctx->QK_op.p, 2 * d, (const E*)w.Wout.p, d, M, d, d, 0};
       EpiResid<Op> ep{w.bb_att, w.g_att, ctx->X, (E*)ctx->X_st, d, ctx->stat_att, ACT_NONE, {w.Wout.inv_scale, ctx->status}, ln_in};
       HIPCHK(ctx, launch_resid<Op>(ga, ep, B, Sp, st));
       mark("gemm_outproj", BS * 2.0 * dd * dd);
diff --git a/oakink2-tamf_amd/csrc/tamf_hip_hooks.h b/oakink2-tamf_amd/csrc/tamf_hip_hooks.h
--- a/oakink2-tamf_amd/csrc/tamf_hip_hooks.h
+++ b/oakink2-tamf_amd/csrc/tamf_hip_hooks.h
@@ -65,6 +65,7 @@
   HIPCHK(ctx, hipMemset(ctx->H_op.p, byte, M * ctx->ff * eb));
   HIPCHK(ctx, hipMemset(ctx->QK_op.p, byte, M * 2 * d * eb));
   HIPCHK(ctx, hipMemset(ctx->A_op.p, byte, M * d * eb));
+  HIPCHK(ctx, hipMemset(ctx->Vt_op.p, byte, (size_t)ctx->vt_elems * eb));
   HIPCHK(ctx, hipMemset(ctx->h1_op.p, byte, BT * d * eb));
   HIPCHK(ctx, hipDeviceSynchronize());
   return 0;
@@ -156,7 +157,7 @@
 }
 
 template <class Op>
-static int test_attn_impl(int B, int S, int H, int hd, const float* qkv, float* out, hipStream_t st) {
+static int test_attn_impl(int B, int S, int H, int hd, const float* qkv, float* out, hipStream_t st, bool inplace = false) {
   typedef typename Op::elem_t E;
   const int d = H * hd, Sp = round_up(S, 8), Skp = round_up(S, 32);
   const long M = (long)B * Sp;
@@ -167,13 +168,13 @@
   E* oo = (E*)tb.get(o_n * Op::EB);
   float* of = (float*)tb.get(o_n * 4);
   if (!qk || !vt || !oo || !of) return fail(nullptr, TAMF_ERR_NOMEM, "hipMalloc failed");
-  (void)hipMemsetAsync(vt, 0, vt_n * Op::EB, st);
+  (void)hipMemsetAsync(vt, inplace ? 0xFF : 0, vt_n * Op::EB, st);
   const float qscale = 1.4426950408889634f / sqrtf((float)hd);
   hipLaunchKernelGGL((qkv_pack_kernel<Op>), grid1d(M * 3 * d), dim3(256), 0, st, qkv, qk, vt, B, S, Sp, Skp, H, hd, qscale);
-  AttnArgs<Op> aa{qk, vt, oo, S, Sp, Skp, d, H, 0};
+  AttnArgs<Op> aa{qk, vt, inplace ? qk : oo, inplace ? 2 * d : d, S, Sp, Skp, d, H, 0};
   hipError_t e = launch_attn<Op>(aa, B, hd, st);
   if (e != hipSuccess) return fail(nullptr, TAMF_ERR_HIP, std::string("attn launch: ") + hipGetErrorString(e));
-  hipLaunchKernelGGL((unpack_operand_kernel<Op>), grid1d(M * d), dim3(256), 0, st, oo, of, M, d, d);
+  hipLaunchKernelGGL((unpack_operand_kernel<Op>), grid1d(M * d), dim3(256), 0, st, aa.out, of, M, d, aa.ldo);
   for (int b = 0; b < B; ++b)
     (void)hipMemcpyAsync(out + (size_t)b * S * d, of + (size_t)b * Sp * d, (size_t)S * d * 4, hipMemcpyDeviceToDevice, st);
   if (hipStreamSynchronize(st) != hipSuccess) return fail(nullptr, TAMF_ERR_HIP, "sync failed");
@@ -189,6 +190,16 @@
   hipStream_t st = (hipStream_t)stream;
   if (precision < 0 || precision > TAMF_PREC_F16X3) return fail(nullptr, TAMF_ERR_INVALID, "unknown precision");
   TAMF_WITH_OP(precision, return test_attn_impl<Op>(B, S, H, hd, qkv_dev, out_dev, st));
+  return 0;
+}
+
+extern "C" int tamf_test_attention_inplace(int32_t precision, int32_t B, int32_t S, int32_t H, int32_t hd, const float* qkv_dev,
+                                           float* out_dev, void* stream) {
+  TAMF_LAUNCH_LOCK;
+  if (B <= 0 || S <= 0 || H <= 0 || !(hd == 64 || hd == 128)) return fail(nullptr, TAMF_ERR_INVALID, "bad attention shape");
+  hipStream_t st = (hipStream_t)stream;
+  if (precision < 0 || precision > TAMF_PREC_F16X3) return fail(nullptr, TAMF_ERR_INVALID, "unknown precision");
+  TAMF_WITH_OP(precision, return test_attn_impl<Op>(B, S, H, hd, qkv_dev, out_dev, st, true));
   return 0;
 }
 
@@ -292,7 +303,7 @@
   if (!qk || !vt || !oo) return fail(nullptr, TAMF_ERR_NOMEM, "hipMalloc failed");
   hipLaunchKernelGGL((fill_operand_kernel<Op>), grid1d(qk_n / 8), dim3(256), 0, st, qk, qk_n, 5u);
   hipLaunchKernelGGL((fill_operand_kernel<Op>), grid1d(vt_n / 8), dim3(256), 0, st, vt, vt_n, 6u);
-  AttnArgs<Op> aa{qk, vt, oo, S, Sp, Skp, d, H, abl};
+  AttnArgs<Op> aa{qk, vt, oo, d, S, Sp, Skp, d, H, abl};
   hipEvent_t e0, e1;
   if (hipEventCreate(&e0) != hipSuccess || hipEventCreate(&e1) != hipSuccess) return fail(nullptr, TAMF_ERR_HIP, "event");
   hipError_t e = hipSuccess;
diff --git a/oakink2-tamf_amd/csrc/tamf_shapes.h b/oakink2-tamf_amd/csrc/tamf_shapes.h
--- a/oakink2-tamf_amd/csrc/tamf_shapes.h
+++ b/oakink2-tamf_amd/csrc/tamf_shapes.h
@@ -63,3 +63,23 @@
   }
   return s;
 }
+
+struct VtPlacement {
+  bool view;
+  unsigned long long off, bytes;
+  unsigned long long alloc_bytes;
+};
+static inline VtPlacement vt_placement(const ScratchLayout& s, long long vt_elems, int elem_bytes, unsigned long long guard) {
+  VtPlacement v{};
+  v.bytes = ((unsigned long long)vt_elems * elem_bytes + 255ull) / 256ull * 256ull;
+  v.alloc_bytes = s.host_bytes;
+  v.view = s.alias && s.qk_bytes + v.bytes <= s.hidden_bytes;
+  if (!v.view) return v;
+  if (guard == 0) {
+    v.off = s.qk_bytes;
+  } else {
+    v.off = s.host_bytes + guard;
+    v.alloc_bytes = v.off + v.bytes;
+  }
+  return v;
+}
diff --git a/oakink2-tamf_amd/oakink2_tamf_amd/_lib.py b/oakink2-tamf_amd/oakink2_tamf_amd/_lib.py
--- a/oakink2-tamf_amd/oakink2_tamf_amd/_lib.py
+++ b/oakink2-tamf_amd/oakink2_tamf_amd/_lib.py
@@ -38,7 +38,7 @@
     "tamf_get_status_flags", "tamf_step_kernel_count", "tamf_loop_stats", "tamf_step_profile", "tamf_refine_profile",
 ]
 HOOK_EXPORTS = [
-    "tamf_test_gemm", "tamf_test_gemm_resid", "tamf_test_attention", "tamf_test_philox", "tamf_test_set_guard_bytes", "tamf_test_check_guards",
+    "tamf_test_gemm", "tamf_test_gemm_resid", "tamf_test_attention", "tamf_test_attention_inplace", "tamf_test_philox", "tamf_test_set_guard_bytes", "tamf_test_check_guards",
     "tamf_test_poke", "tamf_test_fail_alloc_after", "tamf_test_fill_scratch", "tamf_bench_gemm", "tamf_bench_attention", "tamf_bench_mfma_rate", "tamf_set_gemm_tuning",
 ]
 EVAL_EXPORTS = [
diff --git a/oakink2-tamf_amd/oakink2_tamf_amd/hip_backend.py b/oakink2-tamf_amd/oakink2_tamf_amd/hip_backend.py
--- a/oakink2-tamf_amd/oakink2_tamf_amd/hip_backend.py
+++ b/oakink2-tamf_amd/oakink2_tamf_amd/hip_backend.py
@@ -81,6 +81,8 @@
         L.tamf_test_attention.argtypes = [c_int32, c_int32, c_int32, c_int32, c_int32, c_void_p, c_void_p, c_void_p]
         L.tamf_test_philox.argtypes = [c_uint64, c_int64, c_int32, c_int32, c_int32, c_int32, c_void_p, c_void_p]
         L.tamf_set_gemm_tuning.argtypes = [c_int32]
+    if hasattr(L, "tamf_test_attention_inplace"):
+        L.tamf_test_attention_inplace.argtypes = L.tamf_test_attention.argtypes
     if hasattr(L, "tamf_test_gemm_resid"):
         L.tamf_test_gemm_resid.argtypes = [c_int32, c_int32, c_int32, c_int32] + [c_void_p] * 8
     if hasattr(L, "tamf_test_set_guard_bytes"):
@@ -470,13 +472,14 @@
     return y, st_out
 
 
-def test_attention(precision: str, qkv: torch.Tensor, H: int) -> torch.Tensor:
+def test_attention(precision: str, qkv: torch.Tensor, H: int, inplace: bool = False) -> torch.Tensor:
     dev = require_gpu(qkv.device)
     B, S, D3 = qkv.shape
     d = D3 // 3
     out = torch.empty((B, S, d), device=dev, dtype=torch.float32)
     q = _dev_f32(qkv, dev)
-    _check(hooks().tamf_test_attention(PRECISIONS[precision], B, S, H, d // H, c_void_p(q.data_ptr()), c_void_p(out.data_ptr()),
+    fn = hooks().tamf_test_attention_inplace if inplace else hooks().tamf_test_attention
+    _check(fn(PRECISIONS[precision], B, S, H, d // H, c_void_p(q.data_ptr()), c_void_p(out.data_ptr()),
                                      c_void_p(_stream_ptr(dev))), None, hooks())
     return out
 
```

After: 5180 frames/s. No clear change (-0.4%).
